# rasoolims/ImageTranslate

Measured on AMD Instinct MI355X. Metric: train tokens/sec (whole node), 6L enc-dec d=512 seq128 b64, 1/2/4/8 GPU, higher is better.
Workload: dtype bf16; 1 GPU; 6L/6L enc-dec d=512 h=8 ff=2048 V=30000, src[64,128] tgt[64,128], synthetic random-token MT; global_batch=64, seq_len=128, parallelism=dp1, distinct_batches=8, directions=2

## Files before the change

imagetranslate_amd/_lib.py:

```python
import ctypes
import os
from ctypes import POINTER, Structure, c_char_p, c_float, c_int, c_int32, c_int64, c_uint64, c_void_p

_HERE = os.path.dirname(os.path.abspath(__file__))
LIB_PATH = os.environ.get("IMT_LIB") or os.path.join(_HERE, "libimt_hip.so")

IMT_F32, IMT_BF16 = 0, 1
IMT_NT, IMT_NN, IMT_TN = 0, 1, 2
IMT_AUX_NONE, IMT_AUX_GELU_FWD, IMT_AUX_DGELU, IMT_AUX_SPLITK_WS = 0, 1, 2, 3


class GemmArgs(Structure):
    _fields_ = [
        ("dtype", c_int32), ("layout", c_int32),
        ("M", c_int32), ("N", c_int32), ("K", c_int32),
        ("A", c_void_p), ("lda", c_int64),
        ("B", c_void_p), ("ldb", c_int64),
        ("C", c_void_p), ("ldc", c_int64),
        ("c_dtype", c_int32), ("accumulate", c_int32),
        ("bias", c_void_p),
        ("resid", c_void_p), ("ldr", c_int64),
        ("aux", c_void_p), ("ldaux", c_int64),
        ("aux_mode", c_int32), ("split_k", c_int32),
        ("alpha", c_float), ("dropout_p", c_float),
        ("dropout_seed", c_uint64),
        ("alpha_dev", c_void_p),
        ("a_colsum", c_void_p),
        ("force_general", c_int32),
        ("ln_gamma", c_void_p), ("ln_beta", c_void_p),
        ("ln_out", c_void_p), ("ld_ln", c_int64),
        ("ln_mean", c_void_p), ("ln_rstd", c_void_p),
        ("ln_eps", c_float),
        ("splitk_ws", c_void_p), ("splitk_ws_bytes", c_int64),
    ]


class AttnArgs(Structure):
    _fields_ = [
        ("dtype", c_int32),
        ("B", c_int32), ("H", c_int32), ("Tq", c_int32), ("Tk", c_int32), ("head_dim", c_int32),
        ("Q", c_void_p), ("ldq", c_int64),
        ("K", c_void_p), ("ldk", c_int64),
        ("V", c_void_p), ("ldv", c_int64),
        ("O", c_void_p), ("ldo", c_int64),
        ("lse", c_void_p),
        ("key_mask", c_void_p), ("query_mask", c_void_p), ("mask3d", c_void_p),
        ("causal", c_int32), ("scale", c_float), ("dropout_p", c_float),
        ("dropout_seed", c_uint64),
        ("dO", c_void_p), ("lddo", c_int64),
        ("dQ", c_void_p), ("lddq", c_int64),
        ("dK", c_void_p), ("lddk", c_int64),
        ("dV", c_void_p), ("lddv", c_int64),
        ("delta", c_void_p),
    ]


class ProfRow(Structure):
    _fields_ = [("kind", ctypes.c_char * 48), ("launches", c_int64), ("total_ms", ctypes.c_double),
                ("flops", ctypes.c_double), ("bytes", ctypes.c_double)]


class AttnBlock(Structure):
    _fields_ = [("qkv_w", c_int64), ("qkv_b", c_int64), ("o_w", c_int64), ("o_b", c_int64), ("ln_g", c_int64),
                ("ln_b", c_int64)]


class LayerDesc(Structure):
    _fields_ = [("self_attn", AttnBlock), ("cross_attn", AttnBlock),
                ("ff1_w", c_int64), ("ff1_b", c_int64), ("ff2_w", c_int64), ("ff2_b", c_int64),
                ("ln2_g", c_int64), ("ln2_b", c_int64), ("cross_kv_w", c_int64), ("cross_kv_b", c_int64)]


class StackDesc(Structure):
    _fields_ = [
        ("dtype", c_int32),
        ("d", c_int32), ("heads", c_int32), ("ff", c_int32), ("vocab", c_int32), ("max_pos", c_int32),
        ("n_types", c_int32), ("n_layers", c_int32),
        ("is_decoder", c_int32), ("reserved", c_int32),
        ("pad_id", c_int64),
        ("ln_eps", c_float), ("hidden_dropout", c_float), ("attn_dropout", c_float), ("reserved_f", c_float),
        ("emb_word", c_int64), ("emb_pos", c_int64), ("emb_type", c_int64), ("emb_ln_g", c_int64), ("emb_ln_b", c_int64),
        ("layers", POINTER(LayerDesc)),
        ("params", c_void_p),
        ("grads", c_void_p),
    ]


class StackIO(Structure):
    _fields_ = [
        ("B", c_int32), ("T", c_int32), ("Tk", c_int32), ("training", c_int32),
        ("ids", c_void_p), ("type_ids", c_void_p), ("pos_ids", c_void_p),
        ("key_mask", c_void_p), ("query_mask", c_void_p), ("mask3d", c_void_p),
        ("causal", c_int32), ("reserved", c_int32),
        ("enc_states", c_void_p), ("enc_mask", c_void_p),
        ("out", c_void_p),
        ("dropout_seed", c_uint64),
        ("d_out", c_void_p), ("d_enc_states", c_void_p),
        ("wait_events", POINTER(c_void_p)), ("n_wait_events", c_int32), ("reserved2", c_int32),
    ]


class AttnDecodeArgs(Structure):
    _fields_ = [
        ("dtype", c_int32),
        ("R", c_int32), ("H", c_int32), ("head_dim", c_int32), ("n_keys", c_int32), ("rep", c_int32),
        ("Q", c_void_p), ("ldq", c_int64),
        ("K", c_void_p), ("V", c_void_p), ("ld_row", c_int64), ("ld_pos", c_int64),
        ("slots", c_void_p), ("ld_slots", c_int64),
        ("key_mask", c_void_p), ("ld_mask", c_int64),
        ("O", c_void_p), ("ldo", c_int64),
        ("scale", c_float), ("reserved", c_int32),
    ]


class DecodeIO(Structure):
    _fields_ = [
        ("R", c_int32), ("rep", c_int32), ("pos", c_int32), ("Tk", c_int32), ("t_max", c_int32), ("r_max", c_int32),
        ("ids", c_void_p), ("type_ids", c_void_p), ("pos_ids", c_void_p), ("slots", c_void_p), ("enc_mask", c_void_p),
        ("self_cache", c_void_p), ("cross_kv", c_void_p), ("out", c_void_p),
    ]


class BeamArgs(Structure):
    _fields_ = [
        ("B", c_int32), ("beam", c_int32), ("rep", c_int32), ("V", c_int32), ("step", c_int32), ("t_max", c_int32),
        ("logits", c_void_p), ("ld", c_int64),
        ("scores_in", c_void_p), ("sizes_in", c_void_p), ("eos_in", c_void_p), ("max_lens", c_void_p),
        ("hist_in", c_void_p), ("slots_in", c_void_p),
        ("len_penalty_ratio", c_float), ("reserved", c_int32),
        ("pad_idx", c_int64), ("eos", c_int64),
        ("cand_scores", c_void_p), ("cand_idx", c_void_p),
        ("scores_out", c_void_p), ("sizes_out", c_void_p), ("eos_out", c_void_p),
        ("hist_out", c_void_p), ("slots_out", c_void_p), ("parent_out", c_void_p), ("tokens_out", c_void_p),
        ("eos_count", c_void_p),
    ]


class SampleArgs(Structure):
    _fields_ = [
        ("B", c_int32), ("n", c_int32), ("rep", c_int32), ("V", c_int32), ("step", c_int32), ("t_max", c_int32),
        ("logits", c_void_p), ("ld", c_int64),
        ("scores_in", c_void_p), ("eos_in", c_void_p), ("max_lens", c_void_p), ("hist_in", c_void_p), ("slots_in", c_void_p),
        ("temperature", c_float), ("topk", c_int32), ("seed", c_uint64),
        ("pad_idx", c_int64), ("eos", c_int64),
        ("scores_out", c_void_p), ("eos_out", c_void_p),
        ("hist_out", c_void_p), ("slots_out", c_void_p), ("parent_out", c_void_p), ("tokens_out", c_void_p),
        ("eos_count", c_void_p),
    ]


class MassArgs(Structure):
    _fields_ = [
        ("n_rows", c_int32), ("width", c_int32), ("recover_width", c_int32), ("n_special", c_int32), ("vocab", c_int32),
        ("mask_prob", c_float), ("seed", c_uint64), ("mask_id", c_int64), ("pad_id", c_int64),
        ("src_text", c_void_p), ("pad_indices", c_void_p), ("row_offsets", c_void_p), ("first", c_void_p),
        ("src_mask", c_void_p),
        ("to_recover", c_void_p), ("positions", c_void_p), ("targets", c_void_p),
    ]


class MlmArgs(Structure):
    _fields_ = [
        ("n_rows", c_int32), ("width", c_int32), ("n_special", c_int32), ("vocab", c_int32),
        ("mask_eos", c_int32), ("mask_prob", c_float), ("seed", c_uint64), ("mask_id", c_int64), ("eos_id", c_int64),
        ("texts", c_void_p), ("pads", c_void_p), ("ld_pads", c_int64),
        ("mask", c_void_p), ("idx", c_void_p), ("targets", c_void_p), ("count", c_void_p),
    ]


class ScoreArgs(Structure):
    _fields_ = [
        ("dtype", c_int32), ("N", c_int32), ("V", c_int32), ("K", c_int32),
        ("x", c_void_p), ("ldx", c_int64),
        ("w", c_void_p), ("ldw", c_int64),
        ("bias", c_void_p), ("target", c_void_p),
        ("logprob", c_void_p), ("lse", c_void_p),
        ("seg_offsets", c_void_p), ("n_seg", c_int32), ("normalize", c_int32),
        ("seg_score", c_void_p),
        ("ws", c_void_p), ("ws_bytes", c_int64),
    ]


class KnnArgs(Structure):
    _fields_ = [
        ("dtype", c_int32), ("N", c_int32), ("M", c_int32), ("K", c_int32), ("k", c_int32),
        ("x", c_void_p), ("ldx", c_int64),
        ("y", c_void_p), ("ldy", c_int64),
        ("index_base", c_int32), ("splits", c_int32),
        ("val", c_void_p), ("idx", c_void_p),
        ("ws", c_void_p), ("ws_bytes", c_int64),
    ]


class AlignArgs(Structure):
    _fields_ = [
        ("dtype", c_int32), ("B", c_int32), ("S", c_int32), ("T", c_int32), ("d", c_int32),
        ("x", c_void_p), ("ldx", c_int64), ("bsx", c_int64),
        ("y", c_void_p), ("ldy", c_int64), ("bsy", c_int64),
        ("xr", c_void_p), ("yr", c_void_p),
        ("min_sim", c_float), ("reserved", c_int32),
        ("link", c_void_p), ("fwd_idx", c_void_p), ("fwd_val", c_void_p), ("bwd_idx", c_void_p), ("bwd_val", c_void_p),
    ]


class ConvArgs(Structure):
    _fields_ = [
        ("dtype", c_int32),
        ("B", c_int32), ("H", c_int32), ("W", c_int32), ("Cin", c_int32), ("Cout", c_int32), ("KH", c_int32), ("KW", c_int32),
        ("stride", c_int32), ("pad_h", c_int32), ("pad_w", c_int32), ("relu", c_int32),
        ("x", c_void_p), ("w", c_void_p), ("y", c_void_p),
        ("scale", c_void_p), ("shift", c_void_p), ("residual", c_void_p),
    ]


_P = c_void_p
SIGNATURES = {
    "imt_version": (c_int, []),
    "imt_last_error": (c_char_p, []),
    "imt_gemm": (c_int, [POINTER(GemmArgs), _P]),
    "imt_gemm_grouped_tn": (c_int, [POINTER(GemmArgs), c_int, _P]),
    "imt_gemm_grouped_tile_order": (c_int, [POINTER(c_int), POINTER(c_int), c_int, c_int, POINTER(c_int), c_int]),
    "imt_gemm_splitk_ws_bytes": (c_int64, []),
    "imt_gemm_bias_residual_ln_supported": (c_int, [c_int, c_int, c_int]),
    "imt_gemm_bias_residual_ln": (c_int, [c_int, _P, c_int64, _P, c_int64, _P, _P, c_int64, _P, _P, _P, _P, c_int64, _P, _P, c_int, c_int,
                                          c_int, c_float, c_float, c_uint64, _P]),
    "imt_colsum": (c_int, [c_int, _P, c_int64, c_int, c_int, _P, _P, _P]),
    "imt_layernorm_fwd": (c_int, [c_int, _P, _P, _P, _P, _P, _P, c_int, c_int, c_float, c_float, c_uint64, _P]),
    "imt_add_layernorm_fwd": (c_int, [c_int, _P, _P, _P, _P, _P, _P, _P, _P, c_int, c_int, c_float, c_float, c_uint64, _P]),
    "imt_embed_ln_fwd": (c_int, [c_int, _P, _P, _P, _P, _P, _P, _P, _P, _P, _P, _P, _P, c_int, c_int, c_int, c_int, c_int, c_int, c_float,
                                 c_float, c_uint64, _P]),
    "imt_layernorm_bwd": (c_int, [c_int, _P, _P, _P, _P, _P, _P, _P, _P, c_int, c_int, c_float, c_uint64, _P, c_float,
                                  c_uint64, _P, _P]),
    "imt_embed_fwd": (c_int, [c_int, _P, _P, _P, _P, _P, _P, _P, c_int, c_int, c_int, c_int, c_int, c_int, _P]),
    "imt_embed_bwd": (c_int, [c_int, _P, _P, _P, _P, _P, _P, _P, c_int, c_int, c_int, c_int64, _P]),
    "imt_attention_fwd": (c_int, [POINTER(AttnArgs), _P]),
    "imt_attention_bwd": (c_int, [POINTER(AttnArgs), _P]),
    "imt_attention_bwd_proj_supported": (c_int, [c_int, c_int, c_int, c_int, c_int, c_int, c_int]),
    "imt_attention_bwd_proj": (c_int, [POINTER(AttnArgs), _P, c_int64, _P, c_int64, c_int, _P]),
    "imt_gather_rows": (c_int, [c_int, _P, c_int64, _P, _P, c_int64, c_int, c_int, _P]),
    "imt_scatter_rows": (c_int, [c_int, _P, c_int64, _P, _P, c_int64, c_int, c_int, _P]),
    "imt_log_softmax_fwd": (c_int, [c_int, _P, c_int64, _P, c_int64, _P, c_int, c_int, _P]),
    "imt_log_softmax_bwd": (c_int, [_P, c_int64, _P, c_int64, c_int, _P, c_int64, c_int, c_int, _P]),
    "imt_smoothed_nll_fwd": (c_int, [_P, c_int64, _P, _P, c_int, c_int, c_float, c_int64, _P]),
    "imt_smoothed_nll_bwd": (c_int, [_P, _P, _P, c_int64, c_int, c_int, c_float, c_int64, _P]),
    "imt_xent_fused_fwd_bwd": (c_int, [c_int, _P, c_int64, _P, _P, c_int, c_int, c_float, c_int64, c_float, _P]),
    "imt_score_ws_bytes": (c_int64, [c_int, c_int]),
    "imt_score_supported": (c_int, [c_int, c_int, c_int]),
    "imt_score_rows": (c_int, [POINTER(ScoreArgs), _P]),
    "imt_knn_ws_bytes": (c_int64, [c_int, c_int, c_int, c_int]),
    "imt_knn_supported": (c_int, [c_int, c_int]),
    "imt_knn_rows": (c_int, [POINTER(KnnArgs), _P]),
    "imt_align_supported": (c_int, [c_int, c_int]),
    "imt_align_pairs": (c_int, [POINTER(AlignArgs), _P]),
    "imt_scaled_sum": (c_int, [_P, c_int, c_float, _P, _P]),
    "imt_conv2d_supported": (c_int, [c_int, c_int, c_int, c_int, c_int]),
    "imt_conv2d": (c_int, [POINTER(ConvArgs), _P]),
    "imt_maxpool2d_3x3s2": (c_int, [c_int, _P, _P, c_int, c_int, c_int, c_int, _P]),
    "imt_image_nhwc": (c_int, [c_int, _P, _P, c_int, c_int, c_int, POINTER(c_float), POINTER(c_float), _P]),
    "imt_sumsq": (c_int, [_P, c_int64, _P, _P, _P]),
    "imt_ln_partial_reduce": (c_int, [_P, c_int, c_int, _P, _P, _P, _P]),
    "imt_clip_adam": (c_int, [_P, _P, _P, _P, _P, c_int64, _P, c_float, c_float, c_float, c_float, c_float, c_float,
                              c_int64, c_int, _P]),
    "imt_clip_scale": (c_int, [_P, c_int64, _P, c_float, c_float, _P]),
    "imt_cast_f32_to_bf16": (c_int, [_P, _P, c_int64, _P]),
    "imt_gated_mix": (c_int, [c_int, _P, _P, _P, _P, c_int64, c_int, _P]),
    "imt_add_rows_dropout": (c_int, [c_int, _P, c_int, _P, _P, c_int64, c_int, c_int, c_float, c_uint64, _P]),
    "imt_obj_rows": (c_int, [c_int, c_int, _P, _P, _P, _P, _P, _P, _P, c_int64, c_int, c_int, _P, _P]),
    "imt_relu_dropout": (c_int, [c_int, _P, c_int64, c_int, c_float, c_uint64, _P]),
    "imt_relu_dropout_bwd": (c_int, [c_int, _P, _P, _P, c_int64, c_int, c_float, c_uint64, _P]),
    "imt_obj_fold_w": (c_int, [_P, _P, c_int, c_int, _P]),
    "imt_obj_embed_grad": (c_int, [c_int, _P, _P, c_int64, _P, c_int64, c_int, _P]),
    "imt_gated_mix_bwd": (c_int, [c_int, _P, _P, _P, _P, _P, _P, _P, _P, c_int64, c_int, _P]),
    "imt_attn_pool_plan": (c_int, [c_int, c_int, c_int]),
    "imt_attn_pool_fwd": (c_int, [c_int, _P, _P, _P, _P, _P, _P, _P, c_int64, c_int, c_int, _P]),
    "imt_attn_pool_bwd": (c_int, [c_int, _P, _P, _P, _P, _P, _P, _P, _P, _P, _P, _P, _P, c_int64, c_int, c_int, _P]),
    "imt_contrastive": (c_int, [_P, _P, _P, _P, _P, _P, c_int, c_int, c_int, _P]),
    "imt_sent_pool_fwd": (c_int, [c_int, _P, _P, _P, _P, _P, _P, c_int64, c_int, c_int, c_float, c_uint64, _P]),
    "imt_sent_pool_bwd": (c_int, [c_int, _P, _P, _P, _P, _P, _P, _P, _P, _P, c_int64, c_int, c_int, c_float, c_uint64, _P]),
    "imt_l2_dist": (c_int, [c_int, _P, _P, _P, _P, _P, c_int, c_int64, _P]),
    "imt_sensim_loss": (c_int, [_P, _P, _P, _P, _P, _P, c_int, c_int, c_int, c_int, _P]),
    "imt_pair_dot": (c_int, [_P, _P, _P, c_int64, c_int, _P]),
    "imt_pair_dot_bwd": (c_int, [_P, _P, _P, _P, _P, c_int64, c_int, _P]),
    "imt_proposal_attn_ws_bytes": (c_int64, [c_int64, c_int, c_int, c_int]),
    "imt_proposal_attn_fwd": (c_int, [c_int, _P, _P, _P, _P, _P, _P, _P, _P, _P, c_int64, c_int, c_int, c_int, c_int64, c_int64, c_float, _P]),
    "imt_proposal_attn_bwd": (c_int, [c_int, _P, _P, _P, _P, _P, _P, _P, _P, _P, _P, _P, _P, _P, _P, c_int64, c_int64, c_int, c_int, c_int,
                                      c_int64, c_int64, _P]),
    "imt_comm_unique_id_bytes": (c_int, []),
    "imt_comm_get_unique_id": (c_int, [_P]),
    "imt_comm_init": (c_int, [_P, c_int, c_int, POINTER(c_void_p)]),
    "imt_comm_allreduce": (c_int, [_P, _P, c_int64, c_int, _P]),
    "imt_comm_broadcast": (c_int, [_P, _P, c_int64, c_int, c_int, _P]),
    "imt_comm_destroy": (c_int, [_P]),
    "imt_set_gemm_share_cus": (c_int, [c_int]),
    "imt_set_gemm_grouped_tall_min_tiles": (c_int, [c_int]),
    "imt_debug_spin": (c_int, [c_int, c_int, c_int, c_int64, _P]),
    "imt_abi_sizeof": (c_int, [ctypes.c_char_p]),
    "imt_prof_enable": (c_int, [c_int]),
    "imt_prof_report": (c_int, [POINTER(ProfRow), c_int]),
    "imt_stack_workspace_bytes": (c_int64, [POINTER(StackDesc), c_int, c_int, c_int]),
    "imt_stack_forward": (c_int, [POINTER(StackDesc), POINTER(StackIO), _P, c_int64, _P]),
    "imt_stack_backward": (c_int, [POINTER(StackDesc), POINTER(StackIO), _P, c_int64, c_int, c_int, _P]),
    "imt_attention_decode": (c_int, [POINTER(AttnDecodeArgs), _P]),
    "imt_decode_workspace_bytes": (c_int64, [POINTER(StackDesc), c_int]),
    "imt_decode_self_cache_bytes": (c_int64, [POINTER(StackDesc), c_int, c_int]),
    "imt_decode_cross_bytes": (c_int64, [POINTER(StackDesc), c_int, c_int]),
    "imt_decode_begin": (c_int, [POINTER(StackDesc), _P, c_int, c_int, _P, _P]),
    "imt_decode_step": (c_int, [POINTER(StackDesc), POINTER(DecodeIO), _P, c_int64, _P]),
    "imt_decode_check": (c_int, [POINTER(StackDesc), c_int, _P, _P]),
    "imt_beam_step": (c_int, [POINTER(BeamArgs), _P]),
    "imt_sample_step": (c_int, [POINTER(SampleArgs), _P]),
    "imt_select_plan": (c_int, [_P, c_int64, _P, c_int64, c_int, c_int, c_int, _P, _P, _P, _P]),
    "imt_mass_mask": (c_int, [POINTER(MassArgs), _P]),
    "imt_mass_unmask": (c_int, [_P, _P, _P, _P, c_int, c_int, _P]),
    "imt_mlm_mask": (c_int, [POINTER(MlmArgs), _P]),
}

_lib = None


class ImtError(RuntimeError):
    pass


ABI_STRUCTS = {"imt_gemm_args": GemmArgs, "imt_attn_args": AttnArgs, "imt_prof_row": ProfRow, "imt_attn_block": AttnBlock,
               "imt_layer_desc": LayerDesc, "imt_stack_desc": StackDesc, "imt_stack_io": StackIO,
               "imt_attn_decode_args": AttnDecodeArgs, "imt_decode_io": DecodeIO, "imt_beam_args": BeamArgs,
               "imt_mass_args": MassArgs, "imt_score_args": ScoreArgs, "imt_sample_args": SampleArgs,
               "imt_knn_args": KnnArgs, "imt_mlm_args": MlmArgs, "imt_align_args": AlignArgs,
               "imt_conv_args": ConvArgs}


def load():
    global _lib
    if _lib is not None:
        return _lib
    if not os.path.exists(LIB_PATH):
        raise ImtError(
            "imagetranslate_amd: HIP extension %s is missing -- build it with "
            "`python -c 'import __graft_entry__ as g; g.build()'` (there is no CPU fallback)" % LIB_PATH)
    lib = ctypes.CDLL(LIB_PATH)
    for name, (res, args) in SIGNATURES.items():
        fn = getattr(lib, name)
        fn.restype = res
        fn.argtypes = args
    for cname, cls in ABI_STRUCTS.items():
        want = lib.imt_abi_sizeof(cname.encode())
        if want != ctypes.sizeof(cls):
            raise ImtError("imagetranslate_amd: %s is %d bytes in %s but %d in this binding -- rebuild the library "
                           "(python -c 'import __graft_entry__ as g; g.build()')" % (cname, want, LIB_PATH, ctypes.sizeof(cls)))
    _lib = lib
    return lib


def check(rc: int, what: str):
    if rc != 0:
        msg = load().imt_last_error()
        raise ImtError("%s failed (rc=%d): %s" % (what, rc, msg.decode() if msg else ""))
```

imagetranslate_amd/csrc/common.hpp:

```cpp
#pragma once
#include <hip/hip_runtime.h>
#include <stdint.h>
#include <stdio.h>
#include <string.h>
#include "../../include/imt_hip.h"

typedef __bf16 bf16_t;
typedef __attribute__((ext_vector_type(4))) float f32x4;
typedef __attribute__((ext_vector_type(2))) float f32x2;
typedef __attribute__((ext_vector_type(8))) __bf16 bf16x8;
typedef __attribute__((ext_vector_type(4))) __bf16 bf16x4;
typedef __attribute__((ext_vector_type(2))) __bf16 bf16x2;
typedef __attribute__((ext_vector_type(4))) short s16x4;
typedef __attribute__((ext_vector_type(4))) unsigned int u32x4;
typedef __attribute__((ext_vector_type(2))) unsigned int u32x2;

#define IMT_WAVE 64
#define IMT_DEVICE __device__ __forceinline__

void imt_set_error(const char* fmt, ...);

#define IMT_CHECK_ARG(cond, ...)                       \
  do {                                                  \
    if (!(cond)) {                                      \
      imt_set_error(__VA_ARGS__);                       \
      return IMT_ERR_BAD_ARG;                           \
    }                                                   \
  } while (0)

#define IMT_CHECK_LAUNCH()                                                   \
  do {                                                                       \
    hipError_t e__ = hipGetLastError();                                      \
    if (e__ != hipSuccess) {                                                 \
      imt_set_error("%s:%d launch failed: %s", __FILE__, __LINE__,           \
                    hipGetErrorString(e__));                                 \
      return IMT_ERR_LAUNCH;                                                 \
    }                                                                        \
  } while (0)

static inline int imt_cdiv(long a, long b) { return (int)((a + b - 1) / b); }
static inline bool imt_ok_dtype(int t) { return t == IMT_F32 || t == IMT_BF16; }
static inline int imt_dtype_bytes(int t) { return t == IMT_BF16 ? 2 : 4; }
static inline int64_t imt_align256(int64_t bytes) { return (bytes + 255) / 256 * 256; }
template <typename T> struct ImtType { typedef T type; };
template <typename F> static inline int imt_by_dtype(int dtype, F&& f) {
  return dtype == IMT_F32 ? f(ImtType<float>()) : f(ImtType<bf16_t>());
}

bool imt_gemm_grouped_tall(const imt_gemm_args* list, int count);

bool imt_prof_enabled();
const char* imt_prof_intern(const char* kind, int M, int N, int K);
void* imt_prof_begin_launch(const char* kind, double flops, double bytes, hipStream_t st);
void imt_prof_end_launch(void* tok, hipStream_t st);
#include <stdlib.h>
struct ImtTrace {
  static constexpr int MAXB = 4096;
  static constexpr int RING = 64;
  unsigned long long* dev = nullptr;
  const char* kind; int blocks; hipStream_t st;
  struct Slot { const char* kind; int blocks; };
  static Slot* slots() { static Slot s[RING]; return s; }
  static int& count() { static int c = 0; return c; }
  static bool ring() { static const bool r = getenv("IMT_TRACE_RING") != nullptr; return r; }
  ImtTrace(const char* kind_, int blocks_, hipStream_t st_) : kind(kind_), blocks(blocks_), st(st_) {
    static const char* want = getenv("IMT_TRACE");
    if (!want || (strcmp(want, kind_) != 0 && strcmp(want, "all") != 0) || blocks_ > MAXB || blocks_ <= 0) return;
    static unsigned long long* buf = nullptr;
    const size_t slice = (size_t)MAXB * 8;
    if (!buf && hipMalloc(&buf, (ring() ? RING : 1) * slice * sizeof(unsigned long long)) != hipSuccess) return;
    const int slot = ring() ? count() % RING : 0;
    if (ring()) slots()[slot] = Slot{kind_, blocks_};
    dev = buf + slot * slice;
    if (!ring()) (void)hipMemsetAsync(dev, 0, sizeof(unsigned long long) * 8 * blocks_, st);
    else if (slot == 0) (void)hipMemsetAsync(buf, 0, RING * slice * sizeof(unsigned long long), st);
  }
  ~ImtTrace() {
    if (!dev) return;
    static unsigned long long h[MAXB * 8];
    if (ring()) {
      if (++count() % RING != 0) return;
      (void)hipStreamSynchronize(st);
      unsigned long long* base = dev - (size_t)((count() - 1) % RING) * MAXB * 8;
      unsigned long long origin = 0, prev_end = 0;
      for (int s = 0; s < RING; ++s) {
        const Slot& sl = slots()[s];
        (void)hipMemcpy(h, base + (size_t)s * MAXB * 8, sizeof(unsigned long long) * 8 * sl.blocks, hipMemcpyDeviceToHost);
        unsigned long long t0 = ~0ull, t1 = 0, s1 = 0;
        for (int i = 0; i < 8 * sl.blocks; ++i) {
          if (!h[i]) continue;
          if (h[i] < t0) t0 = h[i];
          if (h[i] > t1) t1 = h[i];
          if ((i & 7) == 0 && h[i] > s1) s1 = h[i];
        }
        if (!origin) origin = t0;
        fprintf(stderr, "[ring %2d] %-10s %5d wgs  start %9.2f  last-start +%6.2f  end +%6.2f  dark-before %6.2f us\n", s, sl.kind, sl.blocks,
                (t0 - origin) * 0.01, (s1 - t0) * 0.01, (t1 - t0) * 0.01, prev_end ? ((double)t0 - (double)prev_end) * 0.01 : 0.0);
        prev_end = t1;
      }
      return;
    }
    (void)hipStreamSynchronize(st);
    (void)hipMemcpy(h, dev, sizeof(unsigned long long) * 8 * blocks, hipMemcpyDeviceToHost);
    unsigned long long t0 = ~0ull, t1 = 0;
    double ph[8] = {0, 0, 0, 0, 0, 0, 0, 0};
    int last = 0;
    for (int b = 0; b < blocks; ++b)
      for (int k = 0; k < 8; ++k) {
        const unsigned long long v = h[8 * b + k];
        if (!v) continue;
        if (v < t0) t0 = v;
        if (v > t1) t1 = v;
        if (k > last) last = k;
      }
    for (int b = 0; b < blocks; ++b) {
      unsigned long long prev = h[8 * b];
      for (int k = 1; k <= last; ++k) { const unsigned long long v = h[8 * b + k]; if (v && prev) { ph[k] += (v - prev) * 0.01; prev = v; } }
    }
    fprintf(stderr, "[trace %s] %d workgroups, span %.2f us; mean phases (us):", kind, blocks, (t1 - t0) * 0.01);
    for (int k = 1; k <= last; ++k) fprintf(stderr, " %.2f", ph[k] / blocks);
    fprintf(stderr, "\n");
  }
};
#define IMT_STAMP(trace, k) do { if ((trace) && threadIdx.x == 0) (trace)[8 * blockIdx.x + (k)] = wall_clock64(); } while (0)

struct ImtProfScope {
  void* tok; hipStream_t st;
  ImtProfScope(const char* kind, double flops, double bytes, hipStream_t s)
      : tok(imt_prof_enabled() ? imt_prof_begin_launch(kind, flops, bytes, s) : nullptr), st(s) {}
  ~ImtProfScope() { if (tok) imt_prof_end_launch(tok, st); }
};

IMT_DEVICE int imt_xcd_block(int bid, int nwg) {
  const int q = nwg >> 3, r = nwg & 7, xcd = bid & 7, idx = bid >> 3;
  return (xcd < r ? xcd * (q + 1) : r * (q + 1) + (xcd - r) * q) + idx;
}

template <typename T> IMT_DEVICE float to_f32(T v);
template <> IMT_DEVICE float to_f32<float>(float v) { return v; }
template <> IMT_DEVICE float to_f32<bf16_t>(bf16_t v) { return (float)v; }
template <typename T> IMT_DEVICE T from_f32(float v);
template <> IMT_DEVICE float from_f32<float>(float v) { return v; }
template <> IMT_DEVICE bf16_t from_f32<bf16_t>(float v) { return (bf16_t)v; }

template <typename T> struct Vec4;
template <> struct Vec4<float> {
  typedef f32x4 type;
  static IMT_DEVICE f32x4 load(const float* p) { return *reinterpret_cast<const f32x4*>(p); }
  static IMT_DEVICE void store(float* p, f32x4 v) { *reinterpret_cast<f32x4*>(p) = v; }
  static IMT_DEVICE void store_wt(float* p, f32x4 v) {
    typedef float f32x2_t __attribute__((ext_vector_type(2)));
    const f32x2_t lo = {v[0], v[1]}, hi = {v[2], v[3]};
    __hip_atomic_store(reinterpret_cast<unsigned long long*>(p), __builtin_bit_cast(unsigned long long, lo), __ATOMIC_RELAXED, __HIP_MEMORY_SCOPE_AGENT);
    __hip_atomic_store(reinterpret_cast<unsigned long long*>(p) + 1, __builtin_bit_cast(unsigned long long, hi), __ATOMIC_RELAXED, __HIP_MEMORY_SCOPE_AGENT);
  }
  static IMT_DEVICE type load_raw(const float* p) { return *reinterpret_cast<const f32x4*>(p); }
  static IMT_DEVICE f32x4 cvt(type v) { return v; }
};
template <> struct Vec4<bf16_t> {
  typedef bf16x4 type;
  static IMT_DEVICE f32x4 load(const bf16_t* p) {
    bf16x4 v = *reinterpret_cast<const bf16x4*>(p);
    f32x4 r = {(float)v[0], (float)v[1], (float)v[2], (float)v[3]};
    return r;
  }
  static IMT_DEVICE void store(bf16_t* p, f32x4 v) {
    bf16x4 r = {(bf16_t)v[0], (bf16_t)v[1], (bf16_t)v[2], (bf16_t)v[3]};
    *reinterpret_cast<bf16x4*>(p) = r;
  }
  static IMT_DEVICE void store_wt(bf16_t* p, f32x4 v) {
    bf16x4 r = {(bf16_t)v[0], (bf16_t)v[1], (bf16_t)v[2], (bf16_t)v[3]};
    __hip_atomic_store(reinterpret_cast<unsigned long long*>(p), __builtin_bit_cast(unsigned long long, r), __ATOMIC_RELAXED,
                       __HIP_MEMORY_SCOPE_AGENT);
  }
  static IMT_DEVICE type load_raw(const bf16_t* p) { return *reinterpret_cast<const bf16x4*>(p); }
  static IMT_DEVICE f32x4 cvt(type v) {
    f32x4 r = {(float)v[0], (float)v[1], (float)v[2], (float)v[3]};
    return r;
  }
};

IMT_DEVICE float wave_sum(float v) {
#pragma unroll
  for (int o = 32; o > 0; o >>= 1) v += __shfl_xor(v, o, 64);
  return v;
}
IMT_DEVICE float wave_max(float v) {
#pragma unroll
  for (int o = 32; o > 0; o >>= 1) v = fmaxf(v, __shfl_xor(v, o, 64));
  return v;
}
IMT_DEVICE bool better(float sa, int ia, float sb, int ib) { return sa > sb || (sa == sb && ia < ib); }
IMT_DEVICE void wave_best(float& s, int& i) {
#pragma unroll
  for (int o = 32; o > 0; o >>= 1) {
    const float so = __shfl_xor(s, o, 64);
    const int io = __shfl_xor(i, o, 64);
    if (better(so, io, s, i)) { s = so; i = io; }
  }
}

IMT_DEVICE void erf_and_gauss(float z, float& erf_v, float& gauss) {
  const float x = fabsf(z) * 0.70710678118654752440f;
  const float e = __expf(-x * x);
  const float t = __builtin_amdgcn_rcpf(fmaf(0.3275911f, x, 1.0f));
  float p = fmaf(1.061405429f, t, -1.453152027f);
  p = fmaf(p, t, 1.421413741f);
  p = fmaf(p, t, -0.284496736f);
  p = fmaf(p, t, 0.254829592f);
  const float y = 1.0f - p * t * e;
  erf_v = copysignf(y, z);
  gauss = e;
}
typedef float f32x2 __attribute__((ext_vector_type(2)));
IMT_DEVICE f32x2 pk_fma(f32x2 a, f32x2 b, f32x2 c) { return __builtin_elementwise_fma(a, b, c); }
IMT_DEVICE void erf_and_gauss2(f32x2 z, f32x2& erf_v, f32x2& gauss) {
  const f32x2 x = __builtin_elementwise_abs(z) * 0.70710678118654752440f;
  const f32x2 a = x * x * -1.4426950408889634f;
  f32x2 e, t;
  e.x = __builtin_amdgcn_exp2f(a.x); e.y = __builtin_amdgcn_exp2f(a.y);
  const f32x2 d = pk_fma(x, f32x2{0.3275911f, 0.3275911f}, f32x2{1.f, 1.f});
  t.x = __builtin_amdgcn_rcpf(d.x); t.y = __builtin_amdgcn_rcpf(d.y);
  f32x2 p = pk_fma(t, f32x2{-1.061405429f, -1.061405429f}, f32x2{1.453152027f, 1.453152027f});
  p = pk_fma(p, t, f32x2{-1.421413741f, -1.421413741f});
  p = pk_fma(p, t, f32x2{0.284496736f, 0.284496736f});
  p = pk_fma(p, t, f32x2{-0.254829592f, -0.254829592f});
  const f32x2 y = pk_fma(p * t, e, f32x2{1.f, 1.f});
  erf_v.x = copysignf(y.x, z.x); erf_v.y = copysignf(y.y, z.y);
  gauss = e;
}
IMT_DEVICE f32x4 gelu_erf4(f32x4 v) {
  f32x2 lo = {v[0], v[1]}, hi = {v[2], v[3]}, e0, g0, e1, g1;
  erf_and_gauss2(lo, e0, g0);
  erf_and_gauss2(hi, e1, g1);
  lo = lo * 0.5f * (e0 + 1.0f);
  hi = hi * 0.5f * (e1 + 1.0f);
  return f32x4{lo.x, lo.y, hi.x, hi.y};
}
IMT_DEVICE f32x4 gelu_erf_grad4(f32x4 z) {
  f32x2 lo = {z[0], z[1]}, hi = {z[2], z[3]}, e0, g0, e1, g1;
  erf_and_gauss2(lo, e0, g0);
  erf_and_gauss2(hi, e1, g1);
  lo = pk_fma(lo * 0.39894228040143267794f, g0, (e0 + 1.0f) * 0.5f);
  hi = pk_fma(hi * 0.39894228040143267794f, g1, (e1 + 1.0f) * 0.5f);
  return f32x4{lo.x, lo.y, hi.x, hi.y};
}
IMT_DEVICE float gelu_erf(float z) {
  float er, ga;
  erf_and_gauss(z, er, ga);
  return 0.5f * z * (1.0f + er);
}
IMT_DEVICE float gelu_erf_grad(float z) {
  float er, ga;
  erf_and_gauss(z, er, ga);
  return 0.5f * (1.0f + er) + z * 0.39894228040143267794f * ga;
}

IMT_DEVICE uint32_t mix32(uint32_t x) {
  x ^= x >> 16; x *= 0x7feb352dU; x ^= x >> 15; x *= 0x846ca68bU; x ^= x >> 16;
  return x;
}
IMT_DEVICE float counter_uniform(uint64_t seed, uint32_t stream, uint32_t index) {
  uint32_t h = mix32(index ^ (uint32_t)seed);
  h = mix32(h + stream * 0x9e3779b9U + (uint32_t)(seed >> 32));
  return (float)(h >> 8) * (1.0f / 16777216.0f);
}
IMT_DEVICE uint32_t dropout_key(uint64_t seed) { return (uint32_t)seed ^ ((uint32_t)(seed >> 32) * 0x9e3779b9U); }
IMT_DEVICE void dropout_block(uint32_t key, uint64_t idx4, uint32_t& h_lo, uint32_t& h_hi) {
  h_lo = mix32(((uint32_t)idx4 ^ key) + (uint32_t)(idx4 >> 32) * 0x85ebca6bU);
  h_hi = mix32(h_lo + 0x9e3779b9U);
}
IMT_DEVICE bool dropout_draw(uint32_t h_lo, uint32_t h_hi, int e , uint32_t thresh16) {
  const uint32_t w = (e & 2) ? h_hi : h_lo;
  return ((e & 1) ? (w >> 16) : (w & 0xffffu)) >= thresh16;
}
IMT_DEVICE bool dropout_keep(uint64_t seed, uint64_t idx, uint32_t thresh16) {
  uint32_t lo, hi;
  dropout_block(dropout_key(seed), idx >> 2, lo, hi);
  return dropout_draw(lo, hi, (int)(idx & 3), thresh16);
}
IMT_DEVICE void dropout_apply4(f32x4& v, uint64_t seed, uint64_t idx0, uint32_t thresh16, float inv_keep) {
  uint32_t lo, hi;
  dropout_block(dropout_key(seed), idx0 >> 2, lo, hi);
  v[0] = (lo & 0xffffu) >= thresh16 ? v[0] * inv_keep : 0.f;
  v[1] = (lo >> 16) >= thresh16 ? v[1] * inv_keep : 0.f;
  v[2] = (hi & 0xffffu) >= thresh16 ? v[2] * inv_keep : 0.f;
  v[3] = (hi >> 16) >= thresh16 ? v[3] * inv_keep : 0.f;
}
IMT_DEVICE uint32_t attn_drop_word(uint32_t key, uint64_t pair_idx) {
  return mix32(((uint32_t)pair_idx ^ key) + (uint32_t)(pair_idx >> 32) * 0x85ebca6bU);
}
IMT_DEVICE uint32_t attn_drop_word(uint32_t key, uint32_t pair_idx) { return mix32(pair_idx ^ key); }
IMT_DEVICE bool attn_drop_keep(uint32_t word, int j, uint32_t thresh16) {
  return ((j & 1) ? (word >> 16) : (word & 0xffffu)) >= thresh16;
}
static inline uint32_t dropout_thresh(float p) {
  if (p <= 0.f) return 0u;
  double t = (double)p * 65536.0 + 0.5;
  if (t > 65535.0) t = 65535.0;
  if (t < 1.0) t = 1.0;
  return (uint32_t)t;
}
```

imagetranslate_amd/csrc/model.hip:

```cpp
#include "common.hpp"
#include "decode_fused.hpp"

namespace {

struct Carver {
  char* base; int64_t off;
  explicit Carver(void* b) : base(reinterpret_cast<char*>(b)), off(0) {}
  void* take(int64_t bytes) {
    void* p = base ? base + off : nullptr;
    off += (bytes + 255) & ~(int64_t)255;
    return p;
  }
};

struct AttnWs {
  void* qkv;
  void* kv;
  int64_t kv_ld;
  void* ctx;
  float* lse;
  void* pre_ln;
  float* mean; float* rstd;
  void* out;
};
struct LayerWs {
  AttnWs self_attn, cross;
  void* z; void* h;
  void* pre_ln2; float* mean2; float* rstd2;
  void* out;
};
struct StackWs {
  void* emb_sum; float* emb_mean; float* emb_rstd; void* x0;
  LayerWs* layers;
  void* d_run;
  void* dpre[3]; void* ddrop[3];
  void* d_ctx;
  void* d_ff;
  void* d_qkv;
  void* d_q;
  void* d_kv;
  void* d_emb;
  static constexpr int N_SCRATCH = 4;
  struct Scratch { void* dpre[3]; void* ddrop[3]; void* d_ctx; void* d_ff; void* d_qkv; void* d_q; void* d_kv; } scr[N_SCRATCH];
  void use_scratch(int l) {
    const Scratch& z = scr[l % N_SCRATCH];
    for (int i = 0; i < 3; ++i) { dpre[i] = z.dpre[i]; ddrop[i] = z.ddrop[i]; }
    d_ctx = z.d_ctx; d_ff = z.d_ff; d_qkv = z.d_qkv; d_q = z.d_q; d_kv = z.d_kv;
  }
  void* kv_all; void* d_kv_all;
  float* delta;
  float* ln_partial;
  float* ln_site(int site, int d) const { return ln_partial + (int64_t)site * IMT_LN_BWD_WS_FLOATS(d); }
  void* splitk; int64_t splitk_bytes;
  int64_t bytes;
};

constexpr int MAX_LAYERS = 64;

int64_t kv_w_off(const imt_stack_desc* m, const imt_layer_desc& p) { return p.cross_kv_w >= 0 ? p.cross_kv_w : p.cross_attn.qkv_w + (int64_t)m->d * m->d; }
int64_t kv_b_off(const imt_stack_desc* m, const imt_layer_desc& p) { return p.cross_kv_b >= 0 ? p.cross_kv_b : p.cross_attn.qkv_b + m->d; }
bool cross_kv_batched(const imt_stack_desc* m) {
  if (!m->is_decoder || m->n_layers < 2) return false;
  const int64_t d = m->d;
  for (int l = 0; l < m->n_layers; ++l) {
    const imt_layer_desc& p = m->layers[l];
    if (p.cross_attn.qkv_w < 0 || p.cross_kv_w < 0 || p.cross_kv_b < 0) return false;
    if (p.cross_kv_w != m->layers[0].cross_kv_w + (int64_t)l * 2 * d * d) return false;
    if (p.cross_kv_b != m->layers[0].cross_kv_b + (int64_t)l * 2 * d) return false;
  }
  return true;
}

void carve(const imt_stack_desc* m, int B, int T, int Tk, void* ws, StackWs& w, LayerWs* layers) {
  Carver c(ws);
  const int64_t N = (int64_t)B * T, Nk = (int64_t)B * Tk, d = m->d, ff = m->ff, es = imt_dtype_bytes(m->dtype);
  w.emb_sum = c.take(N * d * es); w.emb_mean = (float*)c.take(N * 4); w.emb_rstd = (float*)c.take(N * 4);
  w.x0 = c.take(N * d * es);
  w.layers = layers;
  const bool batched = cross_kv_batched(m);
  const int64_t L2d = (int64_t)m->n_layers * 2 * d;
  w.kv_all = w.d_kv_all = nullptr;
  if (batched) { w.kv_all = c.take(Nk * L2d * es); w.d_kv_all = c.take(Nk * L2d * es); }
  for (int l = 0; l < m->n_layers; ++l) {
    LayerWs& L = layers[l];
    AttnWs& s = L.self_attn;
    s.qkv = c.take(N * 3 * d * es); s.kv = nullptr; s.ctx = c.take(N * d * es);
    s.lse = (float*)c.take((int64_t)B * m->heads * T * 4);
    s.pre_ln = c.take(N * d * es); s.mean = (float*)c.take(N * 4); s.rstd = (float*)c.take(N * 4);
    s.out = c.take(N * d * es);
    AttnWs& x = L.cross;
    memset(&x, 0, sizeof(x));
    if (m->is_decoder && m->layers[l].cross_attn.qkv_w >= 0) {
      x.qkv = c.take(N * d * es); x.ctx = c.take(N * d * es);
      if (batched) { x.kv = w.kv_all ? (void*)((char*)w.kv_all + (int64_t)l * 2 * d * es) : nullptr; x.kv_ld = L2d; }
      else { x.kv = c.take(Nk * 2 * d * es); x.kv_ld = 2 * d; }
      x.lse = (float*)c.take((int64_t)B * m->heads * T * 4);
      x.pre_ln = c.take(N * d * es); x.mean = (float*)c.take(N * 4); x.rstd = (float*)c.take(N * 4);
      x.out = c.take(N * d * es);
    }
    L.z = c.take(N * ff * es); L.h = c.take(N * ff * es);
    L.pre_ln2 = c.take(N * d * es); L.mean2 = (float*)c.take(N * 4); L.rstd2 = (float*)c.take(N * 4);
    L.out = c.take(N * d * es);
  }
  w.d_run = c.take(N * d * es);
  for (int k = 0; k < StackWs::N_SCRATCH; ++k) {
    StackWs::Scratch& z = w.scr[k];
    for (int i = 0; i < 3; ++i) { z.dpre[i] = c.take(N * d * es); z.ddrop[i] = c.take(N * d * es); }
    z.d_ctx = c.take(N * d * es);
    z.d_ff = c.take(N * ff * es);
    z.d_qkv = c.take(N * 3 * d * es);
    z.d_q = c.take(N * d * es);
    z.d_kv = c.take((Nk > 0 ? Nk : 1) * 2 * d * es);
  }
  w.use_scratch(0);
  w.d_emb = c.take(N * d * es);
  w.delta = (float*)c.take((int64_t)B * m->heads * T * 4);
  w.ln_partial = (float*)c.take((int64_t)(3 * m->n_layers + 1) * IMT_LN_BWD_WS_FLOATS(d) * 4);
  w.splitk_bytes = ((N + 127) / 128) * ((d + 127) / 128) <= 128 ? imt_gemm_splitk_ws_bytes() : 0;
  w.splitk = w.splitk_bytes ? c.take(w.splitk_bytes) : nullptr;
  w.bytes = c.off;
}

struct Ctx {
  const imt_stack_desc* m; hipStream_t st; int dtype; int64_t es;
  void* splitk = nullptr; int64_t splitk_bytes = 0;
  const char* P(int64_t off) const { return reinterpret_cast<const char*>(m->params) + off * es; }
  float* G(int64_t off) const { return m->grads + off; }
};

#define RC(x) do { int rc__ = (x); if (rc__ != IMT_OK) return rc__; } while (0)

int linear_fwd(const Ctx& c, const void* x, int64_t ldx, int M, int K, int64_t w_off, int64_t b_off, int N, void* y, int64_t ldy,
               const void* resid, int64_t ldr, void* aux, int aux_mode, float drop_p, uint64_t seed) {
  imt_gemm_args a;
  memset(&a, 0, sizeof(a));
  a.dtype = c.dtype; a.layout = IMT_NT; a.M = M; a.N = N; a.K = K;
  a.A = x; a.lda = ldx; a.B = c.P(w_off); a.ldb = K; a.C = y; a.ldc = ldy; a.c_dtype = c.dtype;
  a.bias = b_off >= 0 ? c.P(b_off) : nullptr;
  a.resid = resid; a.ldr = ldr; a.aux = aux; a.ldaux = N; a.aux_mode = aux_mode; a.split_k = 1; a.alpha = 1.f;
  a.dropout_p = drop_p; a.dropout_seed = seed;
  a.splitk_ws = c.splitk; a.splitk_ws_bytes = c.splitk_bytes;
  return imt_gemm(&a, c.st);
}

int linear_bwd_input(const Ctx& c, const void* dy, int64_t lddy, int M, int N, int64_t w_off, int K, void* dx, int64_t lddx,
                     const void* resid, int64_t ldr, void* aux, int aux_mode, int accumulate) {
  imt_gemm_args a;
  memset(&a, 0, sizeof(a));
  a.dtype = c.dtype; a.layout = IMT_NN; a.M = M; a.N = K; a.K = N;
  a.A = dy; a.lda = lddy; a.B = c.P(w_off); a.ldb = K; a.C = dx; a.ldc = lddx; a.c_dtype = c.dtype;
  a.resid = resid; a.ldr = ldr; a.aux = aux; a.ldaux = K; a.aux_mode = aux_mode; a.split_k = 1; a.alpha = 1.f;
  a.accumulate = accumulate;
  a.splitk_ws = c.splitk; a.splitk_ws_bytes = c.splitk_bytes;
  return imt_gemm(&a, c.st);
}

bool fuse_dense_ln(const Ctx& c, int M, int N, int K) {
  static const int mode = getenv("IMT_GEMM_LN") ? atoi(getenv("IMT_GEMM_LN")) : -1;
  if (mode == 0 || !imt_gemm_bias_residual_ln_supported(c.dtype, N, K)) return false;
  if (mode == 1) return true;
  return N <= 256 && K <= 1024;
}
int dense_resid_ln(const Ctx& c, const void* x, int64_t ldx, int M, int K, int64_t w_off, int64_t b_off, int N, const void* resid,
                   int64_t g_off, int64_t beta_off, void* pre_ln, void* out, float* mean, float* rstd, float drop_p, uint64_t seed) {
  if (fuse_dense_ln(c, M, N, K))
    return imt_gemm_bias_residual_ln(c.dtype, x, ldx, c.P(w_off), K, b_off >= 0 ? c.P(b_off) : nullptr, resid, N, c.P(g_off), c.P(beta_off),
                                     pre_ln, out, N, mean, rstd, M, N, K, c.m->ln_eps, drop_p, seed, c.st);
  imt_gemm_args a;
  memset(&a, 0, sizeof(a));
  a.dtype = c.dtype; a.layout = IMT_NT; a.M = M; a.N = N; a.K = K;
  a.A = x; a.lda = ldx; a.B = c.P(w_off); a.ldb = K; a.C = pre_ln; a.ldc = N; a.c_dtype = c.dtype;
  a.bias = b_off >= 0 ? c.P(b_off) : nullptr;
  a.resid = resid; a.ldr = N; a.aux_mode = IMT_AUX_NONE; a.split_k = 1; a.alpha = 1.f;
  a.dropout_p = drop_p; a.dropout_seed = seed;
  a.ln_gamma = c.P(g_off); a.ln_beta = c.P(beta_off); a.ln_out = out; a.ld_ln = N; a.ln_mean = mean; a.ln_rstd = rstd;
  a.ln_eps = c.m->ln_eps;
  a.splitk_ws = c.splitk; a.splitk_ws_bytes = c.splitk_bytes;
  return imt_gemm(&a, c.st);
}

struct DeferredDW {
  imt_gemm_args list[16];
  int n = 0;
  bool hold_for_pair() const {
    if (n == 0 || 2 * n > 16) return false;
    imt_gemm_args two[16];
    for (int i = 0; i < n; ++i) two[i] = two[n + i] = list[i];
    return imt_gemm_grouped_tall(two, 2 * n);
  }
  void add(const Ctx& c, const void* dy, int64_t lddy, const void* x, int64_t ldx, int M, int N, int K, int64_t w_off, int64_t b_off) {
    imt_gemm_args& a = list[n++];
    memset(&a, 0, sizeof(a));
    a.dtype = c.dtype; a.layout = IMT_TN; a.M = N; a.N = K; a.K = M;
    a.A = dy; a.lda = lddy; a.B = x; a.ldb = ldx; a.C = c.G(w_off); a.ldc = K; a.c_dtype = IMT_F32; a.alpha = 1.f;
    a.split_k = 1; a.accumulate = 1;
    a.a_colsum = b_off >= 0 ? c.G(b_off) : nullptr;
    const int tiles = imt_cdiv(N, 128) * imt_cdiv(K, 128);
    int sk = 1;
    while (sk < 8 && tiles * sk * 2 <= 256 && M / (sk * 2) >= 512) sk *= 2;
    if (M % (c.dtype == IMT_BF16 ? 64 : 32) != 0) { a.split_k = sk; a.accumulate = (sk == 1); }
  }
  int flush(hipStream_t st) {
    const int rc = n ? imt_gemm_grouped_tn(list, n, st) : IMT_OK;
    n = 0;
    return rc;
  }
};

struct SideQueue {
  hipStream_t st = nullptr;
  hipEvent_t ready[MAX_LAYERS], done[MAX_LAYERS];
  bool ok = false;
  bool init() {
    if (st) return ok;
    if (hipStreamCreateWithFlags(&st, hipStreamNonBlocking) != hipSuccess) { st = (hipStream_t)1; return ok = false; }
    for (int i = 0; i < MAX_LAYERS; ++i)
      if (hipEventCreateWithFlags(&ready[i], hipEventDisableTiming) != hipSuccess ||
          hipEventCreateWithFlags(&done[i], hipEventDisableTiming) != hipSuccess) return ok = false;
    return ok = true;
  }
};
SideQueue g_side;

uint64_t site_seed(uint64_t base, int layer, int site) { return base + 0x9E3779B97F4A7C15ull * (uint64_t)(layer * 16 + site + 1); }

struct MaskSet { const uint8_t* key; const uint8_t* query; const uint8_t* m3d; int causal; };

inline const char* offp(const void* p, int64_t elems, int64_t es) { return reinterpret_cast<const char*>(p) + elems * es; }
inline char* offp(void* p, int64_t elems, int64_t es) { return reinterpret_cast<char*>(p) + elems * es; }

imt_attn_args attn_block_args(const Ctx& c, const AttnWs& w, bool cross, int B, int T, int Tk, const MaskSet& ms, float drop_p,
                              uint64_t seed) {
  const int d = c.m->d;
  imt_attn_args a;
  memset(&a, 0, sizeof(a));
  a.dtype = c.dtype; a.B = B; a.H = c.m->heads; a.Tq = T; a.Tk = cross ? Tk : T; a.head_dim = d / c.m->heads;
  a.Q = w.qkv; a.ldq = cross ? d : 3 * d;
  if (cross) { a.K = w.kv; a.ldk = w.kv_ld; a.V = offp(w.kv, d, c.es); a.ldv = w.kv_ld; }
  else       { a.K = offp(w.qkv, d, c.es); a.ldk = 3 * d; a.V = offp(w.qkv, 2 * d, c.es); a.ldv = 3 * d; }
  a.O = w.ctx; a.ldo = d; a.lse = w.lse;
  a.key_mask = ms.key; a.query_mask = ms.query; a.mask3d = ms.m3d; a.causal = ms.causal;
  a.scale = 1.0f / sqrtf((float)a.head_dim);
  a.dropout_p = drop_p; a.dropout_seed = seed;
  return a;
}

int attn_block_fwd(const Ctx& c, const imt_attn_block& p, AttnWs& w, const void* x, int B, int T, const void* kv_src, int Tk,
                   const MaskSet& ms, bool training, uint64_t seed, int layer, int site0, int64_t kv_w = -1, int64_t kv_b = -1,
                   bool kv_ready = false) {
  const int d = c.m->d;
  const int N = B * T;
  const float hp = training ? c.m->hidden_dropout : 0.f, ap = training ? c.m->attn_dropout : 0.f;
  if (!kv_src) {
    RC(linear_fwd(c, x, d, N, d, p.qkv_w, p.qkv_b, 3 * d, w.qkv, 3 * d, nullptr, 0, nullptr, IMT_AUX_NONE, 0.f, 0));
  } else {
    const int Nk = B * Tk;
    RC(linear_fwd(c, x, d, N, d, p.qkv_w, p.qkv_b, d, w.qkv, d, nullptr, 0, nullptr, IMT_AUX_NONE, 0.f, 0));
    if (!kv_ready)
      RC(linear_fwd(c, kv_src, d, Nk, d, kv_w, kv_b, 2 * d, w.kv, w.kv_ld, nullptr, 0, nullptr, IMT_AUX_NONE, 0.f, 0));
  }
  const imt_attn_args a = attn_block_args(c, w, kv_src != nullptr, B, T, Tk, ms, ap, site_seed(seed, layer, site0));
  RC(imt_attention_fwd(&a, c.st));
  RC(dense_resid_ln(c, w.ctx, d, N, d, p.o_w, p.o_b, d, x, p.ln_g, p.ln_b, w.pre_ln, w.out, w.mean, w.rstd, hp, site_seed(seed, layer, site0 + 1)));
  return IMT_OK;
}

int attn_block_bwd(const Ctx& c, const imt_attn_block& p, AttnWs& w, StackWs& sw, DeferredDW& dw, int slot, const void* x, int B, int T,
                   const void* kv_src, int Tk, const MaskSet& ms, bool training, uint64_t seed, int layer, int site0, const void* dy,
                   void* d_kv_src, int accumulate_kv, int64_t kv_w = -1, int64_t kv_b = -1, void* d_kv_batched = nullptr) {
  const int d = c.m->d;
  const int N = B * T;
  const float hp = training ? c.m->hidden_dropout : 0.f, ap = training ? c.m->attn_dropout : 0.f;
  void* d_pre = sw.dpre[slot];
  void* d_dense = (hp > 0.f) ? sw.ddrop[slot] : d_pre;
  RC(imt_layernorm_bwd(c.dtype, dy, w.pre_ln, c.P(p.ln_g), w.mean, w.rstd, d_pre, c.G(p.ln_g), c.G(p.ln_b), N, d, 0.f, 0,
                       (hp > 0.f) ? d_dense : nullptr, hp, site_seed(seed, layer, site0 + 1), sw.ln_site(3 * layer + slot, d), c.st));
  dw.add(c, d_dense, d, w.ctx, d, N, d, d, p.o_w, p.o_b);
  imt_attn_args a = attn_block_args(c, w, kv_src != nullptr, B, T, Tk, ms, ap, site_seed(seed, layer, site0));
  const bool proj = imt_attention_bwd_proj_supported(a.dtype, a.head_dim, a.H, a.Tq, a.Tk, d, ms.m3d != nullptr);
  if (!proj) RC(linear_bwd_input(c, d_dense, d, N, d, p.o_w, d, sw.d_ctx, d, nullptr, 0, nullptr, IMT_AUX_NONE, 0));
  a.dO = proj ? nullptr : sw.d_ctx; a.lddo = d;
  a.delta = sw.delta;
  auto attn_bwd = [&]() { return proj ? imt_attention_bwd_proj(&a, d_dense, d, c.P(p.o_w), d, d, c.st) : imt_attention_bwd(&a, c.st); };
  if (!kv_src) {
    a.dQ = sw.d_qkv; a.lddq = 3 * d; a.dK = offp(sw.d_qkv, d, c.es); a.lddk = 3 * d; a.dV = offp(sw.d_qkv, 2 * d, c.es); a.lddv = 3 * d;
    RC(attn_bwd());
    dw.add(c, sw.d_qkv, 3 * d, x, d, N, 3 * d, d, p.qkv_w, p.qkv_b);
    RC(linear_bwd_input(c, sw.d_qkv, 3 * d, N, 3 * d, p.qkv_w, d, sw.d_run, d, d_pre, d, nullptr, IMT_AUX_NONE, 0));
  } else {
    const int Nk = B * Tk;
    void* dkv = d_kv_batched ? d_kv_batched : sw.d_kv;
    const int64_t lddkv = d_kv_batched ? w.kv_ld : 2 * d;
    a.dQ = sw.d_q; a.lddq = d; a.dK = dkv; a.lddk = lddkv; a.dV = offp(dkv, d, c.es); a.lddv = lddkv;
    RC(attn_bwd());
    dw.add(c, sw.d_q, d, x, d, N, d, d, p.qkv_w, p.qkv_b);
    RC(linear_bwd_input(c, sw.d_q, d, N, d, p.qkv_w, d, sw.d_run, d, d_pre, d, nullptr, IMT_AUX_NONE, 0));
    dw.add(c, dkv, lddkv, kv_src, d, Nk, 2 * d, d, kv_w, kv_b);
    if (!d_kv_batched) {
      if (d_kv_src)
        RC(linear_bwd_input(c, sw.d_kv, 2 * d, Nk, 2 * d, kv_w, d, d_kv_src, d, nullptr, 0, nullptr, IMT_AUX_NONE, accumulate_kv));
    }
  }
  return IMT_OK;
}

int ffn_fwd(const Ctx& c, const imt_layer_desc& p, LayerWs& w, const void* x, int N, bool training, uint64_t seed, int layer) {
  const int d = c.m->d, ff = c.m->ff;
  const float hp = training ? c.m->hidden_dropout : 0.f;
  RC(linear_fwd(c, x, d, N, d, p.ff1_w, p.ff1_b, ff, w.h, ff, nullptr, 0, w.z, IMT_AUX_GELU_FWD, 0.f, 0));
  RC(dense_resid_ln(c, w.h, ff, N, ff, p.ff2_w, p.ff2_b, d, x, p.ln2_g, p.ln2_b, w.pre_ln2, w.out, w.mean2, w.rstd2, hp, site_seed(seed, layer, 8)));
  return IMT_OK;
}

int ffn_bwd(const Ctx& c, const imt_layer_desc& p, LayerWs& w, StackWs& sw, DeferredDW& dw, const void* x, int N, bool training,
            uint64_t seed, int layer, const void* dy) {
  const int d = c.m->d, ff = c.m->ff;
  const float hp = training ? c.m->hidden_dropout : 0.f;
  void* d_pre = sw.dpre[0];
  void* d_dense = (hp > 0.f) ? sw.ddrop[0] : d_pre;
  RC(imt_layernorm_bwd(c.dtype, dy, w.pre_ln2, c.P(p.ln2_g), w.mean2, w.rstd2, d_pre, c.G(p.ln2_g), c.G(p.ln2_b), N, d, 0.f, 0,
                       (hp > 0.f) ? d_dense : nullptr, hp, site_seed(seed, layer, 8), sw.ln_site(3 * layer, d), c.st));
  dw.add(c, d_dense, d, w.h, ff, N, d, ff, p.ff2_w, p.ff2_b);
  RC(linear_bwd_input(c, d_dense, d, N, d, p.ff2_w, ff, sw.d_ff, ff, nullptr, 0, w.z, IMT_AUX_DGELU, 0));
  dw.add(c, sw.d_ff, ff, x, d, N, ff, d, p.ff1_w, p.ff1_b);
  RC(linear_bwd_input(c, sw.d_ff, ff, N, ff, p.ff1_w, d, sw.d_run, d, d_pre, d, nullptr, IMT_AUX_NONE, 0));
  return IMT_OK;
}

int validate(const imt_stack_desc* m, const imt_stack_io* io, const void* ws, int64_t ws_bytes, StackWs& w, LayerWs* layers) {
  IMT_CHECK_ARG(m && io, "stack: null descriptor");
  IMT_CHECK_ARG(imt_ok_dtype(m->dtype), "stack: bad dtype");
  IMT_CHECK_ARG(m->n_layers >= 0 && m->n_layers <= MAX_LAYERS && (m->n_layers == 0 || m->layers), "stack: bad layer table");
  IMT_CHECK_ARG(m->d > 0 && m->heads > 0 && m->d % m->heads == 0, "stack: hidden size %d not a multiple of heads %d", m->d, m->heads);
  const int dh = m->d / m->heads;
  IMT_CHECK_ARG(dh == 32 || dh == 64, "stack: head_dim %d unsupported (32 or 64)", dh);
  IMT_CHECK_ARG(m->d % 8 == 0 && m->ff % 8 == 0, "stack: d and ff must be multiples of 8");
  IMT_CHECK_ARG(io->B > 0 && io->T > 0, "stack: empty batch");
  IMT_CHECK_ARG(io->T <= m->max_pos || io->pos_ids, "stack: sequence longer than max_position_embeddings");
  IMT_CHECK_ARG(m->params && io->ids && io->out, "stack: null tensor");
  if (m->is_decoder) IMT_CHECK_ARG(io->enc_states && io->Tk > 0, "stack: decoder needs encoder states");
  carve(m, io->B, io->T, m->is_decoder ? io->Tk : 0, const_cast<void*>(ws), w, layers);
  IMT_CHECK_ARG(ws && ws_bytes >= w.bytes, "stack: workspace too small (%lld < %lld)", (long long)ws_bytes, (long long)w.bytes);
  IMT_CHECK_ARG(((uintptr_t)ws & 255) == 0, "stack: workspace must be 256-B aligned");
  return IMT_OK;
}

}

extern "C" int64_t imt_stack_workspace_bytes(const imt_stack_desc* m, int B, int T, int Tk) {
  if (!m || m->n_layers > MAX_LAYERS || (m->n_layers > 0 && !m->layers)) return -1;
  StackWs w; LayerWs layers[MAX_LAYERS];
  carve(m, B, T, m->is_decoder ? Tk : 0, nullptr, w, layers);
  return w.bytes;
}

extern "C" int imt_stack_forward(const imt_stack_desc* m, const imt_stack_io* io, void* ws, int64_t ws_bytes, void* stream) {
  StackWs w; LayerWs layers[MAX_LAYERS];
  RC(validate(m, io, ws, ws_bytes, w, layers));
  Ctx c{m, (hipStream_t)stream, m->dtype, imt_dtype_bytes(m->dtype)};
  c.splitk = w.splitk; c.splitk_bytes = w.splitk_bytes;
  const int B = io->B, T = io->T, N = B * T, d = m->d;
  const bool training = io->training != 0;
  const uint64_t seed = io->dropout_seed;
  void* x0 = (m->n_layers == 0) ? io->out : w.x0;
  auto wait_site = [&](int k) {
    if (io->wait_events && k < io->n_wait_events && io->wait_events[k])
      (void)hipStreamWaitEvent(c.st, (hipEvent_t)const_cast<void*>(io->wait_events[k]), 0);
  };
  wait_site(0);
  RC(imt_embed_ln_fwd(c.dtype, io->ids, io->pos_ids, io->type_ids, c.P(m->emb_word), c.P(m->emb_pos), c.P(m->emb_type), c.P(m->emb_ln_g),
                      c.P(m->emb_ln_b), w.emb_sum, x0, w.emb_mean, w.emb_rstd, N, T, d, m->vocab, m->max_pos, m->n_types, m->ln_eps,
                      training ? m->hidden_dropout : 0.f, site_seed(seed, 1000, 0), c.st));
  const void* x = x0;
  const MaskSet self_ms{io->key_mask, io->query_mask, io->mask3d, io->causal};
  const MaskSet cross_ms{io->enc_mask, nullptr, nullptr, 0};
  const bool batched = cross_kv_batched(m);
  if (batched)
    RC(linear_fwd(c, io->enc_states, d, B * io->Tk, d, m->layers[0].cross_kv_w, m->layers[0].cross_kv_b, m->n_layers * 2 * d, w.kv_all,
                  (int64_t)m->n_layers * 2 * d, nullptr, 0, nullptr, IMT_AUX_NONE, 0.f, 0));
  for (int l = 0; l < m->n_layers; ++l) {
    const imt_layer_desc& p = m->layers[l];
    LayerWs& L = layers[l];
    wait_site(1 + l);
    RC(attn_block_fwd(c, p.self_attn, L.self_attn, x, B, T, nullptr, 0, self_ms, training, seed, l, 0));
    const void* a = L.self_attn.out;
    if (m->is_decoder && p.cross_attn.qkv_w >= 0) {
      RC(attn_block_fwd(c, p.cross_attn, L.cross, a, B, T, io->enc_states, io->Tk, cross_ms, training, seed, l, 4, kv_w_off(m, p),
                        kv_b_off(m, p), batched));
      a = L.cross.out;
    }
    if (l == m->n_layers - 1) L.out = io->out;
    RC(ffn_fwd(c, p, L, a, N, training, seed, l));
    x = L.out;
  }
  return IMT_OK;
}

extern "C" int imt_stack_backward(const imt_stack_desc* m, const imt_stack_io* io, void* ws, int64_t ws_bytes, int layer_lo,
                                  int layer_hi, void* stream) {
  StackWs w; LayerWs layers[MAX_LAYERS];
  RC(validate(m, io, ws, ws_bytes, w, layers));
  IMT_CHECK_ARG(m->grads && io->d_out, "stack_backward: grads / d_out missing");
  IMT_CHECK_ARG(0 <= layer_lo && layer_lo <= layer_hi && layer_hi <= m->n_layers, "stack_backward: bad layer range");
  Ctx c{m, (hipStream_t)stream, m->dtype, imt_dtype_bytes(m->dtype)};
  c.splitk = w.splitk; c.splitk_bytes = w.splitk_bytes;
  const int B = io->B, T = io->T, N = B * T, d = m->d;
  const bool training = io->training != 0;
  const uint64_t seed = io->dropout_seed;
  const MaskSet self_ms{io->key_mask, io->query_mask, io->mask3d, io->causal};
  const MaskSet cross_ms{io->enc_mask, nullptr, nullptr, 0};
  const void* dy = (layer_hi == m->n_layers) ? io->d_out : w.d_run;
  const bool batched = cross_kv_batched(m);
  DeferredDW dw;
  const int64_t lnf = IMT_LN_BWD_WS_FLOATS(d);
  if (layer_hi > layer_lo) (void)hipMemsetAsync(w.ln_site(3 * layer_lo, d), 0, (size_t)(3 * (layer_hi - layer_lo)) * lnf * 4, c.st);
  if (layer_lo == 0) (void)hipMemsetAsync(w.ln_site(3 * m->n_layers, d), 0, (size_t)lnf * 4, c.st);
  static const bool side_env = !(getenv("IMT_DW_SIDE_STREAM") && atoi(getenv("IMT_DW_SIDE_STREAM")) == 0);
  const bool whole = layer_lo == 0 && layer_hi == m->n_layers && m->n_layers >= 2;
  const bool side = side_env && !imt_prof_enabled() && whole && g_side.init();
  const bool pairs = whole && !imt_prof_enabled();
  int last_side = -1;
  int held = -1;
  for (int l = layer_hi - 1; l >= layer_lo; --l) {
    const imt_layer_desc& p = m->layers[l];
    LayerWs& L = layers[l];
    w.use_scratch(l);
    if (side && l + StackWs::N_SCRATCH < layer_hi) (void)hipStreamWaitEvent(c.st, g_side.done[l + StackWs::N_SCRATCH], 0);
    if (l == m->n_layers - 1) L.out = io->out;
    const bool has_cross = m->is_decoder && p.cross_attn.qkv_w >= 0;
    const void* x_in = (l == 0) ? w.x0 : (const void*)layers[l - 1].out;
    const void* a_self = L.self_attn.out;
    const void* a_ffn_in = has_cross ? L.cross.out : a_self;
    RC(ffn_bwd(c, p, L, w, dw, a_ffn_in, N, training, seed, l, dy));
    if (has_cross) {
      const bool first_cross = (l == m->n_layers - 1);
      void* dkv_l = batched ? offp(w.d_kv_all, (int64_t)l * 2 * d, c.es) : nullptr;
      RC(attn_block_bwd(c, p.cross_attn, L.cross, w, dw, 1, a_self, B, T, io->enc_states, io->Tk, cross_ms, training, seed, l, 4, w.d_run,
                        io->d_enc_states, first_cross ? 0 : 1, kv_w_off(m, p), kv_b_off(m, p), dkv_l));
    }
    RC(attn_block_bwd(c, p.self_attn, L.self_attn, w, dw, 2, x_in, B, T, nullptr, 0, self_ms, training, seed, l, 0, w.d_run, nullptr, 0));
    const bool first_of_pair = pairs && held < 0 && l > layer_lo && dw.hold_for_pair();
    if (first_of_pair) {
      held = l;
    } else if (side) {
      (void)hipEventRecord(g_side.ready[l], c.st);
      (void)hipStreamWaitEvent(g_side.st, g_side.ready[l], 0);
      RC(dw.flush(g_side.st));
      (void)hipEventRecord(g_side.done[l], g_side.st);
      if (held >= 0) (void)hipEventRecord(g_side.done[held], g_side.st);
      held = -1;
      last_side = l;
    } else {
      RC(dw.flush(c.st));
      held = -1;
    }
    dy = w.d_run;
  }
  if (layer_lo == 0 && batched) {
    const int Nk = B * io->Tk;
    const int L2d = m->n_layers * 2 * d;
    if (io->d_enc_states)
      RC(linear_bwd_input(c, w.d_kv_all, L2d, Nk, L2d, m->layers[0].cross_kv_w, d, io->d_enc_states, d, nullptr, 0, nullptr, IMT_AUX_NONE, 0));
  }
  if (layer_lo == 0) {
    const void* dy0 = (m->n_layers == 0) ? io->d_out : dy;
    RC(imt_layernorm_bwd(c.dtype, dy0, w.emb_sum, c.P(m->emb_ln_g), w.emb_mean, w.emb_rstd, w.d_emb, c.G(m->emb_ln_g), c.G(m->emb_ln_b), N, d,
                         training ? m->hidden_dropout : 0.f, site_seed(seed, 1000, 0), nullptr, 0.f, 0, w.ln_site(3 * m->n_layers, d), c.st));
    RC(imt_embed_bwd(c.dtype, io->ids, io->pos_ids, io->type_ids, w.d_emb, c.G(m->emb_word), c.G(m->emb_pos), c.G(m->emb_type), N, T, d,
                     m->pad_id, c.st));
  }
  {
    static int64_t g_off[3 * MAX_LAYERS + 1], b_off[3 * MAX_LAYERS + 1];
    const int first = 3 * layer_lo, emb = 3 * m->n_layers;
    const int last = (layer_lo == 0) ? emb + 1 : 3 * layer_hi;
    for (int sidx = first; sidx < last; ++sidx) {
      g_off[sidx - first] = -1; b_off[sidx - first] = -1;
      if (sidx == emb) { g_off[sidx - first] = m->emb_ln_g; b_off[sidx - first] = m->emb_ln_b; continue; }
      const int l = sidx / 3, slot = sidx % 3;
      if (l >= layer_hi) continue;
      const imt_layer_desc& p = m->layers[l];
      if (slot == 0) { g_off[sidx - first] = p.ln2_g; b_off[sidx - first] = p.ln2_b; }
      else if (slot == 2) { g_off[sidx - first] = p.self_attn.ln_g; b_off[sidx - first] = p.self_attn.ln_b; }
      else if (m->is_decoder && p.cross_attn.qkv_w >= 0) { g_off[sidx - first] = p.cross_attn.ln_g; b_off[sidx - first] = p.cross_attn.ln_b; }
    }
    if (last > first) RC(imt_ln_partial_reduce(w.ln_site(first, d), last - first, d, g_off, b_off, m->grads, c.st));
  }
  if (last_side >= 0) (void)hipStreamWaitEvent(c.st, g_side.done[last_side], 0);
  return IMT_OK;
}

namespace {

struct DecodeWs {
  void* emb_sum; void* x; void* ctx; void* pre_ln; void* a; void* q; void* b; void* h; void* z; float* mean; float* rstd;
  void* splitk; int64_t splitk_bytes;
  char* fused; int64_t fused_layer_bytes; unsigned* fused_bar;
  int64_t bytes;
};

bool fused_decode_shape(const imt_stack_desc* m) {
  return m->dtype == IMT_BF16 && imt_decode_fused_shape(m->d, m->heads, m->ff, m->n_layers);
}

void carve_decode(const imt_stack_desc* m, int r_max, void* ws, DecodeWs& w) {
  Carver c(ws);
  const int64_t R = r_max, d = m->d, ff = m->ff, es = imt_dtype_bytes(m->dtype);
  w.emb_sum = c.take(R * d * es); w.x = c.take(R * d * es); w.ctx = c.take(R * d * es); w.pre_ln = c.take(R * d * es);
  w.a = c.take(R * d * es); w.q = c.take(R * d * es); w.b = c.take(R * d * es);
  w.h = c.take(R * ff * es); w.z = c.take(R * ff * es);
  w.mean = (float*)c.take(R * 4); w.rstd = (float*)c.take(R * 4);
  w.splitk_bytes = imt_gemm_splitk_ws_bytes();
  w.splitk = c.take(w.splitk_bytes);
  w.fused = nullptr; w.fused_layer_bytes = 0; w.fused_bar = nullptr;
  if (fused_decode_shape(m)) {
    w.fused_layer_bytes = (imt_decode_fused_layer_bytes(r_max, m->d, m->ff) + 255) & ~(int64_t)255;
    w.fused = (char*)c.take(w.fused_layer_bytes * m->n_layers);
    w.fused_bar = (unsigned*)c.take(IMT_FUSED_BAR_WORDS * sizeof(unsigned));
  }
  w.bytes = c.off;
}

int validate_decoder(const imt_stack_desc* m) {
  IMT_CHECK_ARG(m, "decode: null descriptor");
  IMT_CHECK_ARG(imt_ok_dtype(m->dtype), "decode: bad dtype");
  IMT_CHECK_ARG(m->is_decoder, "decode: stack is not a decoder");
  IMT_CHECK_ARG(m->n_layers > 0 && m->n_layers <= MAX_LAYERS && m->layers, "decode: bad layer table");
  IMT_CHECK_ARG(m->d > 0 && m->heads > 0 && m->d % m->heads == 0, "decode: hidden size %d not a multiple of heads %d", m->d, m->heads);
  const int dh = m->d / m->heads;
  IMT_CHECK_ARG(dh == 32 || dh == 64, "decode: head_dim %d unsupported (32 or 64)", dh);
  IMT_CHECK_ARG(m->d % 8 == 0 && m->ff % 8 == 0, "decode: d and ff must be multiples of 8");
  IMT_CHECK_ARG(m->params, "decode: null parameter buffer");
  for (int l = 0; l < m->n_layers; ++l)
    IMT_CHECK_ARG(m->layers[l].cross_attn.qkv_w >= 0, "decode: layer %d has no crossattention block", l);
  return IMT_OK;
}

}

extern "C" int64_t imt_decode_workspace_bytes(const imt_stack_desc* m, int r_max) {
  if (!m || r_max <= 0) return -1;
  DecodeWs w;
  carve_decode(m, r_max, nullptr, w);
  return w.bytes;
}
extern "C" int64_t imt_decode_self_cache_bytes(const imt_stack_desc* m, int r_max, int t_max) {
  if (!m || r_max <= 0 || t_max <= 0) return -1;
  return (int64_t)m->n_layers * r_max * t_max * 3 * m->d * imt_dtype_bytes(m->dtype);
}
extern "C" int64_t imt_decode_cross_bytes(const imt_stack_desc* m, int B, int Tk) {
  if (!m || B <= 0 || Tk <= 0) return -1;
  return (int64_t)m->n_layers * B * Tk * 2 * m->d * imt_dtype_bytes(m->dtype);
}

extern "C" int imt_decode_begin(const imt_stack_desc* m, const void* enc_states, int B, int Tk, void* cross_kv, void* stream) {
  RC(validate_decoder(m));
  IMT_CHECK_ARG(enc_states && cross_kv && B > 0 && Tk > 0, "decode_begin: bad arguments");
  Ctx c{m, (hipStream_t)stream, m->dtype, imt_dtype_bytes(m->dtype)};
  const int d = m->d;
  const int64_t per_layer = (int64_t)B * Tk * 2 * d;
  for (int l = 0; l < m->n_layers; ++l) {
    const imt_attn_block& p = m->layers[l].cross_attn;
    RC(linear_fwd(c, enc_states, d, B * Tk, d, kv_w_off(m, m->layers[l]), kv_b_off(m, m->layers[l]), 2 * d,
                  offp(cross_kv, l * per_layer, c.es), 2 * d, nullptr, 0, nullptr, IMT_AUX_NONE, 0.f, 0));
  }
  return IMT_OK;
}

extern "C" int imt_decode_check(const imt_stack_desc* m, int r_max, const void* ws, void* stream) {
  RC(validate_decoder(m));
  IMT_CHECK_ARG(ws && r_max > 0, "decode_check: bad arguments");
  DecodeWs w;
  carve_decode(m, r_max, const_cast<void*>(ws), w);
  if (!w.fused || !imt_decode_fused_enabled()) return IMT_OK;
  unsigned status = 0;
  if (hipMemcpyAsync(&status, w.fused_bar + IMT_FUSED_BAR_WORDS - 1, sizeof(unsigned), hipMemcpyDeviceToHost, (hipStream_t)stream) != hipSuccess ||
      hipStreamSynchronize((hipStream_t)stream) != hipSuccess) {
    imt_set_error("decode_check: cannot read the status word");
    return IMT_ERR_LAUNCH;
  }
  if (status != 0) {
    imt_set_error("decode: a one-launch decoder step was abandoned (grid barrier %u timed out); its tokens are not valid", status & 0xfffu);
    return IMT_ERR_LAUNCH;
  }
  return IMT_OK;
}

extern "C" int imt_decode_step(const imt_stack_desc* m, const imt_decode_io* io, void* ws, int64_t ws_bytes, void* stream) {
  RC(validate_decoder(m));
  IMT_CHECK_ARG(io, "decode_step: null io");
  IMT_CHECK_ARG(io->R > 0 && io->rep > 0 && io->R % io->rep == 0 && io->R <= io->r_max, "decode_step: bad row counts (R=%d rep=%d r_max=%d)", io->R, io->rep, io->r_max);
  IMT_CHECK_ARG(io->pos >= 0 && io->pos < io->t_max && io->Tk > 0, "decode_step: position %d outside the cache (t_max=%d)", io->pos, io->t_max);
  IMT_CHECK_ARG(io->ids && io->pos_ids && io->self_cache && io->cross_kv && io->out, "decode_step: null tensor");
  DecodeWs w;
  carve_decode(m, io->r_max, ws, w);
  IMT_CHECK_ARG(ws && ws_bytes >= w.bytes, "decode_step: workspace too small (%lld < %lld)", (long long)ws_bytes, (long long)w.bytes);
  IMT_CHECK_ARG(((uintptr_t)ws & 255) == 0, "decode_step: workspace must be 256-B aligned");
  Ctx c{m, (hipStream_t)stream, m->dtype, imt_dtype_bytes(m->dtype)};
  c.splitk = w.splitk; c.splitk_bytes = w.splitk_bytes;
  const int R = io->R, d = m->d, ff = m->ff, H = m->heads, dh = d / H;
  const int64_t row3 = (int64_t)io->t_max * 3 * d;
  const int64_t self_layer = (int64_t)io->r_max * row3;
  const int B = R / io->rep;
  const int64_t cross_layer = (int64_t)B * io->Tk * 2 * d;
  if (w.fused && imt_decode_fused_enabled()) {
    ImtFusedArgs f;
    memset(&f, 0, sizeof(f));
    const bf16_t* P = reinterpret_cast<const bf16_t*>(m->params);
    for (int l = 0; l < m->n_layers; ++l) {
      const imt_layer_desc& p = m->layers[l];
      ImtFusedLayer& L = f.L[l];
      L.wqkv = P + p.self_attn.qkv_w; L.bqkv = P + p.self_attn.qkv_b; L.wo = P + p.self_attn.o_w; L.bo = P + p.self_attn.o_b;
      L.g1 = P + p.self_attn.ln_g; L.b1 = P + p.self_attn.ln_b;
      L.wq = P + p.cross_attn.qkv_w; L.bq = P + p.cross_attn.qkv_b; L.wo2 = P + p.cross_attn.o_w; L.bo2 = P + p.cross_attn.o_b;
      L.g2 = P + p.cross_attn.ln_g; L.b2 = P + p.cross_attn.ln_b;
      L.w1 = P + p.ff1_w; L.bf1 = P + p.ff1_b; L.w2 = P + p.ff2_w; L.bf2 = P + p.ff2_b; L.g3 = P + p.ln2_g; L.b3 = P + p.ln2_b;
      L.cache = reinterpret_cast<bf16_t*>(offp(io->self_cache, l * self_layer, c.es));
      L.cross_kv = reinterpret_cast<const bf16_t*>(offp(io->cross_kv, l * cross_layer, c.es));
      Carver fc(w.fused + l * w.fused_layer_bytes);
      const int64_t rm = io->r_max;
      L.xin = (bf16_t*)fc.take(rm * d * 2); L.ctx1 = (bf16_t*)fc.take(rm * d * 2); L.a = (bf16_t*)fc.take(rm * d * 2);
      L.q = (bf16_t*)fc.take(rm * d * 2); L.ctx2 = (bf16_t*)fc.take(rm * d * 2); L.b = (bf16_t*)fc.take(rm * d * 2);
      L.h = (bf16_t*)fc.take(rm * ff * 2);
      L.pre1 = (float*)fc.take(rm * d * 4); L.pre2 = (float*)fc.take(rm * d * 4); L.pre3 = (float*)fc.take(rm * d * 4);
    }
    f.n_layers = m->n_layers; f.d = d; f.R = R; f.rep = io->rep; f.pos = io->pos; f.Tk = io->Tk; f.t_max = io->t_max; f.r_max = io->r_max;
    f.H = H; f.dh = dh; f.ff = ff;
    f.ids = io->ids; f.pos_ids = io->pos_ids; f.type_ids = io->type_ids;
    f.emb_word = P + m->emb_word; f.emb_pos = P + m->emb_pos; f.emb_type = P + m->emb_type; f.emb_g = P + m->emb_ln_g; f.emb_b = P + m->emb_ln_b;
    f.vocab = m->vocab; f.max_pos = m->max_pos; f.n_types = m->n_types;
    f.out = reinterpret_cast<bf16_t*>(io->out);
    f.slots = io->slots; f.enc_mask = io->enc_mask; f.eps = m->ln_eps; f.bar = w.fused_bar;
    if (io->pos == 0 && hipMemsetAsync(w.fused_bar + IMT_FUSED_BAR_WORDS - 1, 0, sizeof(unsigned), c.st) != hipSuccess) {
      imt_set_error("decode_step: memset failed");
      return IMT_ERR_LAUNCH;
    }
    return imt_decode_fused_launch(f, c.st);
  }
  RC(imt_embed_ln_fwd(c.dtype, io->ids, io->pos_ids, io->type_ids, c.P(m->emb_word), c.P(m->emb_pos), c.P(m->emb_type), c.P(m->emb_ln_g),
                      c.P(m->emb_ln_b), w.emb_sum, w.x, w.mean, w.rstd, R, 1, d, m->vocab, m->max_pos, m->n_types, m->ln_eps, 0.f, 0, c.st));
  const void* x = w.x;
  for (int l = 0; l < m->n_layers; ++l) {
    const imt_layer_desc& p = m->layers[l];
    void* cache_l = offp(io->self_cache, l * self_layer, c.es);
    void* qkv_new = offp(cache_l, (int64_t)io->pos * 3 * d, c.es);
    RC(linear_fwd(c, x, d, R, d, p.self_attn.qkv_w, p.self_attn.qkv_b, 3 * d, qkv_new, row3, nullptr, 0, nullptr, IMT_AUX_NONE, 0.f, 0));
    imt_attn_decode_args a;
    memset(&a, 0, sizeof(a));
    a.dtype = c.dtype; a.R = R; a.H = H; a.head_dim = dh; a.n_keys = io->pos + 1; a.rep = 1;
    a.Q = qkv_new; a.ldq = row3;
    a.K = offp(cache_l, d, c.es); a.V = offp(cache_l, 2 * d, c.es); a.ld_row = row3; a.ld_pos = 3 * d;
    a.slots = io->slots; a.ld_slots = io->t_max;
    a.O = w.ctx; a.ldo = d; a.scale = 1.0f / sqrtf((float)dh);
    RC(imt_attention_decode(&a, c.st));
    RC(dense_resid_ln(c, w.ctx, d, R, d, p.self_attn.o_w, p.self_attn.o_b, d, x, p.self_attn.ln_g, p.self_attn.ln_b, w.pre_ln, w.a, w.mean, w.rstd, 0.f, 0));
    RC(linear_fwd(c, w.a, d, R, d, p.cross_attn.qkv_w, p.cross_attn.qkv_b, d, w.q, d, nullptr, 0, nullptr, IMT_AUX_NONE, 0.f, 0));
    const void* kv_l = offp(io->cross_kv, l * cross_layer, c.es);
    memset(&a, 0, sizeof(a));
    a.dtype = c.dtype; a.R = R; a.H = H; a.head_dim = dh; a.n_keys = io->Tk; a.rep = io->rep;
    a.Q = w.q; a.ldq = d;
    a.K = kv_l; a.V = offp(kv_l, d, c.es); a.ld_row = (int64_t)io->Tk * 2 * d; a.ld_pos = 2 * d;
    a.key_mask = io->enc_mask; a.ld_mask = io->Tk;
    a.O = w.ctx; a.ldo = d; a.scale = 1.0f / sqrtf((float)dh);
    RC(imt_attention_decode(&a, c.st));
    RC(dense_resid_ln(c, w.ctx, d, R, d, p.cross_attn.o_w, p.cross_attn.o_b, d, w.a, p.cross_attn.ln_g, p.cross_attn.ln_b, w.pre_ln, w.b, w.mean, w.rstd, 0.f, 0));
    RC(linear_fwd(c, w.b, d, R, d, p.ff1_w, p.ff1_b, ff, w.h, ff, nullptr, 0, w.z, IMT_AUX_GELU_FWD, 0.f, 0));
    void* y = (l == m->n_layers - 1) ? io->out : w.x;
    RC(dense_resid_ln(c, w.h, ff, R, ff, p.ff2_w, p.ff2_b, d, w.b, p.ln2_g, p.ln2_b, w.pre_ln, y, w.mean, w.rstd, 0.f, 0));
    x = y;
  }
  return IMT_OK;
}
```

imagetranslate_amd/csrc/rowops.hip:

```cpp
#include <stdlib.h>
#include "common.hpp"

namespace {

constexpr int ROWS_PER_BLOCK = 4;

template <typename T> struct LnSrc {
  const T* x; const T* resid; T* sum_out;
  const int64_t* ids; const int64_t* pos_ids; const int64_t* type_ids;
  const T* word; const T* pos; const T* type;
  int seq_len, vocab, max_pos, n_types;
};

template <typename T, int NCH, int SRC>
__global__ __launch_bounds__(256) void ln_fwd_kernel(LnSrc<T> src, const T* __restrict__ gamma,
                                                     const T* __restrict__ beta, T* __restrict__ y,
                                                     float* __restrict__ mean_out, float* __restrict__ rstd_out,
                                                     int rows, int d, float eps, uint32_t thresh, float inv_keep,
                                                     uint64_t seed) {
  const int lane = threadIdx.x & 63;
  const int row = imt_xcd_block(blockIdx.x, gridDim.x) * ROWS_PER_BLOCK + (threadIdx.x >> 6);
  if (row >= rows) return;
  f32x4 v[NCH], gv[NCH], bv[NCH];
  float s = 0.f;
  if (SRC == 2) {
    int64_t wi = src.ids[row];
    int64_t pi = src.pos_ids ? src.pos_ids[row] : (int64_t)(row % src.seq_len);
    int64_t ti = src.type_ids ? src.type_ids[row] : 0;
    if (wi < 0 || wi >= src.vocab) wi = 0;
    if (pi < 0 || pi >= src.max_pos) pi = 0;
    if (ti < 0 || ti >= src.n_types) ti = 0;
    const T* wr = src.word + wi * d;
    const T* pr = src.pos + pi * d;
    const T* tr = src.type + ti * d;
#pragma unroll
    for (int i = 0; i < NCH; ++i) {
      const int c = min(lane * 4 + i * 256, d - 4);
      const f32x4 a = Vec4<T>::load(wr + c), b = Vec4<T>::load(pr + c), t = Vec4<T>::load(tr + c);
      gv[i] = Vec4<T>::load(gamma + c);
      bv[i] = Vec4<T>::load(beta + c);
      v[i] = a + b;
      v[i] += t;
    }
  } else {
    const T* xr = src.x + (int64_t)row * d;
    const T* rr = (SRC == 1) ? src.resid + (int64_t)row * d : xr;
#pragma unroll
    for (int i = 0; i < NCH; ++i) {
      const int c = min(lane * 4 + i * 256, d - 4);
      v[i] = Vec4<T>::load(xr + c);
      if (SRC == 1) v[i] += Vec4<T>::load(rr + c);
      gv[i] = Vec4<T>::load(gamma + c);
      bv[i] = Vec4<T>::load(beta + c);
    }
  }
  if (SRC != 0) {
    T* so = src.sum_out + (int64_t)row * d;
#pragma unroll
    for (int i = 0; i < NCH; ++i) {
      const int c = lane * 4 + i * 256;
#pragma unroll
      for (int e = 0; e < 4; ++e) v[i][e] = to_f32<T>(from_f32<T>(v[i][e]));
      if (c < d) Vec4<T>::store(so + c, v[i]);
    }
  }
#pragma unroll
  for (int i = 0; i < NCH; ++i)
    if (lane * 4 + i * 256 < d) s += v[i][0] + v[i][1] + v[i][2] + v[i][3];
  const float mean = wave_sum(s) / (float)d;
  float q = 0.f;
#pragma unroll
  for (int i = 0; i < NCH; ++i) {
    const int c = lane * 4 + i * 256;
    if (c < d) {
#pragma unroll
      for (int e = 0; e < 4; ++e) { const float t = v[i][e] - mean; q += t * t; }
    }
  }
  const float var = wave_sum(q) / (float)d;
  const float rstd = 1.0f / sqrtf(var + eps);
  if (lane == 0) { mean_out[row] = mean; rstd_out[row] = rstd; }
  T* yr = y + (int64_t)row * d;
#pragma unroll
  for (int i = 0; i < NCH; ++i) {
    const int c = lane * 4 + i * 256;
    if (c < d) {
      const f32x4 g = gv[i], b = bv[i];
      f32x4 o;
#pragma unroll
      for (int e = 0; e < 4; ++e) o[e] = (v[i][e] - mean) * rstd * g[e] + b[e];
      if (thresh) dropout_apply4(o, seed, (uint64_t)row * d + c, thresh, inv_keep);
      Vec4<T>::store(yr + c, o);
    }
  }
}

template <typename T, int NCH, int WPB>
__global__ __launch_bounds__(WPB * 64, ((WPB == 8 && NCH <= 2 && sizeof(T) == 2) ? 4 : 1)) void ln_bwd_kernel(const T* __restrict__ dy, const T* __restrict__ x,
                                                     const T* __restrict__ gamma, const float* __restrict__ mean,
                                                     const float* __restrict__ rstd, T* __restrict__ dx,
                                                     float* __restrict__ dgamma, float* __restrict__ dbeta, int rows,
                                                     int d, int rows_per_wave, uint32_t y_thresh, float y_inv_keep,
                                                     uint64_t y_seed, T* __restrict__ dx_drop, uint32_t dx_thresh,
                                                     float dx_inv_keep, uint64_t dx_seed, float* __restrict__ partial,
                                                     unsigned long long* trace) {
  __shared__ float red[2][WPB][NCH * 256];
  IMT_STAMP(trace, 0);
  const int lane = threadIdx.x & 63, w = threadIdx.x >> 6;
  f32x4 g[NCH], ag[NCH], ab[NCH];
#pragma unroll
  for (int i = 0; i < NCH; ++i) {
    const int c = lane * 4 + i * 256;
    g[i] = Vec4<T>::load(gamma + min(c, d - 4));
    ag[i] = f32x4{0.f, 0.f, 0.f, 0.f};
    ab[i] = f32x4{0.f, 0.f, 0.f, 0.f};
  }
  const int row_begin = (imt_xcd_block(blockIdx.x, gridDim.x) * WPB + w) * rows_per_wave;
  constexpr int RB = 4;
  for (int r0 = 0; r0 < rows_per_wave; r0 += RB) {
    f32x4 xb[RB][NCH], db[RB][NCH];
    float mub[RB], rsb[RB];
#pragma unroll
    for (int k = 0; k < RB; ++k) {
      const int row = min(row_begin + r0 + k, rows - 1);
      mub[k] = mean[row];
      rsb[k] = rstd[row];
#pragma unroll
      for (int i = 0; i < NCH; ++i) {
        const int c = min(lane * 4 + i * 256, d - 4);
        xb[k][i] = Vec4<T>::load(x + (int64_t)row * d + c);
        db[k][i] = Vec4<T>::load(dy + (int64_t)row * d + c);
      }
    }
    if (r0 == 0) IMT_STAMP(trace, 1);
#pragma unroll
    for (int k = 0; k < RB; ++k) {
      const int row = row_begin + r0 + k;
      if (r0 == 0 && k == 1) IMT_STAMP(trace, 3);
      if (!((r0 + k < rows_per_wave) && (row < rows))) continue;
      const float mu = mub[k], rs = rsb[k];
      float s1 = 0.f, s2 = 0.f;
#pragma unroll
      for (int i = 0; i < NCH; ++i) {
        const int c = lane * 4 + i * 256;
        if (c < d) {
          if (y_thresh) dropout_apply4(db[k][i], y_seed, (uint64_t)row * d + c, y_thresh, y_inv_keep);
#pragma unroll
          for (int e = 0; e < 4; ++e) {
            xb[k][i][e] = (xb[k][i][e] - mu) * rs;
            const float dg = db[k][i][e] * g[i][e];
            s1 += dg;
            s2 += dg * xb[k][i][e];
            ag[i][e] += db[k][i][e] * xb[k][i][e];
            ab[i][e] += db[k][i][e];
          }
        }
      }
      const float c1 = wave_sum(s1) / (float)d, c2 = wave_sum(s2) / (float)d;
      if (r0 == 0 && k == 0) IMT_STAMP(trace, 2);
#pragma unroll
      for (int i = 0; i < NCH; ++i) {
        const int c = lane * 4 + i * 256;
        if (c < d) {
          f32x4 o;
#pragma unroll
          for (int e = 0; e < 4; ++e) o[e] = rs * (db[k][i][e] * g[i][e] - c1 - xb[k][i][e] * c2);
          Vec4<T>::store(dx + (int64_t)row * d + c, o);
          if (dx_drop) {
            f32x4 o2 = o;
            if (dx_thresh) dropout_apply4(o2, dx_seed, (uint64_t)row * d + c, dx_thresh, dx_inv_keep);
            Vec4<T>::store(dx_drop + (int64_t)row * d + c, o2);
          }
        }
      }
    }
  }
  IMT_STAMP(trace, 5);
#pragma unroll
  for (int i = 0; i < NCH; ++i)
#pragma unroll
    for (int e = 0; e < 4; ++e) {
      red[0][w][i * 256 + lane * 4 + e] = ag[i][e];
      red[1][w][i * 256 + lane * 4 + e] = ab[i][e];
    }
  __syncthreads();
  for (int c = threadIdx.x; c < d; c += WPB * 64) {
    float sg = 0.f, sb = 0.f;
#pragma unroll
    for (int k = 0; k < WPB; ++k) { sg += red[0][k][c]; sb += red[1][k][c]; }
    if (partial) {
      float* pc = partial + (size_t)(blockIdx.x & (IMT_LN_PARTIAL_COPIES - 1)) * 2 * d;
      atomicAdd(pc + c, sg);
      atomicAdd(pc + d + c, sb);
    } else if (dgamma) {
      atomicAdd(dgamma + c, sg);
      atomicAdd(dbeta + c, sb);
    }
  }
  IMT_STAMP(trace, 6);
}

template <typename T>
__global__ __launch_bounds__(256) void embed_fwd_kernel(const int64_t* __restrict__ ids, const int64_t* __restrict__ pos_ids,
                                                        const int64_t* __restrict__ type_ids, const T* __restrict__ word,
                                                        const T* __restrict__ pos, const T* __restrict__ type,
                                                        T* __restrict__ out, int n_tokens, int seq_len, int d, int vocab,
                                                        int max_pos, int n_types) {
  const int lane = threadIdx.x & 63;
  const int n = imt_xcd_block(blockIdx.x, gridDim.x) * ROWS_PER_BLOCK + (threadIdx.x >> 6);
  if (n >= n_tokens) return;
  int64_t wi = ids[n];
  int64_t pi = pos_ids ? pos_ids[n] : (int64_t)(n % seq_len);
  int64_t ti = type_ids ? type_ids[n] : 0;
  if (wi < 0 || wi >= vocab) wi = 0;
  if (pi < 0 || pi >= max_pos) pi = 0;
  if (ti < 0 || ti >= n_types) ti = 0;
  const T* wr = word + wi * d;
  const T* pr = pos + pi * d;
  const T* tr = type + ti * d;
  for (int c = lane * 4; c < d; c += 256) {
    f32x4 v = Vec4<T>::load(wr + c) + Vec4<T>::load(pr + c);
    v += Vec4<T>::load(tr + c);
    Vec4<T>::store(out + (int64_t)n * d + c, v);
  }
}

template <typename T, int NT_REG>
__global__ __launch_bounds__(256) void embed_bwd_kernel(const int64_t* __restrict__ ids, const int64_t* __restrict__ pos_ids,
                                                        const int64_t* __restrict__ type_ids, const T* __restrict__ dsum,
                                                        float* __restrict__ dword, float* __restrict__ dpos,
                                                        float* __restrict__ dtype_tab, int n_tokens, int seq_len, int d,
                                                        int64_t pad_id, int tokb) {
  const bool posmajor = (pos_ids == nullptr) && (n_tokens % seq_len == 0);
  const int nsent = n_tokens / seq_len;
  int first, stride, count, p_own = 0;
  if (posmajor) {
    p_own = blockIdx.x % seq_len;
    const int s0 = (blockIdx.x / seq_len) * tokb;
    first = s0 * seq_len + p_own; stride = seq_len; count = min(tokb, nsent - s0);
  } else {
    first = imt_xcd_block(blockIdx.x, gridDim.x) * tokb; stride = 1; count = min(tokb, n_tokens - first);
  }
  if (count <= 0) return;
  for (int c = threadIdx.x; c < d; c += 256) {
    float tacc[NT_REG], pacc = 0.f;
#pragma unroll
    for (int k = 0; k < NT_REG; ++k) tacc[k] = 0.f;
    for (int kb = 0; kb < count; kb += 4) {
      float vb[4];
      int64_t wb[4], pb[4], tb[4];
      const int64_t* pp = pos_ids ? pos_ids : ids;
      const int64_t* tp = type_ids ? type_ids : ids;
#pragma unroll
      for (int k = 0; k < 4; ++k) {
        const int n = first + min(kb + k, count - 1) * stride;
        vb[k] = to_f32<T>(dsum[(int64_t)n * d + c]);
        wb[k] = ids[n];
        pb[k] = pp[n];
        tb[k] = tp[n];
      }
#pragma unroll
      for (int k = 0; k < 4; ++k) {
        if (kb + k >= count) break;
        const int n = first + (kb + k) * stride;
        const float v = vb[k];
        const int64_t wi = wb[k];
        const int64_t ti = type_ids ? tb[k] : 0;
        if (wi != pad_id) atomicAdd(dword + wi * d + c, v);
        if (posmajor) pacc += v;
        else atomicAdd(dpos + (pos_ids ? pb[k] : (int64_t)(n % seq_len)) * d + c, v);
        bool hit = false;
#pragma unroll
        for (int q = 0; q < NT_REG; ++q)
          if (ti == q) { tacc[q] += v; hit = true; }
        if (!hit) atomicAdd(dtype_tab + ti * d + c, v);
      }
    }
    if (posmajor) atomicAdd(dpos + (int64_t)p_own * d + c, pacc);
#pragma unroll
    for (int k = 0; k < NT_REG; ++k)
      if (tacc[k] != 0.f) atomicAdd(dtype_tab + (int64_t)k * d + c, tacc[k]);
  }
}

template <typename T>
__global__ __launch_bounds__(256) void colsum_kernel(const T* __restrict__ X, int64_t ldx, int M, int N,
                                                     float* __restrict__ out, int rows_per_block,
                                                     const float* __restrict__ scale_dev) {
  __shared__ f32x4 red[4][64];
  const int lane = threadIdx.x & 63, w = threadIdx.x >> 6;
  const int c = blockIdx.x * 256 + lane * 4;
  const int r0 = blockIdx.y * rows_per_block;
  const int r1 = min(M, r0 + rows_per_block);
  f32x4 acc = {0.f, 0.f, 0.f, 0.f};
  if (c < N) {
    const bool full = (c + 3 < N);
    for (int r = r0 + w; r < r1; r += 4) {
      if (full) acc += Vec4<T>::load(X + (int64_t)r * ldx + c);
      else
        for (int e = 0; e < 4 && c + e < N; ++e) acc[e] += to_f32<T>(X[(int64_t)r * ldx + c + e]);
    }
  }
  red[w][lane] = acc;
  __syncthreads();
  if (w == 0 && c < N) {
    f32x4 s = red[0][lane] + red[1][lane] + red[2][lane] + red[3][lane];
    if (scale_dev) s *= scale_dev[0];
    for (int e = 0; e < 4 && c + e < N; ++e) atomicAdd(out + c + e, s[e]);
  }
}

template <typename T>
__global__ __launch_bounds__(256) void gather_rows_kernel(const T* __restrict__ x, int64_t ldx, const int32_t* __restrict__ idx,
                                                          T* __restrict__ out, int64_t ldo, int n_sel, int d, int scatter) {
  const int lane = threadIdx.x & 63;
  const int r = imt_xcd_block(blockIdx.x, gridDim.x) * ROWS_PER_BLOCK + (threadIdx.x >> 6);
  if (r >= n_sel) return;
  const int64_t src = scatter ? (int64_t)r : (int64_t)idx[r];
  const int64_t dst = scatter ? (int64_t)idx[r] : (int64_t)r;
  for (int c = lane * 4; c < d; c += 256) {
    typedef typename Vec4<T>::type raw_t;
    *reinterpret_cast<raw_t*>(out + dst * ldo + c) = *reinterpret_cast<const raw_t*>(x + src * ldx + c);
  }
}

__global__ __launch_bounds__(256) void cast_bf16_kernel(const float* __restrict__ src, bf16_t* __restrict__ dst, int64_t n) {
  const int64_t stride = (int64_t)gridDim.x * 256 * 4;
  for (int64_t i = ((int64_t)blockIdx.x * 256 + threadIdx.x) * 4; i < n; i += stride) {
    if (i + 3 < n) Vec4<bf16_t>::store(dst + i, Vec4<float>::load(src + i));
    else
      for (int64_t e = i; e < n; ++e) dst[e] = (bf16_t)src[e];
  }
}

template <typename T>
__global__ __launch_bounds__(256) void gated_mix_kernel(const T* __restrict__ a, const T* __restrict__ b,
                                                        const T* __restrict__ gate, T* __restrict__ out, int64_t rows, int d) {
  const int lane = threadIdx.x & 63;
  const int64_t r = (int64_t)blockIdx.x * ROWS_PER_BLOCK + (threadIdx.x >> 6);
  if (r >= rows) return;
  for (int c = lane * 4; c < d; c += 256) {
    const f32x4 av = Vec4<T>::load(a + r * d + c), bv = Vec4<T>::load(b + r * d + c), gv = Vec4<T>::load(gate + c);
    f32x4 o;
#pragma unroll
    for (int e = 0; e < 4; ++e) {
      const float s = 1.0f / (1.0f + __expf(-(gv[e] + 1e-7f)));
      o[e] = s * av[e] + (1.0f - s) * bv[e];
    }
    Vec4<T>::store(out + r * d + c, o);
  }
}

template <typename TI, typename TO>
__global__ __launch_bounds__(256) void add_rows_dropout_kernel(const TI* __restrict__ x, TO* __restrict__ out,
                                                               const TO* __restrict__ add, int64_t rows, int d, int period,
                                                               uint32_t thresh, float inv_keep, uint64_t seed) {
  const int lane = threadIdx.x & 63;
  const int64_t r = (int64_t)blockIdx.x * ROWS_PER_BLOCK + (threadIdx.x >> 6);
  if (r >= rows) return;
  const TO* ar = add ? add + (int64_t)(r % period) * d : nullptr;
  for (int c = lane * 4; c < d; c += 256) {
    f32x4 v = Vec4<TI>::load(x + r * d + c);
    if (ar) v += Vec4<TO>::load(ar + c);
    if (thresh) dropout_apply4(v, seed, (uint64_t)r * d + c, thresh, inv_keep);
    Vec4<TO>::store(out + r * d + c, v);
  }
}

template <typename T, int NCH>
int ln_fwd_launch(int mode, const LnSrc<T>& src, const void* gamma, const void* beta, void* y, float* mean, float* rstd, int rows,
                  int d, float eps, float p, uint64_t seed, hipStream_t st) {
  static const char* const kinds[3] = {"layernorm_fwd", "add_layernorm_fwd", "embed_ln_fwd"};
  ImtProfScope prof(kinds[mode], 0.0, (mode == 0 ? 2.0 : mode == 1 ? 4.0 : 5.0) * rows * d * sizeof(T), st);
  const dim3 grid(imt_cdiv(rows, ROWS_PER_BLOCK));
  const uint32_t th = dropout_thresh(p);
  const float ik = p > 0.f ? 1.f / (1.f - p) : 1.f;
  if (mode == 0)
    hipLaunchKernelGGL((ln_fwd_kernel<T, NCH, 0>), grid, dim3(256), 0, st, src, (const T*)gamma, (const T*)beta, (T*)y, mean, rstd, rows, d, eps, th, ik, seed);
  else if (mode == 1)
    hipLaunchKernelGGL((ln_fwd_kernel<T, NCH, 1>), grid, dim3(256), 0, st, src, (const T*)gamma, (const T*)beta, (T*)y, mean, rstd, rows, d, eps, th, ik, seed);
  else
    hipLaunchKernelGGL((ln_fwd_kernel<T, NCH, 2>), grid, dim3(256), 0, st, src, (const T*)gamma, (const T*)beta, (T*)y, mean, rstd, rows, d, eps, th, ik, seed);
  IMT_CHECK_LAUNCH();
  return IMT_OK;
}

template <typename T, int NCH>
int ln_bwd_launch(const void* dy, const void* x, const void* gamma, const float* mean, const float* rstd, void* dx,
                  float* dgamma, float* dbeta, int rows, int d, float yp, uint64_t yseed, void* dx_drop, float dxp,
                  uint64_t dxseed, float* partial, hipStream_t st) {
  int wpb = 8;
  if (const char* e = getenv("IMT_LN_WPB")) wpb = atoi(e);
  int nblk = partial ? 512 : 256;
  if (const char* e = getenv("IMT_LN_BLOCKS")) nblk = atoi(e) > 0 ? atoi(e) : nblk;
  int rpw = imt_cdiv(rows, nblk * wpb);
  if (rpw < 1) rpw = 1;
  const int blocks = imt_cdiv(rows, rpw * wpb);
  ImtProfScope prof("layernorm_bwd", 0.0, (dx_drop ? 4.0 : 3.0) * rows * d * sizeof(T), st);
#define IMT_LN_BWD_LAUNCH(W)                                                                                          \
  hipLaunchKernelGGL((ln_bwd_kernel<T, NCH, W>), dim3(blocks), dim3(W * 64), 0, st, (const T*)dy, (const T*)x,        \
                     (const T*)gamma, mean, rstd, (T*)dx, dgamma, dbeta, rows, d, rpw, dropout_thresh(yp),            \
                     yp > 0.f ? 1.f / (1.f - yp) : 1.f, yseed, (T*)dx_drop, dropout_thresh(dxp),                      \
                     dxp > 0.f ? 1.f / (1.f - dxp) : 1.f, dxseed, partial, trace)
  ImtTrace tr("ln_bwd", blocks, st);
  unsigned long long* trace = tr.dev;
  if (wpb == 4) IMT_LN_BWD_LAUNCH(4);
  else if (wpb == 8) IMT_LN_BWD_LAUNCH(8);
  else IMT_LN_BWD_LAUNCH(16);
#undef IMT_LN_BWD_LAUNCH
  IMT_CHECK_LAUNCH();
  return IMT_OK;
}

#define IMT_DISPATCH_NCH(FN, T, d, ...)                                          \
  do {                                                                           \
    const int nch__ = imt_cdiv(d, 256);                                          \
    if (nch__ <= 1) return FN<T, 1>(__VA_ARGS__);                                \
    if (nch__ <= 2) return FN<T, 2>(__VA_ARGS__);                                \
    if (nch__ <= 3) return FN<T, 3>(__VA_ARGS__);                                \
    if (nch__ <= 4) return FN<T, 4>(__VA_ARGS__);                                \
    imt_set_error("layernorm: d=%d > 1024 unsupported", d);                      \
    return IMT_ERR_UNSUPPORTED;                                                  \
  } while (0)

}

template <typename T>
int ln_fwd_dispatch(int mode, const LnSrc<T>& src, const void* gamma, const void* beta, void* y, float* mean, float* rstd, int rows,
                    int d, float eps, float p, uint64_t seed, hipStream_t st) {
  IMT_DISPATCH_NCH(ln_fwd_launch, T, d, mode, src, gamma, beta, y, mean, rstd, rows, d, eps, p, seed, st);
}

extern "C" int imt_layernorm_fwd(int dtype, const void* x, const void* gamma, const void* beta, void* y, float* mean,
                                 float* rstd, int rows, int d, float eps, float dropout_p, uint64_t dropout_seed,
                                 void* stream) {
  IMT_CHECK_ARG(imt_ok_dtype(dtype), "layernorm_fwd: bad dtype");
  IMT_CHECK_ARG(d > 0 && d % 4 == 0, "layernorm_fwd: d must be a positive multiple of 4");
  if (rows <= 0) return IMT_OK;
  IMT_CHECK_ARG(x && gamma && beta && y && mean && rstd, "layernorm_fwd: null pointer");
  hipStream_t st = (hipStream_t)stream;
  return imt_by_dtype(dtype, [&](auto tag) {
    using T = typename decltype(tag)::type;
    LnSrc<T> s{}; s.x = (const T*)x;
    return ln_fwd_dispatch<T>(0, s, gamma, beta, y, mean, rstd, rows, d, eps, dropout_p, dropout_seed, st);
  });
}

extern "C" int imt_add_layernorm_fwd(int dtype, const void* x, const void* resid, const void* gamma, const void* beta, void* sum_out,
                                     void* y, float* mean, float* rstd, int rows, int d, float eps, float dropout_p,
                                     uint64_t dropout_seed, void* stream) {
  IMT_CHECK_ARG(imt_ok_dtype(dtype), "add_layernorm_fwd: bad dtype");
  IMT_CHECK_ARG(d > 0 && d % 4 == 0, "add_layernorm_fwd: d must be a positive multiple of 4");
  if (rows <= 0) return IMT_OK;
  IMT_CHECK_ARG(x && resid && gamma && beta && sum_out && y && mean && rstd, "add_layernorm_fwd: null pointer");
  hipStream_t st = (hipStream_t)stream;
  return imt_by_dtype(dtype, [&](auto tag) {
    using T = typename decltype(tag)::type;
    LnSrc<T> s{}; s.x = (const T*)x; s.resid = (const T*)resid; s.sum_out = (T*)sum_out;
    return ln_fwd_dispatch<T>(1, s, gamma, beta, y, mean, rstd, rows, d, eps, dropout_p, dropout_seed, st);
  });
}

extern "C" int imt_embed_ln_fwd(int dtype, const int64_t* ids, const int64_t* pos_ids, const int64_t* type_ids, const void* word,
                                const void* pos, const void* type, const void* gamma, const void* beta, void* sum_out, void* y,
                                float* mean, float* rstd, int n_tokens, int seq_len, int d, int vocab, int max_pos, int n_types,
                                float eps, float dropout_p, uint64_t dropout_seed, void* stream) {
  IMT_CHECK_ARG(imt_ok_dtype(dtype), "embed_ln_fwd: bad dtype");
  IMT_CHECK_ARG(d > 0 && d % 4 == 0 && seq_len > 0, "embed_ln_fwd: bad dims");
  if (n_tokens <= 0) return IMT_OK;
  IMT_CHECK_ARG(ids && word && pos && type && gamma && beta && sum_out && y && mean && rstd, "embed_ln_fwd: null pointer");
  hipStream_t st = (hipStream_t)stream;
  return imt_by_dtype(dtype, [&](auto tag) {
    using T = typename decltype(tag)::type;
    LnSrc<T> s{}; s.ids = ids; s.pos_ids = pos_ids; s.type_ids = type_ids; s.word = (const T*)word; s.pos = (const T*)pos;
    s.type = (const T*)type; s.sum_out = (T*)sum_out; s.seq_len = seq_len; s.vocab = vocab; s.max_pos = max_pos; s.n_types = n_types;
    return ln_fwd_dispatch<T>(2, s, gamma, beta, y, mean, rstd, n_tokens, d, eps, dropout_p, dropout_seed, st);
  });
}

constexpr int LN_MAX_SITES = 224;
struct LnReduceArgs { int n, d; int64_t g_off[LN_MAX_SITES], b_off[LN_MAX_SITES]; };
__global__ __launch_bounds__(256) void ln_partial_reduce_kernel(const float* __restrict__ partials, float* __restrict__ grads,
                                                                LnReduceArgs a) {
  const int site = blockIdx.y;
  const int c = blockIdx.x * 256 + threadIdx.x;
  if (c >= 2 * a.d || a.g_off[site] < 0) return;
  const float* p = partials + (size_t)site * IMT_LN_PARTIAL_COPIES * 2 * a.d + c;
  float sum = 0.f;
#pragma unroll
  for (int k = 0; k < IMT_LN_PARTIAL_COPIES; ++k) sum += p[(size_t)k * 2 * a.d];
  float* g = grads + (c < a.d ? a.g_off[site] + c : a.b_off[site] + (c - a.d));
  *g += sum;
}

extern "C" int imt_ln_partial_reduce(const float* partials, int n_sites, int d, const int64_t* host_dgamma_off,
                                     const int64_t* host_dbeta_off, float* grads, void* stream) {
  if (n_sites <= 0) return IMT_OK;
  IMT_CHECK_ARG(partials && grads && host_dgamma_off && host_dbeta_off && d > 0, "ln_partial_reduce: bad args");
  IMT_CHECK_ARG(n_sites <= LN_MAX_SITES, "ln_partial_reduce: at most %d sites per call", LN_MAX_SITES);
  LnReduceArgs a;
  a.n = n_sites; a.d = d;
  for (int i = 0; i < n_sites; ++i) { a.g_off[i] = host_dgamma_off[i]; a.b_off[i] = host_dbeta_off[i]; }
  hipStream_t st = (hipStream_t)stream;
  ImtProfScope prof("ln_partial_reduce", 0.0, (double)n_sites * (2.0 * IMT_LN_PARTIAL_COPIES + 2.0) * d * 4.0, st);
  hipLaunchKernelGGL(ln_partial_reduce_kernel, dim3(imt_cdiv(2 * d, 256), n_sites), dim3(256), 0, st, partials, grads, a);
  IMT_CHECK_LAUNCH();
  return IMT_OK;
}

extern "C" int imt_layernorm_bwd(int dtype, const void* dy, const void* x, const void* gamma, const float* mean,
                                 const float* rstd, void* dx, float* dgamma, float* dbeta, int rows, int d,
                                 float y_dropout_p, uint64_t y_dropout_seed, void* dx_drop, float dx_dropout_p,
                                 uint64_t dx_dropout_seed, float* partial_ws, void* stream) {
  IMT_CHECK_ARG(imt_ok_dtype(dtype), "layernorm_bwd: bad dtype");
  IMT_CHECK_ARG(d > 0 && d % 4 == 0, "layernorm_bwd: d must be a positive multiple of 4");
  if (rows <= 0) return IMT_OK;
  IMT_CHECK_ARG(dy && x && gamma && mean && rstd && dx && dgamma && dbeta, "layernorm_bwd: null pointer");
  hipStream_t st = (hipStream_t)stream;
  return imt_by_dtype(dtype, [&](auto tag) -> int {
    using T = typename decltype(tag)::type;
    IMT_DISPATCH_NCH(ln_bwd_launch, T, d, dy, x, gamma, mean, rstd, dx, dgamma, dbeta, rows, d, y_dropout_p,
                     y_dropout_seed, dx_drop, dx_dropout_p, dx_dropout_seed, partial_ws, st);
  });
}

extern "C" int imt_embed_fwd(int dtype, const int64_t* ids, const int64_t* pos_ids, const int64_t* type_ids,
                             const void* word, const void* pos, const void* type, void* out, int n_tokens, int seq_len,
                             int d, int vocab, int max_pos, int n_types, void* stream) {
  IMT_CHECK_ARG(imt_ok_dtype(dtype), "embed_fwd: bad dtype");
  IMT_CHECK_ARG(d > 0 && d % 4 == 0 && seq_len > 0, "embed_fwd: bad dims");
  if (n_tokens <= 0) return IMT_OK;
  IMT_CHECK_ARG(ids && word && pos && type && out, "embed_fwd: null pointer");
  hipStream_t st = (hipStream_t)stream;
  dim3 grid(imt_cdiv(n_tokens, ROWS_PER_BLOCK));
  ImtProfScope prof("embed_fwd", 0.0, 4.0 * n_tokens * d * imt_dtype_bytes(dtype), st);
  return imt_by_dtype(dtype, [&](auto tag) {
    using T = typename decltype(tag)::type;
    hipLaunchKernelGGL(embed_fwd_kernel<T>, grid, dim3(256), 0, st, ids, pos_ids, type_ids, (const T*)word, (const T*)pos,
                       (const T*)type, (T*)out, n_tokens, seq_len, d, vocab, max_pos, n_types);
    IMT_CHECK_LAUNCH();
    return IMT_OK;
  });
}

extern "C" int imt_embed_bwd(int dtype, const int64_t* ids, const int64_t* pos_ids, const int64_t* type_ids,
                             const void* dsum, float* dword, float* dpos, float* dtype_tab, int n_tokens, int seq_len,
                             int d, int64_t pad_id, void* stream) {
  IMT_CHECK_ARG(imt_ok_dtype(dtype), "embed_bwd: bad dtype");
  IMT_CHECK_ARG(d > 0 && seq_len > 0, "embed_bwd: bad dims");
  if (n_tokens <= 0) return IMT_OK;
  IMT_CHECK_ARG(ids && dsum && dword && dpos && dtype_tab, "embed_bwd: null pointer");
  hipStream_t st = (hipStream_t)stream;
  static const int tokb_env = getenv("IMT_EMBED_TOKB") ? atoi(getenv("IMT_EMBED_TOKB")) : 0;
  const int tokb = tokb_env > 0 ? tokb_env : 16;
  const bool posmajor = (pos_ids == nullptr) && (n_tokens % seq_len == 0);
  dim3 grid(posmajor ? seq_len * imt_cdiv(n_tokens / seq_len, tokb) : imt_cdiv(n_tokens, tokb));
  ImtProfScope prof("embed_bwd", 0.0, (double)n_tokens * d * (imt_dtype_bytes(dtype) + 16.0), st);
  return imt_by_dtype(dtype, [&](auto tag) {
    using T = typename decltype(tag)::type;
    hipLaunchKernelGGL((embed_bwd_kernel<T, 4>), grid, dim3(256), 0, st, ids, pos_ids, type_ids, (const T*)dsum, dword, dpos,
                       dtype_tab, n_tokens, seq_len, d, pad_id, tokb);
    IMT_CHECK_LAUNCH();
    return IMT_OK;
  });
}

extern "C" int imt_colsum(int dtype, const void* X, int64_t ldx, int M, int N, float* out, const float* scale_dev,
                          void* stream) {
  IMT_CHECK_ARG(imt_ok_dtype(dtype), "colsum: bad dtype");
  if (M <= 0 || N <= 0) return IMT_OK;
  IMT_CHECK_ARG(X && out && ldx % 4 == 0, "colsum: bad args");
  hipStream_t st = (hipStream_t)stream;
  const int rpb = 64;
  dim3 grid(imt_cdiv(N, 256), imt_cdiv(M, rpb));
  ImtProfScope prof("colsum", 0.0, (double)M * N * imt_dtype_bytes(dtype), st);
  return imt_by_dtype(dtype, [&](auto tag) {
    using T = typename decltype(tag)::type;
    hipLaunchKernelGGL(colsum_kernel<T>, grid, dim3(256), 0, st, (const T*)X, ldx, M, N, out, rpb, scale_dev);
    IMT_CHECK_LAUNCH();
    return IMT_OK;
  });
}

static int gather_scatter(int dtype, const void* x, int64_t ldx, const int32_t* idx, void* out, int64_t ldo, int n_sel,
                          int d, int scatter, void* stream) {
  IMT_CHECK_ARG(imt_ok_dtype(dtype), "gather_rows: bad dtype");
  IMT_CHECK_ARG(d > 0 && d % 4 == 0 && ldx % 4 == 0 && ldo % 4 == 0, "gather_rows: d/ld must be multiples of 4");
  if (n_sel <= 0) return IMT_OK;
  IMT_CHECK_ARG(x && idx && out, "gather_rows: null pointer");
  hipStream_t st = (hipStream_t)stream;
  dim3 grid(imt_cdiv(n_sel, ROWS_PER_BLOCK));
  ImtProfScope prof(scatter ? "scatter_rows" : "gather_rows", 0.0, 2.0 * n_sel * d * imt_dtype_bytes(dtype), st);
  return imt_by_dtype(dtype, [&](auto tag) {
    using T = typename decltype(tag)::type;
    hipLaunchKernelGGL(gather_rows_kernel<T>, grid, dim3(256), 0, st, (const T*)x, ldx, idx, (T*)out, ldo, n_sel, d, scatter);
    IMT_CHECK_LAUNCH();
    return IMT_OK;
  });
}

extern "C" int imt_gather_rows(int dtype, const void* x, int64_t ldx, const int32_t* idx, void* out, int64_t ldo,
                               int n_sel, int d, void* stream) {
  return gather_scatter(dtype, x, ldx, idx, out, ldo, n_sel, d, 0, stream);
}
extern "C" int imt_scatter_rows(int dtype, const void* dout, int64_t ldo, const int32_t* idx, void* dx, int64_t ldx,
                                int n_sel, int d, void* stream) {
  return gather_scatter(dtype, dout, ldo, idx, dx, ldx, n_sel, d, 1, stream);
}

extern "C" int imt_cast_f32_to_bf16(const float* src, void* dst, int64_t n, void* stream) {
  if (n <= 0) return IMT_OK;
  IMT_CHECK_ARG(src && dst, "cast: null pointer");
  int blocks = imt_cdiv(n, 1024);
  if (blocks > 2048) blocks = 2048;
  ImtProfScope prof("cast_f32_to_bf16", 0.0, 6.0 * n, (hipStream_t)stream);
  hipLaunchKernelGGL(cast_bf16_kernel, dim3(blocks), dim3(256), 0, (hipStream_t)stream, src, (bf16_t*)dst, n);
  IMT_CHECK_LAUNCH();
  return IMT_OK;
}

extern "C" int imt_add_rows_dropout(int in_dtype, const void* x, int out_dtype, void* out, const void* add, int64_t rows,
                                    int d, int period, float dropout_p, uint64_t dropout_seed, void* stream) {
  IMT_CHECK_ARG(imt_ok_dtype(in_dtype) && imt_ok_dtype(out_dtype), "add_rows_dropout: bad dtype");
  IMT_CHECK_ARG(d > 0 && d % 4 == 0, "add_rows_dropout: d must be a multiple of 4");
  IMT_CHECK_ARG(!add || period > 0, "add_rows_dropout: period must be positive");
  IMT_CHECK_ARG(dropout_p >= 0.f && dropout_p < 1.f, "add_rows_dropout: dropout_p outside [0, 1)");
  if (rows <= 0) return IMT_OK;
  IMT_CHECK_ARG(x && out, "add_rows_dropout: null pointer");
  hipStream_t st = (hipStream_t)stream;
  dim3 grid(imt_cdiv(rows, ROWS_PER_BLOCK));
  const uint32_t th = dropout_thresh(dropout_p);
  const float ik = dropout_p > 0.f ? 1.f / (1.f - dropout_p) : 1.f;
  ImtProfScope prof("add_rows_dropout", 0.0, (double)rows * d * (imt_dtype_bytes(in_dtype) + imt_dtype_bytes(out_dtype)), st);
  return imt_by_dtype(in_dtype, [&](auto in_tag) {
    return imt_by_dtype(out_dtype, [&](auto out_tag) {
      using TI = typename decltype(in_tag)::type;
      using TO = typename decltype(out_tag)::type;
      hipLaunchKernelGGL((add_rows_dropout_kernel<TI, TO>), grid, dim3(256), 0, st, (const TI*)x, (TO*)out, (const TO*)add, rows, d,
                         period, th, ik, dropout_seed);
      IMT_CHECK_LAUNCH();
      return IMT_OK;
    });
  });
}

extern "C" int imt_gated_mix(int dtype, const void* a, const void* b, const void* gate, void* out, int64_t rows, int d,
                             void* stream) {
  IMT_CHECK_ARG(imt_ok_dtype(dtype), "gated_mix: bad dtype");
  IMT_CHECK_ARG(d > 0 && d % 4 == 0, "gated_mix: d must be a multiple of 4");
  if (rows <= 0) return IMT_OK;
  hipStream_t st = (hipStream_t)stream;
  dim3 grid(imt_cdiv(rows, ROWS_PER_BLOCK));
  return imt_by_dtype(dtype, [&](auto tag) {
    using T = typename decltype(tag)::type;
    hipLaunchKernelGGL(gated_mix_kernel<T>, grid, dim3(256), 0, st, (const T*)a, (const T*)b, (const T*)gate, (T*)out, rows, d);
    IMT_CHECK_LAUNCH();
    return IMT_OK;
  });
}
```

imagetranslate_amd/hip_ops.py:

```python
import contextlib
import ctypes
import os
import math

import torch

from . import _lib as L
from ._lib import IMT_AUX_DGELU, IMT_AUX_GELU_FWD, IMT_AUX_NONE, IMT_AUX_SPLITK_WS, IMT_BF16, IMT_F32, IMT_NN, IMT_NT, IMT_TN


def dt(t: torch.Tensor) -> int:
    if t.dtype == torch.float32:
        return IMT_F32
    if t.dtype == torch.bfloat16:
        return IMT_BF16
    raise TypeError("imagetranslate_amd supports float32 and bfloat16 tensors, got %s" % t.dtype)


def _stream():
    return ctypes.c_void_p(torch.cuda.current_stream().cuda_stream)


def _p(t):
    return None if t is None else ctypes.c_void_p(t.data_ptr())


def _req_cuda(*ts):
    for t in ts:
        if t is not None and not t.is_cuda:
            raise L.ImtError("imagetranslate_amd HIP ops need tensors on the GPU (no CPU fallback)")


def alloc_rows(n_rows, width, dtype, device):
    padded = (width + 7) // 8 * 8
    if padded == width:
        return torch.empty((n_rows, width), device=device, dtype=dtype)
    return torch.zeros((n_rows, padded), device=device, dtype=dtype)[:, :width]


def rows16(t):
    if t.dim() == 2 and t.stride(1) == 1 and (t.stride(0) % 8 == 0 or t.shape[0] <= 1) and t.data_ptr() % 16 == 0:
        return t
    out = alloc_rows(t.shape[0], t.shape[1], t.dtype, t.device)
    out.copy_(t)
    return out


def _rowmajor(t):
    assert t.dim() == 2 and t.stride(1) == 1, "row-major 2-D view expected"
    return t.stride(0)


def gemm(A, B, layout, *, out=None, out_dtype=None, bias=None, resid=None, aux=None, aux_mode=IMT_AUX_NONE,
         accumulate=False, split_k=1, alpha=1.0, dropout_p=0.0, dropout_seed=0, alpha_dev=None, a_colsum=None,
         force_general=False, ln=None, splitk_ws=None, _launch=True):
    _req_cuda(A, B, out, bias, resid, aux)
    if layout == IMT_NT:
        M, K = A.shape; N = B.shape[0]; assert B.shape[1] == K
    elif layout == IMT_NN:
        M, K = A.shape; N = B.shape[1]; assert B.shape[0] == K
    else:
        K, M = A.shape; N = B.shape[1]; assert B.shape[0] == K
    if out is None:
        out = alloc_rows(M, N, out_dtype or A.dtype, A.device)
        assert not accumulate and split_k == 1
    a = L.GemmArgs()
    a.dtype, a.layout = dt(A), layout
    a.M, a.N, a.K = M, N, K
    a.A, a.lda = A.data_ptr(), _rowmajor(A)
    a.B, a.ldb = B.data_ptr(), _rowmajor(B)
    a.C, a.ldc = out.data_ptr(), _rowmajor(out)
    a.c_dtype = dt(out)
    a.accumulate = int(accumulate)
    a.bias = bias.data_ptr() if bias is not None else None
    a.resid, a.ldr = (resid.data_ptr(), _rowmajor(resid)) if resid is not None else (None, 0)
    a.aux, a.ldaux = (aux.data_ptr(), _rowmajor(aux)) if aux is not None else (None, 0)
    a.aux_mode, a.split_k = aux_mode, split_k
    a.alpha, a.dropout_p, a.dropout_seed = alpha, dropout_p, dropout_seed
    a.alpha_dev = alpha_dev.data_ptr() if alpha_dev is not None else None
    a.a_colsum = a_colsum.data_ptr() if a_colsum is not None else None
    a.force_general = int(force_general)
    if splitk_ws is not None:
        _req_cuda(splitk_ws)
        a.splitk_ws, a.splitk_ws_bytes = splitk_ws.data_ptr(), splitk_ws.numel() * splitk_ws.element_size()
    if ln is not None:
        _req_cuda(ln["gamma"], ln["beta"], ln["out"], ln["mean"], ln["rstd"])
        a.ln_gamma, a.ln_beta = ln["gamma"].data_ptr(), ln["beta"].data_ptr()
        a.ln_out, a.ld_ln = ln["out"].data_ptr(), _rowmajor(ln["out"])
        a.ln_mean, a.ln_rstd = ln["mean"].data_ptr(), ln["rstd"].data_ptr()
        a.ln_eps = float(ln.get("eps", 1e-12))
    if not _launch:
        return a
    L.check(L.load().imt_gemm(ctypes.byref(a), _stream()), "imt_gemm")
    return out


_SPLITK_WS = {}


def splitk_workspace(device):
    key = (device.type, device.index)
    ws = _SPLITK_WS.get(key)
    if ws is None:
        ws = torch.empty(int(L.load().imt_gemm_splitk_ws_bytes()) // 4, device=device, dtype=torch.float32)
        _SPLITK_WS[key] = ws
    return ws


def dw_split_k(rows: int, N: int, K: int, rows_per_split: int) -> int:
    return max(1, min(rows // rows_per_split, 512 // max(1, ((N + 127) // 128) * ((K + 127) // 128))))


@contextlib.contextmanager
def grouped_tall_min_tiles(min_tiles):
    prev = L.load().imt_set_gemm_grouped_tall_min_tiles(int(min_tiles))
    try:
        yield
    finally:
        L.load().imt_set_gemm_grouped_tall_min_tiles(prev)


def gemm_grouped_tn(problems, tile_rows=0):
    arr = (L.GemmArgs * len(problems))()
    for i, pr in enumerate(problems):
        arr[i] = gemm(pr["A"], pr["B"], IMT_TN, out=pr["out"], accumulate=True, a_colsum=pr.get("a_colsum"), _launch=False)
    with grouped_tall_min_tiles({128: 1 << 30, 256: 1}[tile_rows]) if tile_rows else contextlib.nullcontext():
        L.check(L.load().imt_gemm_grouped_tn(arr, len(problems), _stream()), "imt_gemm_grouped_tn")


def grouped_tile_order(grids, plain=False):
    n = len(grids)
    total = sum(r * c for r, c in grids)
    rows, cols = (ctypes.c_int * n)(*[g[0] for g in grids]), (ctypes.c_int * n)(*[g[1] for g in grids])
    order = (ctypes.c_int * (3 * total))()
    L.check(L.load().imt_gemm_grouped_tile_order(rows, cols, n, int(plain), order, total), "imt_gemm_grouped_tile_order")
    return [(order[3 * w], order[3 * w + 1], order[3 * w + 2]) for w in range(total)]


def gemm_bias_residual_ln(x, w, bias, resid, gamma, beta, eps=1e-12, dropout_p=0.0, dropout_seed=0, want_pre_ln=True):
    _req_cuda(x, w, bias, resid, gamma, beta)
    M, K = x.shape
    N = w.shape[0]
    assert w.shape[1] == K
    out = torch.empty((M, N), device=x.device, dtype=x.dtype)
    pre = torch.empty((M, N), device=x.device, dtype=x.dtype) if want_pre_ln else None
    mean = torch.empty(M, device=x.device, dtype=torch.float32)
    rstd = torch.empty(M, device=x.device, dtype=torch.float32)
    L.check(L.load().imt_gemm_bias_residual_ln(dt(x), _p(x), _rowmajor(x), _p(w), _rowmajor(w), _p(bias), _p(resid),
                                               _rowmajor(resid) if resid is not None else 0, _p(gamma), _p(beta), _p(pre), _p(out), N,
                                               _p(mean), _p(rstd), M, N, K, eps, dropout_p, dropout_seed, _stream()),
            "imt_gemm_bias_residual_ln")
    return out, pre, mean, rstd


def colsum(X, out, scale_dev=None):
    _req_cuda(X, out)
    L.check(L.load().imt_colsum(dt(X), _p(X), _rowmajor(X), X.shape[0], X.shape[1], _p(out), _p(scale_dev), _stream()),
            "imt_colsum")
    return out


def layernorm_fwd(x, gamma, beta, eps=1e-12, dropout_p=0.0, dropout_seed=0):
    _req_cuda(x, gamma, beta)
    rows, d = x.shape
    y = torch.empty_like(x)
    mean = torch.empty(rows, device=x.device, dtype=torch.float32)
    rstd = torch.empty(rows, device=x.device, dtype=torch.float32)
    L.check(L.load().imt_layernorm_fwd(dt(x), _p(x), _p(gamma), _p(beta), _p(y), _p(mean), _p(rstd), rows, d, eps,
                                       dropout_p, dropout_seed, _stream()), "imt_layernorm_fwd")
    return y, mean, rstd


def add_layernorm_fwd(x, resid, gamma, beta, eps=1e-12, dropout_p=0.0, dropout_seed=0):
    _req_cuda(x, resid, gamma, beta)
    rows, d = x.shape
    y, ssum = torch.empty_like(x), torch.empty_like(x)
    mean = torch.empty(rows, device=x.device, dtype=torch.float32)
    rstd = torch.empty(rows, device=x.device, dtype=torch.float32)
    L.check(L.load().imt_add_layernorm_fwd(dt(x), _p(x), _p(resid), _p(gamma), _p(beta), _p(ssum), _p(y), _p(mean), _p(rstd), rows, d,
                                           eps, dropout_p, dropout_seed, _stream()), "imt_add_layernorm_fwd")
    return y, ssum, mean, rstd


def embed_ln_fwd(ids, pos_ids, type_ids, word, pos, typ, gamma, beta, seq_len, eps=1e-12, dropout_p=0.0, dropout_seed=0):
    _req_cuda(ids, word, gamma, beta)
    n, d = ids.numel(), word.shape[1]
    y = torch.empty((n, d), device=word.device, dtype=word.dtype)
    ssum = torch.empty_like(y)
    mean = torch.empty(n, device=word.device, dtype=torch.float32)
    rstd = torch.empty(n, device=word.device, dtype=torch.float32)
    L.check(L.load().imt_embed_ln_fwd(dt(word), _p(ids), _p(pos_ids), _p(type_ids), _p(word), _p(pos), _p(typ), _p(gamma), _p(beta),
                                      _p(ssum), _p(y), _p(mean), _p(rstd), n, seq_len, d, word.shape[0], pos.shape[0], typ.shape[0], eps,
                                      dropout_p, dropout_seed, _stream()), "imt_embed_ln_fwd")
    return y, ssum, mean, rstd


LN_PARTIAL_COPIES = 32


def layernorm_bwd(dy, x, gamma, mean, rstd, dgamma, dbeta, y_dropout_p=0.0, y_dropout_seed=0, want_dx_drop=False,
                  dx_dropout_p=0.0, dx_dropout_seed=0, partial_ws=None):
    _req_cuda(dy, x, gamma, dgamma, dbeta, partial_ws)
    rows, d = x.shape
    dx = torch.empty_like(x)
    dx_drop = torch.empty_like(x) if want_dx_drop else None
    ws = partial_ws
    if ws is not None:
        assert ws.dtype == torch.float32 and ws.is_contiguous() and ws.numel() == LN_PARTIAL_COPIES * 2 * d
    L.check(L.load().imt_layernorm_bwd(dt(x), _p(dy), _p(x), _p(gamma), _p(mean), _p(rstd), _p(dx), _p(dgamma),
                                       _p(dbeta), rows, d, y_dropout_p, y_dropout_seed, _p(dx_drop), dx_dropout_p,
                                       dx_dropout_seed, _p(ws), _stream()), "imt_layernorm_bwd")
    return (dx, dx_drop) if want_dx_drop else dx


def ln_partial_reduce(partials, grads, dgamma_offsets, dbeta_offsets):
    _req_cuda(partials, grads)
    n, copies, two, d = partials.shape
    assert copies == LN_PARTIAL_COPIES and two == 2 and partials.is_contiguous() and grads.dtype == torch.float32
    g = (ctypes.c_int64 * n)(*[int(v) for v in dgamma_offsets])
    b = (ctypes.c_int64 * n)(*[int(v) for v in dbeta_offsets])
    L.check(L.load().imt_ln_partial_reduce(_p(partials), n, d, g, b, _p(grads), _stream()), "imt_ln_partial_reduce")


def embed_fwd(ids, pos_ids, type_ids, word, pos, typ, seq_len):
    _req_cuda(ids, word)
    n = ids.numel()
    d = word.shape[1]
    out = torch.empty((n, d), device=word.device, dtype=word.dtype)
    L.check(L.load().imt_embed_fwd(dt(word), _p(ids), _p(pos_ids), _p(type_ids), _p(word), _p(pos), _p(typ), _p(out), n,
                                   seq_len, d, word.shape[0], pos.shape[0], typ.shape[0], _stream()), "imt_embed_fwd")
    return out


def embed_bwd(ids, pos_ids, type_ids, dsum, dword, dpos, dtype_tab, seq_len, pad_id):
    _req_cuda(ids, dsum, dword, dpos, dtype_tab)
    n, d = dsum.shape
    L.check(L.load().imt_embed_bwd(dt(dsum), _p(ids), _p(pos_ids), _p(type_ids), _p(dsum), _p(dword), _p(dpos),
                                   _p(dtype_tab), n, seq_len, d, pad_id, _stream()), "imt_embed_bwd")


def _attn_args(q, k, v, B, H, Tq, Tk, head_dim, key_mask, query_mask, mask3d, causal, scale, dropout_p, dropout_seed):
    a = L.AttnArgs()
    a.dtype = dt(q)
    a.B, a.H, a.Tq, a.Tk, a.head_dim = B, H, Tq, Tk, head_dim
    a.Q, a.ldq = q.data_ptr(), _rowmajor(q)
    a.K, a.ldk = k.data_ptr(), _rowmajor(k)
    a.V, a.ldv = v.data_ptr(), _rowmajor(v)
    a.key_mask = key_mask.data_ptr() if key_mask is not None else None
    a.query_mask = query_mask.data_ptr() if query_mask is not None else None
    a.mask3d = mask3d.data_ptr() if mask3d is not None else None
    a.causal = int(causal)
    a.scale = scale if scale is not None else 1.0 / math.sqrt(head_dim)
    a.dropout_p, a.dropout_seed = dropout_p, dropout_seed
    return a


def attention_fwd(q, k, v, B, H, Tq, Tk, head_dim, key_mask=None, query_mask=None, mask3d=None, causal=False,
                  scale=None, dropout_p=0.0, dropout_seed=0, o=None, lse=None):
    _req_cuda(q, k, v, key_mask, query_mask, mask3d, o, lse)
    a = _attn_args(q, k, v, B, H, Tq, Tk, head_dim, key_mask, query_mask, mask3d, causal, scale, dropout_p, dropout_seed)
    if o is None:
        o = torch.empty((B * Tq, H * head_dim), device=q.device, dtype=q.dtype)
    else:
        assert o.dtype == q.dtype and tuple(o.shape) == (B * Tq, H * head_dim), "attention_fwd: o must be [B*Tq, H*head_dim] of q's dtype"
    if lse is None:
        lse = torch.empty((B, H, Tq), device=q.device, dtype=torch.float32)
    else:
        assert lse.dtype == torch.float32 and tuple(lse.shape) == (B, H, Tq) and lse.is_contiguous(), "attention_fwd: lse must be contiguous fp32 [B, H, Tq]"
    a.O, a.ldo, a.lse = o.data_ptr(), _rowmajor(o), lse.data_ptr()
    L.check(L.load().imt_attention_fwd(ctypes.byref(a), _stream()), "imt_attention_fwd")
    return o, lse


def attention_bwd(do, q, k, v, o, lse, B, H, Tq, Tk, head_dim, key_mask=None, query_mask=None, mask3d=None,
                  causal=False, scale=None, dropout_p=0.0, dropout_seed=0, dq=None, dk=None, dv=None):
    _req_cuda(do, q, k, v, o, lse)
    a = _attn_args(q, k, v, B, H, Tq, Tk, head_dim, key_mask, query_mask, mask3d, causal, scale, dropout_p, dropout_seed)
    if dq is None:
        dq = torch.empty((B * Tq, H * head_dim), device=q.device, dtype=q.dtype)
    if dk is None:
        dk = torch.empty((B * Tk, H * head_dim), device=q.device, dtype=q.dtype)
    if dv is None:
        dv = torch.empty((B * Tk, H * head_dim), device=q.device, dtype=q.dtype)
    delta = torch.empty((B, H, Tq), device=q.device, dtype=torch.float32)
    a.O, a.ldo, a.lse = o.data_ptr(), _rowmajor(o), lse.data_ptr()
    a.dO, a.lddo = do.data_ptr(), _rowmajor(do)
    a.dQ, a.lddq = dq.data_ptr(), _rowmajor(dq)
    a.dK, a.lddk = dk.data_ptr(), _rowmajor(dk)
    a.dV, a.lddv = dv.data_ptr(), _rowmajor(dv)
    a.delta = delta.data_ptr()
    L.check(L.load().imt_attention_bwd(ctypes.byref(a), _stream()), "imt_attention_bwd")
    return dq, dk, dv


def attention_bwd_proj(dy, w_o, q, k, v, o, lse, B, H, Tq, Tk, head_dim, key_mask=None, query_mask=None, causal=False,
                       scale=None, dropout_p=0.0, dropout_seed=0, do_out=None):
    _req_cuda(dy, w_o, q, k, v, o, lse, do_out)
    d = H * head_dim
    a = _attn_args(q, k, v, B, H, Tq, Tk, head_dim, key_mask, query_mask, None, causal, scale, dropout_p, dropout_seed)
    dq = torch.empty((B * Tq, d), device=q.device, dtype=q.dtype)
    dk = torch.empty((B * Tk, d), device=q.device, dtype=q.dtype)
    dv = torch.empty((B * Tk, d), device=q.device, dtype=q.dtype)
    delta = torch.empty((B, H, Tq), device=q.device, dtype=torch.float32)
    a.O, a.ldo, a.lse = o.data_ptr(), _rowmajor(o), lse.data_ptr()
    if do_out is not None:
        a.dO, a.lddo = do_out.data_ptr(), _rowmajor(do_out)
    a.dQ, a.lddq = dq.data_ptr(), _rowmajor(dq)
    a.dK, a.lddk = dk.data_ptr(), _rowmajor(dk)
    a.dV, a.lddv = dv.data_ptr(), _rowmajor(dv)
    a.delta = delta.data_ptr()
    L.check(L.load().imt_attention_bwd_proj(ctypes.byref(a), _p(dy), _rowmajor(dy), _p(w_o), _rowmajor(w_o), d, _stream()),
            "imt_attention_bwd_proj")
    return dq, dk, dv


def gather_rows(x, idx):
    _req_cuda(x, idx)
    out = torch.empty((idx.numel(), x.shape[1]), device=x.device, dtype=x.dtype)
    L.check(L.load().imt_gather_rows(dt(x), _p(x), _rowmajor(x), _p(idx), _p(out), out.stride(0) if out.numel() else x.shape[1],
                                     idx.numel(), x.shape[1], _stream()), "imt_gather_rows")
    return out


def scatter_rows(dout, idx, dx):
    _req_cuda(dout, idx, dx)
    L.check(L.load().imt_scatter_rows(dt(dout), _p(dout), _rowmajor(dout) if dout.numel() else dx.shape[1], _p(idx), _p(dx),
                                      _rowmajor(dx), idx.numel(), dx.shape[1], _stream()), "imt_scatter_rows")
    return dx


def log_softmax_fwd(logits):
    _req_cuda(logits)
    N, V = logits.shape
    lp = alloc_rows(N, V, torch.float32, logits.device)
    lse = torch.empty(N, device=logits.device, dtype=torch.float32)
    L.check(L.load().imt_log_softmax_fwd(dt(logits), _p(logits), _rowmajor(logits) if N else V, _p(lp), lp.stride(0) if N else V, _p(lse), N, V,
                                         _stream()), "imt_log_softmax_fwd")
    return lp, lse


_SCORE_WS = {}
SCORE_CHUNK_ROWS = 2048


def score_workspace(device, nbytes):
    key = (device.type, device.index)
    ws = _SCORE_WS.get(key)
    if ws is None or ws.numel() < nbytes:
        ws = torch.empty(int(nbytes), device=device, dtype=torch.uint8)
        _SCORE_WS[key] = ws
    return ws


def score_rows(x, weight, bias, targets, seg_offsets=None, normalize=True):
    _req_cuda(x, weight, bias, targets, seg_offsets)
    N, K = x.shape
    V = weight.shape[0]
    assert weight.shape[1] == K and weight.dtype == x.dtype and (bias is None or bias.dtype == x.dtype)
    assert targets.dtype == torch.int64 and targets.numel() == N
    dev = x.device
    n_seg = 0 if seg_offsets is None else seg_offsets.numel() - 1
    logprob = torch.empty(N, device=dev, dtype=torch.float32)
    lse = torch.empty(N, device=dev, dtype=torch.float32)
    seg = torch.zeros(max(n_seg, 0), device=dev, dtype=torch.float32) if seg_offsets is not None else None
    if N == 0:
        return logprob, lse, seg
    x, weight, targets = rows16(x), rows16(weight), targets.contiguous()
    if bias is not None and (bias.data_ptr() % 16 or bias.stride(0) != 1):
        bias = bias.clone()
    lib = L.load()
    if lib.imt_score_supported(dt(x), V, K):
        if seg_offsets is not None:
            assert seg_offsets.dtype == torch.int64 and n_seg >= 1
            seg_offsets = seg_offsets.contiguous()
        nbytes = int(lib.imt_score_ws_bytes(N, V))
        ws = score_workspace(dev, nbytes)
        a = L.ScoreArgs()
        a.dtype, a.N, a.V, a.K = dt(x), N, V, K
        a.x, a.ldx = x.data_ptr(), _rowmajor(x) if N > 1 else max(K, x.stride(0))
        a.w, a.ldw = weight.data_ptr(), _rowmajor(weight) if V > 1 else max(K, weight.stride(0))
        a.bias = bias.data_ptr() if bias is not None else None
        a.target, a.logprob, a.lse = targets.data_ptr(), logprob.data_ptr(), lse.data_ptr()
        if seg_offsets is not None:
            a.seg_offsets, a.n_seg, a.seg_score = seg_offsets.data_ptr(), n_seg, seg.data_ptr()
        a.normalize = int(bool(normalize))
        a.ws, a.ws_bytes = ws.data_ptr(), nbytes
        L.check(lib.imt_score_rows(ctypes.byref(a), _stream()), "imt_score_rows")
        return logprob, lse, seg
    valid = (targets >= 0) & (targets < V)
    safe = torch.where(valid, targets, torch.zeros_like(targets))
    for r0 in range(0, N, SCORE_CHUNK_ROWS):
        r1 = min(N, r0 + SCORE_CHUNK_ROWS)
        logits = gemm(x[r0:r1], weight, IMT_NT, bias=bias, out_dtype=torch.float32)
        lp, l = log_softmax_fwd(logits)
        logprob[r0:r1] = lp.gather(1, safe[r0:r1].unsqueeze(1)).squeeze(1)
        lse[r0:r1] = l
    logprob.masked_fill_(~valid, 0.0)
    if seg_offsets is not None:
        off = seg_offsets.clamp(0, N)
        csum = torch.cat([logprob.new_zeros(1, dtype=torch.float64), logprob.double().cumsum(0)])
        ccnt = torch.cat([off.new_zeros(1), valid.long().cumsum(0)])
        tot = (csum[off[1:]] - csum[off[:-1]])
        cnt = (ccnt[off[1:]] - ccnt[off[:-1]])
        if normalize:
            tot = torch.where(cnt > 0, tot / cnt.clamp(min=1).double(), tot)
        seg = tot.float()
    return logprob, lse, seg


KNN_MAX_K = 8


def _knn_operand(t):
    tile = 128 // t.element_size()
    K = t.shape[1]
    if K % tile:
        out = torch.zeros((t.shape[0], (K + tile - 1) // tile * tile), device=t.device, dtype=t.dtype)
        out[:, :K] = t
        return out
    return rows16(t)


def _knn_max_rows(t):
    ld = max(t.shape[1], t.stride(0))
    return ((1 << 31) - 1) // (ld * t.element_size()) - 256


def knn_rows(x, y, k, *, splits=0, _key_chunk=None, _query_chunk=None):
    _req_cuda(x, y)
    N, K = x.shape
    M = y.shape[0]
    if y.shape[1] != K or y.dtype != x.dtype:
        raise ValueError("knn_rows: queries %s %s against keys %s %s" % (tuple(x.shape), x.dtype, tuple(y.shape), y.dtype))
    if not 1 <= k <= KNN_MAX_K:
        raise ValueError("knn_rows: k = %d outside 1..%d" % (k, KNN_MAX_K))
    dev = x.device
    if N == 0 or M == 0:
        return (torch.full((N, k), float("-inf"), device=dev, dtype=torch.float32),
                torch.full((N, k), -1, device=dev, dtype=torch.int64))
    x, y = _knn_operand(x), _knn_operand(y)
    Kp = x.shape[1]
    lib = L.load()
    if not lib.imt_knn_supported(dt(x), Kp):
        raise L.ImtError("knn_rows: (dtype %s, K %d) is not taken by imt_knn_rows" % (x.dtype, Kp))
    q_rows = max(1, min(_knn_max_rows(x), int(_query_chunk) if _query_chunk else N))
    k_rows = max(1, min(_knn_max_rows(y), int(_key_chunk) if _key_chunk else M))
    val = torch.empty((N, k), device=dev, dtype=torch.float32)
    idx = torch.empty((N, k), device=dev, dtype=torch.int64)
    n_chunks = (M + k_rows - 1) // k_rows
    for r0 in range(0, N, q_rows):
        r1 = min(N, r0 + q_rows)
        xs = x[r0:r1]
        cv = torch.empty((r1 - r0, n_chunks * k), device=dev, dtype=torch.float32)
        ci = torch.empty((r1 - r0, n_chunks * k), device=dev, dtype=torch.int32)
        for c, c0 in enumerate(range(0, M, k_rows)):
            ys = y[c0:min(M, c0 + k_rows)]
            v = torch.empty((r1 - r0, k), device=dev, dtype=torch.float32)
            i = torch.empty((r1 - r0, k), device=dev, dtype=torch.int32)
            nbytes = int(lib.imt_knn_ws_bytes(xs.shape[0], ys.shape[0], k, splits))
            ws = score_workspace(dev, nbytes)
            a = L.KnnArgs()
            a.dtype, a.N, a.M, a.K, a.k = dt(x), xs.shape[0], ys.shape[0], Kp, k
            a.x, a.ldx = xs.data_ptr(), max(Kp, xs.stride(0))
            a.y, a.ldy = ys.data_ptr(), max(Kp, ys.stride(0))
            a.index_base, a.splits = c0, int(splits)
            a.val, a.idx = v.data_ptr(), i.data_ptr()
            a.ws, a.ws_bytes = ws.data_ptr(), nbytes
            L.check(lib.imt_knn_rows(ctypes.byref(a), _stream()), "imt_knn_rows")
            cv[:, c * k:(c + 1) * k] = v
            ci[:, c * k:(c + 1) * k] = i
        if n_chunks == 1:
            val[r0:r1], idx[r0:r1] = cv, ci.long()
        else:
            sv, order = torch.sort(cv, dim=1, descending=True, stable=True)
            val[r0:r1] = sv[:, :k]
            idx[r0:r1] = ci.gather(1, order[:, :k]).long()
    return val, idx


ALIGN_MAX_LEN = 512


def _align_operand(t):
    step = 128 // t.element_size()
    epv = 16 // t.element_size()
    B, rows, d = t.shape
    if d % step:
        out = torch.zeros((B, rows, (d + step - 1) // step * step), device=t.device, dtype=t.dtype)
        out[:, :, :d] = t
        return out
    ok = t.stride(2) == 1 and t.data_ptr() % 16 == 0
    ok = ok and (rows == 1 or (t.stride(1) >= d and t.stride(1) % epv == 0))
    ok = ok and (B == 1 or (t.stride(0) % epv == 0 and t.stride(0) >= (rows - 1) * (t.stride(1) if rows > 1 else 0) + d))
    return t if ok else t.contiguous()


def align_pairs(x, y, x_range, y_range, min_sim=float("-inf")):
    if x.dim() != 3 or y.dim() != 3 or x.shape[0] != y.shape[0] or x.shape[2] != y.shape[2] or x.dtype != y.dtype:
        raise ValueError("align_pairs: x %s %s against y %s %s" % (tuple(x.shape), x.dtype, tuple(y.shape), y.dtype))
    B, S, d = x.shape
    T = y.shape[1]
    if x.dtype not in (torch.float32, torch.bfloat16):
        raise ValueError("align_pairs: float32 or bfloat16 states, got %s" % x.dtype)
    for name, rng in (("x_range", x_range), ("y_range", y_range)):
        if tuple(rng.shape) != (B, 2) or rng.dtype.is_floating_point or rng.dtype == torch.bool:
            raise ValueError("align_pairs: %s must be integer [%d, 2], got %s %s" % (name, B, tuple(rng.shape), rng.dtype))
    _req_cuda(x, y, x_range, y_range)
    dev = x.device
    link = torch.full((B, S), -1, device=dev, dtype=torch.int32)
    fwd_idx = torch.full((B, S), -1, device=dev, dtype=torch.int32)
    fwd_val = torch.full((B, S), float("-inf"), device=dev, dtype=torch.float32)
    bwd_idx = torch.full((B, T), -1, device=dev, dtype=torch.int32)
    bwd_val = torch.full((B, T), float("-inf"), device=dev, dtype=torch.float32)
    if B > 0:
        x, y = _align_operand(x), _align_operand(y)
        dp = x.shape[2]
        lib = L.load()
        if not lib.imt_align_supported(dt(x), dp):
            raise L.ImtError("align_pairs: (dtype %s, d %d) is not taken by imt_align_pairs" % (x.dtype, dp))
        lim = torch.iinfo(torch.int32)
        xr = x_range.clamp(lim.min, lim.max).to(torch.int32).contiguous()
        yr = y_range.clamp(lim.min, lim.max).to(torch.int32).contiguous()
        a = L.AlignArgs()
        a.dtype, a.B, a.S, a.T, a.d = dt(x), B, S, T, dp
        a.x, a.ldx = x.data_ptr(), x.stride(1) if S > 1 else dp
        a.bsx = x.stride(0) if B > 1 else (S - 1) * a.ldx + dp
        a.y, a.ldy = y.data_ptr(), y.stride(1) if T > 1 else dp
        a.bsy = y.stride(0) if B > 1 else (T - 1) * a.ldy + dp
        a.xr, a.yr = xr.data_ptr(), yr.data_ptr()
        a.min_sim = float(min_sim)
        a.link, a.fwd_idx, a.fwd_val = link.data_ptr(), fwd_idx.data_ptr(), fwd_val.data_ptr()
        a.bwd_idx, a.bwd_val = bwd_idx.data_ptr(), bwd_val.data_ptr()
        L.check(lib.imt_align_pairs(ctypes.byref(a), _stream()), "imt_align_pairs")
    return link.long(), fwd_idx.long(), fwd_val, bwd_idx.long(), bwd_val


def conv_out_size(size, kernel, stride, pad):
    return (size + 2 * pad - kernel) // stride + 1


def conv2d_nhwc(x, w, *, stride=1, pad=0, scale=None, shift=None, residual=None, relu=False, out=None):
# ... 443 lines not shown
```

include/imt_hip.h:

```cpp
#ifndef IMT_HIP_H
#define IMT_HIP_H
#include <stdint.h>
#ifdef __cplusplus
extern "C" {
#endif

#define IMT_OK 0
#define IMT_ERR_BAD_ARG (-1)
#define IMT_ERR_UNSUPPORTED (-2)
#define IMT_ERR_LAUNCH (-3)

#define IMT_F32 0
#define IMT_BF16 1

int imt_version(void);
const char* imt_last_error(void);

int imt_abi_sizeof(const char* struct_name);

typedef struct imt_prof_row {
  char kind[48];
  int64_t launches;
  double total_ms;
  double flops;
  double bytes;
} imt_prof_row;
int imt_debug_spin(int blocks, int threads, int lds_bytes, int64_t cycles, void* stream);
int imt_prof_enable(int on);
int imt_prof_report(imt_prof_row* rows, int max_kinds);

#define IMT_NT 0
#define IMT_NN 1
#define IMT_TN 2
#define IMT_AUX_NONE 0
#define IMT_AUX_GELU_FWD 1
#define IMT_AUX_DGELU 2
#define IMT_AUX_SPLITK_WS 3

typedef struct imt_gemm_args {
  int32_t dtype, layout;
  int32_t M, N, K;
  const void* A; int64_t lda;
  const void* B; int64_t ldb;
  void* C; int64_t ldc;
  int32_t c_dtype;
  int32_t accumulate;
  const void* bias;
  const void* resid; int64_t ldr;
  void* aux; int64_t ldaux;
  int32_t aux_mode;
  int32_t split_k;
  float alpha;
  float dropout_p;
  uint64_t dropout_seed;
  const float* alpha_dev;
  float* a_colsum;
  int32_t force_general;
  const void* ln_gamma; const void* ln_beta;
  void* ln_out; int64_t ld_ln;
  float* ln_mean; float* ln_rstd;
  float ln_eps;
  void* splitk_ws; int64_t splitk_ws_bytes;
} imt_gemm_args;
int64_t imt_gemm_splitk_ws_bytes(void);
int imt_gemm(const imt_gemm_args* a, void* stream);
int imt_gemm_grouped_tn(const imt_gemm_args* list, int count, void* stream);
int imt_gemm_grouped_tile_order(const int* tile_rows, const int* tile_cols, int count, int plain, int* order, int order_tiles);

int imt_gemm_bias_residual_ln_supported(int dtype, int N, int K);
int imt_gemm_bias_residual_ln(int dtype, const void* x, int64_t ldx, const void* w, int64_t ldw, const void* bias,
                              const void* resid, int64_t ldr, const void* gamma, const void* beta, void* pre_ln, void* out,
                              int64_t ldo, float* mean, float* rstd, int M, int N, int K, float eps, float dropout_p,
                              uint64_t dropout_seed, void* stream);

int imt_colsum(int dtype, const void* X, int64_t ldx, int M, int N, float* out, const float* scale_dev, void* stream);

int imt_layernorm_fwd(int dtype, const void* x, const void* gamma, const void* beta, void* y, float* mean,
                      float* rstd, int rows, int d, float eps, float dropout_p, uint64_t dropout_seed,
                      void* stream);
int imt_add_layernorm_fwd(int dtype, const void* x, const void* resid, const void* gamma, const void* beta, void* sum_out,
                          void* y, float* mean, float* rstd, int rows, int d, float eps, float dropout_p,
                          uint64_t dropout_seed, void* stream);
int imt_layernorm_bwd(int dtype, const void* dy, const void* x, const void* gamma, const float* mean,
                      const float* rstd, void* dx, float* dgamma, float* dbeta, int rows, int d,
                      float y_dropout_p, uint64_t y_dropout_seed, void* dx_drop, float dx_dropout_p,
                      uint64_t dx_dropout_seed, float* partial_ws, void* stream);
#define IMT_LN_PARTIAL_COPIES 32
#define IMT_LN_BWD_WS_FLOATS(d) (IMT_LN_PARTIAL_COPIES * 2 * (int64_t)(d))
int imt_ln_partial_reduce(const float* partials, int n_sites, int d, const int64_t* host_dgamma_off,
                          const int64_t* host_dbeta_off, float* grads, void* stream);

int imt_embed_fwd(int dtype, const int64_t* ids, const int64_t* pos_ids, const int64_t* type_ids,
                  const void* word, const void* pos, const void* type, void* out, int n_tokens, int seq_len,
                  int d, int vocab, int max_pos, int n_types, void* stream);
int imt_embed_bwd(int dtype, const int64_t* ids, const int64_t* pos_ids, const int64_t* type_ids,
                  const void* dsum, float* dword, float* dpos, float* dtype_tab, int n_tokens, int seq_len, int d,
                  int64_t pad_id, void* stream);
int imt_embed_ln_fwd(int dtype, const int64_t* ids, const int64_t* pos_ids, const int64_t* type_ids, const void* word,
                     const void* pos, const void* type, const void* gamma, const void* beta, void* sum_out, void* y,
                     float* mean, float* rstd, int n_tokens, int seq_len, int d, int vocab, int max_pos, int n_types, float eps,
                     float dropout_p, uint64_t dropout_seed, void* stream);

typedef struct imt_attn_args {
  int32_t dtype;
  int32_t B, H, Tq, Tk, head_dim;
  const void* Q; int64_t ldq;
  const void* K; int64_t ldk;
  const void* V; int64_t ldv;
  void* O; int64_t ldo;
  float* lse;
  const uint8_t* key_mask;
  const uint8_t* query_mask;
  const uint8_t* mask3d;
  int32_t causal;
  float scale;
  float dropout_p;
  uint64_t dropout_seed;
  const void* dO; int64_t lddo;
  void* dQ; int64_t lddq;
  void* dK; int64_t lddk;
  void* dV; int64_t lddv;
  float* delta;
} imt_attn_args;
int imt_attention_fwd(const imt_attn_args* a, void* stream);
int imt_attention_bwd(const imt_attn_args* a, void* stream);
int imt_attention_bwd_proj_supported(int dtype, int head_dim, int H, int Tq, int Tk, int d_model, int has_mask3d);
int imt_attention_bwd_proj(const imt_attn_args* a, const void* dy, int64_t lddy, const void* w_o, int64_t ldw, int d_model,
                           void* stream);

int imt_gather_rows(int dtype, const void* x, int64_t ldx, const int32_t* idx, void* out, int64_t ldo, int n_sel,
                    int d, void* stream);
int imt_scatter_rows(int dtype, const void* dout, int64_t ldo, const int32_t* idx, void* dx, int64_t ldx, int n_sel,
                     int d, void* stream);

int imt_log_softmax_fwd(int dtype, const void* logits, int64_t ld, float* lp, int64_t ldlp, float* lse, int N, int V,
                        void* stream);
int imt_log_softmax_bwd(const float* dlp, int64_t lddlp, const float* lp, int64_t ldlp, int out_dtype, void* dlogits,
                        int64_t ld, int N, int V, void* stream);
int imt_smoothed_nll_fwd(const float* lp, int64_t ldlp, const int64_t* target, float* loss, int N, int V,
                         float epsilon, int64_t ignore_index, void* stream);
int imt_smoothed_nll_bwd(const float* dloss, const int64_t* target, float* dlp, int64_t lddlp, int N, int V,
                         float epsilon, int64_t ignore_index, void* stream);
int imt_xent_fused_fwd_bwd(int dtype, void* logits, int64_t ld, const int64_t* target, float* loss_rows, int N,
                           int V, float epsilon, int64_t ignore_index, float grad_scale, void* stream);

typedef struct imt_score_args {
  int32_t dtype;
  int32_t N, V, K;
  const void* x; int64_t ldx;
  const void* w; int64_t ldw;
  const void* bias;
  const int64_t* target;
  float* logprob;
  float* lse;
  const int64_t* seg_offsets;
  int32_t n_seg, normalize;
  float* seg_score;
  void* ws; int64_t ws_bytes;
} imt_score_args;
int64_t imt_score_ws_bytes(int N, int V);
int imt_score_supported(int dtype, int V, int K);
int imt_score_rows(const imt_score_args* a, void* stream);
#define IMT_KNN_MAX_K 8
#define IMT_KNN_MAX_SPLITS 256
typedef struct imt_knn_args {
  int32_t dtype;
  int32_t N, M, K, k;
  const void* x; int64_t ldx;
  const void* y; int64_t ldy;
  int32_t index_base;
  int32_t splits;
  float* val;
  int32_t* idx;
  void* ws; int64_t ws_bytes;
} imt_knn_args;
int64_t imt_knn_ws_bytes(int N, int M, int k, int splits);
int imt_knn_supported(int dtype, int K);
int imt_knn_rows(const imt_knn_args* a, void* stream);
#define IMT_ALIGN_MAX_LEN 512
typedef struct imt_align_args {
  int32_t dtype;
  int32_t B, S, T, d;
  const void* x; int64_t ldx, bsx;
  const void* y; int64_t ldy, bsy;
  const int32_t* xr;
  const int32_t* yr;
  float min_sim; int32_t reserved;
  int32_t* link;
  int32_t* fwd_idx; float* fwd_val;
  int32_t* bwd_idx; float* bwd_val;
} imt_align_args;
int imt_align_supported(int dtype, int d);
int imt_align_pairs(const imt_align_args* a, void* stream);
int imt_scaled_sum(const float* x, int n, float scale, float* out, void* stream);

typedef struct imt_conv_args {
  int32_t dtype;
  int32_t B, H, W, Cin, Cout, KH, KW;
  int32_t stride, pad_h, pad_w;
  int32_t relu;
  const void* x; const void* w; void* y;
  const float* scale; const float* shift;
  const void* residual;
} imt_conv_args;
int imt_conv2d_supported(int dtype, int Cin, int KH, int KW, int stride);
int imt_conv2d(const imt_conv_args* a, void* stream);
int imt_maxpool2d_3x3s2(int dtype, const void* x, void* y, int B, int H, int W, int C, void* stream);
int imt_image_nhwc(int dtype, const uint8_t* img, void* out, int B, int H, int W, const float* host_mean, const float* host_std,
                   void* stream);

int imt_comm_unique_id_bytes(void);
int imt_comm_get_unique_id(void* host_id_out);
int imt_comm_init(const void* host_unique_id, int world_size, int rank, void** comm_out);
int imt_comm_allreduce(void* comm, void* buf, int64_t count, int dtype, void* stream);
int imt_comm_broadcast(void* comm, void* buf, int64_t count, int dtype, int root, void* stream);
int imt_comm_destroy(void* comm);

int imt_set_gemm_share_cus(int share_cus);
int imt_set_gemm_grouped_tall_min_tiles(int min_tiles);

#define IMT_SUMSQ_WS_FLOATS 1024
int imt_sumsq(const float* g, int64_t n, float* out, float* partial_ws, void* stream);
int imt_clip_adam(float* p, float* g, float* m, float* v, void* p_bf16, int64_t n, const float* sumsq,
                  float max_norm, float grad_scale, float lr, float beta1, float beta2, float eps, int64_t step,
                  int zero_grad, void* stream);
int imt_clip_scale(float* g, int64_t n, const float* sumsq, float max_norm, float grad_scale, void* stream);
int imt_cast_f32_to_bf16(const float* src, void* dst, int64_t n, void* stream);
int imt_gated_mix(int dtype, const void* a, const void* b, const void* gate, void* out, int64_t rows, int d,
                  void* stream);
int imt_add_rows_dropout(int in_dtype, const void* x, int out_dtype, void* out, const void* add, int64_t rows, int d,
                         int period, float dropout_p, uint64_t dropout_seed, void* stream);

#define IMT_OBJ_FEAT_DIM 1024
#define IMT_OBJ_LABELS 91
#define IMT_GATED_MIX_BWD_PARTS 64
int imt_obj_rows(int feat_dtype, int dtype, const int64_t* labels, const void* feats, const float* boxes, const void* emb,
                 const void* w, void* x_out, void* w_out, int64_t R, int d, int Kp, int* status, void* stream);
int imt_relu_dropout(int dtype, void* y, int64_t rows, int d, float dropout_p, uint64_t dropout_seed, void* stream);
int imt_relu_dropout_bwd(int dtype, const void* dy, const void* y, void* dz, int64_t rows, int d, float dropout_p,
                         uint64_t dropout_seed, void* stream);
int imt_obj_fold_w(const float* dw_pad, float* grad, int d, int Kp, void* stream);
int imt_obj_embed_grad(int dtype, const int64_t* labels, const void* dx, int64_t ldx, float* grad, int64_t R, int d,
                       void* stream);
int imt_gated_mix_bwd(int dtype, const void* dy, const void* a, const void* b, const void* gate, void* da, void* db,
                      float* dgate, float* partial_ws, int64_t rows, int d, void* stream);

#define IMT_POOL_MAX_S 4096
#define IMT_POOL_MAX_D 1024
#define IMT_POOL_LDS_BYTES 65536
#define IMT_CONTRASTIVE_MAX_N 4096
int imt_attn_pool_plan(int dtype, int S, int d);
int imt_attn_pool_fwd(int dtype, const void* x, const void* w, const void* b, const uint8_t* mask, float* u, float* probs,
                      float* norm, int64_t rows, int S, int d, void* stream);
int imt_attn_pool_bwd(int dtype, const void* x, const void* w, const uint8_t* mask, const float* u, const float* probs,
                      const float* norm, const float* du, const float* du_scale, void* dx, float* dw, float* db, float* ws,
                      int64_t rows, int S, int d, void* stream);
int imt_contrastive(const float* img, const float* txt, float* loss, float* d_img, float* d_txt, float* ws, int B, int N, int d,
                    void* stream);

#define IMT_L2_DIST_PARTS 256
int imt_sent_pool_fwd(int dtype, const void* x, const void* w, const void* b, const uint8_t* mask, void* v, float* probs,
                      int64_t rows, int S, int d, float dropout_p, uint64_t dropout_seed, void* stream);
int imt_sent_pool_bwd(int dtype, const void* x, const void* w, const uint8_t* mask, const float* probs, const void* dv, void* dx,
                      float* dw, float* db, float* ws, int64_t rows, int S, int d, float dropout_p, uint64_t dropout_seed,
                      void* stream);
int imt_l2_dist(int dtype, const void* pred, const void* target, float* loss, void* dpred, float* ws, int B, int64_t n,
                void* stream);

int imt_sensim_loss(const float* scat, const float* tcat, float* loss, float* d_scat, float* d_tcat, float* ws, int B, int Ns,
                    int Nt, int d, void* stream);
int imt_pair_dot(const float* a, const float* b, float* out, int64_t rows, int d, void* stream);
int imt_pair_dot_bwd(const float* a, const float* b, const float* g, float* da, float* db, int64_t rows, int d, void* stream);

#define IMT_PROPOSAL_MAX_D 1024
int64_t imt_proposal_attn_ws_bytes(int64_t rows, int rows_per_group, int P, int d);
int imt_proposal_attn_fwd(int dtype, const void* x, const void* table, const int64_t* prop, const float* gate, const float* gamma,
                          const float* beta, void* y, float* scores, float* stats, int64_t rows, int rows_per_group, int P, int d,
                          int64_t vocab, int64_t pad_idx, float eps, void* stream);
int imt_proposal_attn_bwd(int dtype, const void* dy, const void* x, const void* table, const int64_t* prop, const float* gate,
                          const float* gamma, const float* scores, const float* stats, void* dx, float* dtable, float* dgate,
                          float* dgamma, float* dbeta, void* ws, int64_t ws_bytes, int64_t rows, int rows_per_group, int P, int d,
                          int64_t vocab, int64_t pad_idx, void* stream);


typedef struct imt_attn_block {
  int64_t qkv_w, qkv_b;
  int64_t o_w, o_b;
  int64_t ln_g, ln_b;
} imt_attn_block;

typedef struct imt_layer_desc {
  imt_attn_block self_attn;
  imt_attn_block cross_attn;
  int64_t ff1_w, ff1_b;
  int64_t ff2_w, ff2_b;
  int64_t ln2_g, ln2_b;
  int64_t cross_kv_w, cross_kv_b;
} imt_layer_desc;

typedef struct imt_stack_desc {
  int32_t dtype;
  int32_t d, heads, ff, vocab, max_pos, n_types, n_layers;
  int32_t is_decoder;
  int32_t reserved;
  int64_t pad_id;
  float ln_eps, hidden_dropout, attn_dropout;
  float reserved_f;
  int64_t emb_word, emb_pos, emb_type, emb_ln_g, emb_ln_b;
  const imt_layer_desc* layers;
  const void* params;
  float* grads;
} imt_stack_desc;

typedef struct imt_stack_io {
  int32_t B, T;
  int32_t Tk;
  int32_t training;
  const int64_t* ids;
  const int64_t* type_ids;
  const int64_t* pos_ids;
  const uint8_t* key_mask;
  const uint8_t* query_mask;
  const uint8_t* mask3d;
  int32_t causal;
  int32_t reserved;
  const void* enc_states;
  const uint8_t* enc_mask;
  void* out;
  uint64_t dropout_seed;
  const void* d_out;
  void* d_enc_states;
  const void* const* wait_events;
  int32_t n_wait_events;
  int32_t reserved2;
} imt_stack_io;

int64_t imt_stack_workspace_bytes(const imt_stack_desc* m, int B, int T, int Tk);
int imt_stack_forward(const imt_stack_desc* m, const imt_stack_io* io, void* ws, int64_t ws_bytes, void* stream);
int imt_stack_backward(const imt_stack_desc* m, const imt_stack_io* io, void* ws, int64_t ws_bytes, int layer_lo,
                       int layer_hi, void* stream);

typedef struct imt_attn_decode_args {
  int32_t dtype;
  int32_t R, H, head_dim;
  int32_t n_keys;
  int32_t rep;
  const void* Q; int64_t ldq;
  const void* K; const void* V;
  int64_t ld_row, ld_pos;
  const int32_t* slots; int64_t ld_slots;
  const uint8_t* key_mask; int64_t ld_mask;
  void* O; int64_t ldo;
  float scale;
  int32_t reserved;
} imt_attn_decode_args;
int imt_attention_decode(const imt_attn_decode_args* a, void* stream);

typedef struct imt_decode_io {
  int32_t R;
  int32_t rep;
  int32_t pos;
  int32_t Tk;
  int32_t t_max, r_max;
  const int64_t* ids;
  const int64_t* type_ids;
  const int64_t* pos_ids;
  const int32_t* slots;
  const uint8_t* enc_mask;
  void* self_cache;
  const void* cross_kv;
  void* out;
} imt_decode_io;
int64_t imt_decode_workspace_bytes(const imt_stack_desc* m, int r_max);
int64_t imt_decode_self_cache_bytes(const imt_stack_desc* m, int r_max, int t_max);
int64_t imt_decode_cross_bytes(const imt_stack_desc* m, int B, int Tk);
int imt_decode_begin(const imt_stack_desc* m, const void* enc_states, int B, int Tk, void* cross_kv, void* stream);
int imt_decode_step(const imt_stack_desc* m, const imt_decode_io* io, void* ws, int64_t ws_bytes, void* stream);
int imt_decode_check(const imt_stack_desc* m, int r_max, const void* ws, void* stream);

typedef struct imt_beam_args {
  int32_t B, beam, rep, V;
  int32_t step, t_max;
  const float* logits; int64_t ld;
  const float* scores_in;
  const float* sizes_in;
  const uint8_t* eos_in;
  const int64_t* max_lens;
  const int64_t* hist_in;
  const int32_t* slots_in;
  float len_penalty_ratio;
  int32_t reserved;
  int64_t pad_idx, eos;
  float* cand_scores; int32_t* cand_idx;
  float* scores_out; float* sizes_out; uint8_t* eos_out;
  int64_t* hist_out;
  int32_t* slots_out;
  int32_t* parent_out;
  int64_t* tokens_out;
  int32_t* eos_count;
} imt_beam_args;
// ... 68 lines not shown
```

Measured before the change: 1.176 million tokens/s.

## Fuse embedding LayerNorm backward with embedding scatter and fold workspace zeroing into forward

Adds a fused embed_ln_bwd kernel that computes the embedding LayerNorm backward and directly scatters gradients into word, position and type tables. It keeps position and type sums in registers to cut atomics and skips writing and rereading the intermediate d_emb. The LN partial-workspace memsets are removed from backward and done by the spare threads of the embedding LN forward kernel. The workspace grows by two sites for type-table partials. This adds complexity and more atomics on the word table.

Result: no change. 1.186 million tokens/s, median of 6 (+0.8%).

```diff
diff --git a/imagetranslate_amd/_lib.py b/imagetranslate_amd/_lib.py
--- a/imagetranslate_amd/_lib.py
+++ b/imagetranslate_amd/_lib.py
@@ -233,6 +233,8 @@
                                   c_uint64, _P, _P]),
     "imt_embed_fwd": (c_int, [c_int, _P, _P, _P, _P, _P, _P, _P, c_int, c_int, c_int, c_int, c_int, c_int, _P]),
     "imt_embed_bwd": (c_int, [c_int, _P, _P, _P, _P, _P, _P, _P, c_int, c_int, c_int, c_int64, _P]),
+    "imt_embed_ln_bwd": (c_int, [c_int, _P, _P, _P, _P, _P, c_float, c_uint64, _P, _P, _P, c_int64, c_int, c_int, c_int, _P, _P, _P, _P, _P,
+                                 _P, _P, _P, _P]),
     "imt_attention_fwd": (c_int, [POINTER(AttnArgs), _P]),
     "imt_attention_bwd": (c_int, [POINTER(AttnArgs), _P]),
     "imt_attention_bwd_proj_supported": (c_int, [c_int, c_int, c_int, c_int, c_int, c_int, c_int]),
diff --git a/imagetranslate_amd/csrc/common.hpp b/imagetranslate_amd/csrc/common.hpp
--- a/imagetranslate_amd/csrc/common.hpp
+++ b/imagetranslate_amd/csrc/common.hpp
@@ -48,6 +48,11 @@
 }
 
 bool imt_gemm_grouped_tall(const imt_gemm_args* list, int count);
+
+int imt_embed_ln_fwd_zero(int dtype, const int64_t* ids, const int64_t* pos_ids, const int64_t* type_ids, const void* word,
+                          const void* pos, const void* type, const void* gamma, const void* beta, void* sum_out, void* y,
+                          float* mean, float* rstd, int n_tokens, int seq_len, int d, int vocab, int max_pos, int n_types,
+                          float eps, float dropout_p, uint64_t dropout_seed, float* zero_ptr, int64_t zero_floats, void* stream);
 
 bool imt_prof_enabled();
 const char* imt_prof_intern(const char* kind, int M, int N, int K);
diff --git a/imagetranslate_amd/csrc/model.hip b/imagetranslate_amd/csrc/model.hip
--- a/imagetranslate_amd/csrc/model.hip
+++ b/imagetranslate_amd/csrc/model.hip
@@ -115,7 +115,7 @@
   w.use_scratch(0);
   w.d_emb = c.take(N * d * es);
   w.delta = (float*)c.take((int64_t)B * m->heads * T * 4);
-  w.ln_partial = (float*)c.take((int64_t)(3 * m->n_layers + 1) * IMT_LN_BWD_WS_FLOATS(d) * 4);
+  w.ln_partial = (float*)c.take((int64_t)(3 * m->n_layers + 3) * IMT_LN_BWD_WS_FLOATS(d) * 4);
   w.splitk_bytes = ((N + 127) / 128) * ((d + 127) / 128) <= 128 ? imt_gemm_splitk_ws_bytes() : 0;
   w.splitk = w.splitk_bytes ? c.take(w.splitk_bytes) : nullptr;
   w.bytes = c.off;
@@ -368,9 +368,10 @@
       (void)hipStreamWaitEvent(c.st, (hipEvent_t)const_cast<void*>(io->wait_events[k]), 0);
   };
   wait_site(0);
-  RC(imt_embed_ln_fwd(c.dtype, io->ids, io->pos_ids, io->type_ids, c.P(m->emb_word), c.P(m->emb_pos), c.P(m->emb_type), c.P(m->emb_ln_g),
-                      c.P(m->emb_ln_b), w.emb_sum, x0, w.emb_mean, w.emb_rstd, N, T, d, m->vocab, m->max_pos, m->n_types, m->ln_eps,
-                      training ? m->hidden_dropout : 0.f, site_seed(seed, 1000, 0), c.st));
+  RC(imt_embed_ln_fwd_zero(c.dtype, io->ids, io->pos_ids, io->type_ids, c.P(m->emb_word), c.P(m->emb_pos), c.P(m->emb_type), c.P(m->emb_ln_g),
+                           c.P(m->emb_ln_b), w.emb_sum, x0, w.emb_mean, w.emb_rstd, N, T, d, m->vocab, m->max_pos, m->n_types, m->ln_eps,
+                           training ? m->hidden_dropout : 0.f, site_seed(seed, 1000, 0), w.ln_partial,
+                           (int64_t)(3 * m->n_layers + 3) * IMT_LN_BWD_WS_FLOATS(d), c.st));
   const void* x = x0;
   const MaskSet self_ms{io->key_mask, io->query_mask, io->mask3d, io->causal};
   const MaskSet cross_ms{io->enc_mask, nullptr, nullptr, 0};
@@ -412,9 +413,6 @@
   const void* dy = (layer_hi == m->n_layers) ? io->d_out : w.d_run;
   const bool batched = cross_kv_batched(m);
   DeferredDW dw;
-  const int64_t lnf = IMT_LN_BWD_WS_FLOATS(d);
-  if (layer_hi > layer_lo) (void)hipMemsetAsync(w.ln_site(3 * layer_lo, d), 0, (size_t)(3 * (layer_hi - layer_lo)) * lnf * 4, c.st);
-  if (layer_lo == 0) (void)hipMemsetAsync(w.ln_site(3 * m->n_layers, d), 0, (size_t)lnf * 4, c.st);
   static const bool side_env = !(getenv("IMT_DW_SIDE_STREAM") && atoi(getenv("IMT_DW_SIDE_STREAM")) == 0);
   const bool whole = layer_lo == 0 && layer_hi == m->n_layers && m->n_layers >= 2;
   const bool side = side_env && !imt_prof_enabled() && whole && g_side.init();
@@ -464,18 +462,36 @@
   }
   if (layer_lo == 0) {
     const void* dy0 = (m->n_layers == 0) ? io->d_out : dy;
-    RC(imt_layernorm_bwd(c.dtype, dy0, w.emb_sum, c.P(m->emb_ln_g), w.emb_mean, w.emb_rstd, w.d_emb, c.G(m->emb_ln_g), c.G(m->emb_ln_b), N, d,
-                         training ? m->hidden_dropout : 0.f, site_seed(seed, 1000, 0), nullptr, 0.f, 0, w.ln_site(3 * m->n_layers, d), c.st));
-    RC(imt_embed_bwd(c.dtype, io->ids, io->pos_ids, io->type_ids, w.d_emb, c.G(m->emb_word), c.G(m->emb_pos), c.G(m->emb_type), N, T, d,
-                     m->pad_id, c.st));
+    const float emb_p = training ? m->hidden_dropout : 0.f;
+    float* emb_partial = w.ln_site(3 * m->n_layers, d);
+    const char* sw = getenv("IMT_EMBED_LN_BWD");
+    int rc = IMT_ERR_UNSUPPORTED;
+    if (!(sw && atoi(sw) == 0))
+      rc = imt_embed_ln_bwd(c.dtype, dy0, w.emb_sum, c.P(m->emb_ln_g), w.emb_mean, w.emb_rstd, emb_p, site_seed(seed, 1000, 0), io->ids,
+                            io->pos_ids, io->type_ids, m->pad_id, N, T, d, c.G(m->emb_word), c.G(m->emb_pos), c.G(m->emb_type),
+                            c.G(m->emb_ln_g), c.G(m->emb_ln_b), emb_partial, w.ln_site(3 * m->n_layers + 1, d), nullptr, c.st);
+    if (rc == IMT_ERR_UNSUPPORTED) {
+      RC(imt_layernorm_bwd(c.dtype, dy0, w.emb_sum, c.P(m->emb_ln_g), w.emb_mean, w.emb_rstd, w.d_emb, c.G(m->emb_ln_g), c.G(m->emb_ln_b), N, d,
+                           emb_p, site_seed(seed, 1000, 0), nullptr, 0.f, 0, emb_partial, c.st));
+      RC(imt_embed_bwd(c.dtype, io->ids, io->pos_ids, io->type_ids, w.d_emb, c.G(m->emb_word), c.G(m->emb_pos), c.G(m->emb_type), N, T, d,
+                       m->pad_id, c.st));
+    } else {
+      RC(rc);
+    }
   }
   {
-    static int64_t g_off[3 * MAX_LAYERS + 1], b_off[3 * MAX_LAYERS + 1];
+    static int64_t g_off[3 * MAX_LAYERS + 3], b_off[3 * MAX_LAYERS + 3];
     const int first = 3 * layer_lo, emb = 3 * m->n_layers;
-    const int last = (layer_lo == 0) ? emb + 1 : 3 * layer_hi;
+    const int last = (layer_lo == 0) ? emb + 3 : 3 * layer_hi;
     for (int sidx = first; sidx < last; ++sidx) {
       g_off[sidx - first] = -1; b_off[sidx - first] = -1;
       if (sidx == emb) { g_off[sidx - first] = m->emb_ln_g; b_off[sidx - first] = m->emb_ln_b; continue; }
+      if (sidx > emb) {
+        const int t0 = 2 * (sidx - emb - 1);
+        if (t0 < m->n_types) g_off[sidx - first] = m->emb_type + (int64_t)t0 * d;
+        if (t0 + 1 < m->n_types) b_off[sidx - first] = m->emb_type + (int64_t)(t0 + 1) * d;
+        continue;
+      }
       const int l = sidx / 3, slot = sidx % 3;
       if (l >= layer_hi) continue;
       const imt_layer_desc& p = m->layers[l];
diff --git a/imagetranslate_amd/csrc/rowops.hip b/imagetranslate_amd/csrc/rowops.hip
--- a/imagetranslate_amd/csrc/rowops.hip
+++ b/imagetranslate_amd/csrc/rowops.hip
@@ -17,10 +17,15 @@
                                                      const T* __restrict__ beta, T* __restrict__ y,
                                                      float* __restrict__ mean_out, float* __restrict__ rstd_out,
                                                      int rows, int d, float eps, uint32_t thresh, float inv_keep,
-                                                     uint64_t seed) {
+                                                     uint64_t seed, f32x4* __restrict__ zero_ptr, int64_t zero_vec4) {
   const int lane = threadIdx.x & 63;
   const int row = imt_xcd_block(blockIdx.x, gridDim.x) * ROWS_PER_BLOCK + (threadIdx.x >> 6);
-  if (row >= rows) return;
+  auto zero_share = [&]() {
+    if (SRC == 2 && zero_ptr)
+      for (int64_t i = (int64_t)blockIdx.x * 256 + threadIdx.x; i < zero_vec4; i += (int64_t)gridDim.x * 256)
+        zero_ptr[i] = f32x4{0.f, 0.f, 0.f, 0.f};
+  };
+  if (row >= rows) { zero_share(); return; }
   f32x4 v[NCH], gv[NCH], bv[NCH];
   float s = 0.f;
   if (SRC == 2) {
@@ -93,6 +98,7 @@
       Vec4<T>::store(yr + c, o);
     }
   }
+  zero_share();
 }
 
 template <typename T, int NCH, int WPB>
@@ -283,6 +289,201 @@
   }
 }
 
+template <typename T> struct EmbLnBwdArgs {
+  const T* dy; const T* x; const T* gamma; const float* mean; const float* rstd; T* dx;
+  const int64_t* ids; const int64_t* pos_ids; const int64_t* type_ids;
+  float* dword; float* dpos; float* dtype_tab; float* dgamma; float* dbeta; float* partial; float* type_partial;
+  int64_t pad_id;
+  uint64_t y_seed; uint32_t y_thresh; float y_inv_keep;
+  int rows, d, seq_len, rows_per_wave, posmajor;
+};
+
+IMT_DEVICE void lds_barrier() { asm volatile("s_waitcnt lgkmcnt(0)\n\ts_barrier" ::: "memory"); }
+IMT_DEVICE int64_t uniform64(int64_t v) {
+  const uint32_t lo = __builtin_amdgcn_readfirstlane((uint32_t)v), hi = __builtin_amdgcn_readfirstlane((uint32_t)((uint64_t)v >> 32));
+  return (int64_t)(((uint64_t)hi << 32) | lo);
+}
+
+template <typename T, int NCH, int NT_REG>
+__global__ __launch_bounds__(512, ((NCH <= 2 && sizeof(T) == 2) ? 4 : 1)) void embed_ln_bwd_kernel(EmbLnBwdArgs<T> a,
+                                                                                                   unsigned long long* trace) {
+  constexpr int WPB = 8, NTH = WPB * 64, W = NCH * 256, CPT = (W + NTH - 1) / NTH;
+  __shared__ float lay[WPB][W];
+  __shared__ int64_t m_word[WPB], m_pos[WPB], m_type[WPB];
+  __shared__ int m_live[WPB];
+  IMT_STAMP(trace, 0);
+  const int lane = threadIdx.x & 63, w = __builtin_amdgcn_readfirstlane(threadIdx.x >> 6);
+  const int d = a.d, rows = a.rows;
+  f32x4 g[NCH], ag[NCH], ab[NCH];
+#pragma unroll
+  for (int i = 0; i < NCH; ++i) {
+    const int c = lane * 4 + i * 256;
+    g[i] = Vec4<T>::load(a.gamma + min(c, d - 4));
+    ag[i] = f32x4{0.f, 0.f, 0.f, 0.f};
+    ab[i] = f32x4{0.f, 0.f, 0.f, 0.f};
+  }
+  int64_t first;
+  int stride, count, p_own = 0;
+  if (a.posmajor) {
+    p_own = blockIdx.x % a.seq_len;
+    const int s0 = ((blockIdx.x / a.seq_len) * WPB + w) * a.rows_per_wave;
+    first = (int64_t)s0 * a.seq_len + p_own; stride = a.seq_len; count = min(a.rows_per_wave, rows / a.seq_len - s0);
+  } else {
+    const int rb = (imt_xcd_block(blockIdx.x, gridDim.x) * WPB + w) * a.rows_per_wave;
+    first = rb; stride = 1; count = min(a.rows_per_wave, rows - rb);
+  }
+  const int64_t* pp = a.pos_ids ? a.pos_ids : a.ids;
+  const int64_t* tp = a.type_ids ? a.type_ids : a.ids;
+  float pacc[CPT], tacc[NT_REG][CPT];
+#pragma unroll
+  for (int q = 0; q < CPT; ++q) {
+    pacc[q] = 0.f;
+#pragma unroll
+    for (int t = 0; t < NT_REG; ++t) tacc[t][q] = 0.f;
+  }
+  constexpr int RB = 2;
+  for (int r0 = 0; r0 < a.rows_per_wave; r0 += RB) {
+    f32x4 xb[RB][NCH], db[RB][NCH];
+    float mub[RB], rsb[RB];
+    int64_t wb[RB], pb[RB], tb[RB];
+#pragma unroll
+    for (int k = 0; k < RB; ++k) {
+      const int64_t row = min(first + (int64_t)min(r0 + k, max(count - 1, 0)) * stride, (int64_t)rows - 1);
+      mub[k] = a.mean[row];
+      rsb[k] = a.rstd[row];
+      wb[k] = a.ids[row];
+      pb[k] = pp[row];
+      tb[k] = tp[row];
+#pragma unroll
+      for (int i = 0; i < NCH; ++i) {
+        const int c = min(lane * 4 + i * 256, d - 4);
+        xb[k][i] = Vec4<T>::load(a.x + row * d + c);
+        db[k][i] = Vec4<T>::load(a.dy + row * d + c);
+      }
+    }
+    if (r0 == 0) IMT_STAMP(trace, 1);
+    asm volatile("" : "+v"(db[RB - 1][NCH - 1][3]));
+#pragma unroll
+    for (int k = 0; k < RB; ++k) {
+      if (r0 + k >= a.rows_per_wave) break;
+      const bool live = r0 + k < count;
+      const int64_t row = first + (int64_t)(r0 + k) * stride;
+      if (live) {
+        const float mu = mub[k], rs = rsb[k];
+        float s1 = 0.f, s2 = 0.f;
+#pragma unroll
+        for (int i = 0; i < NCH; ++i) {
+          const int c = lane * 4 + i * 256;
+          if (c < d) {
+            if (a.y_thresh) dropout_apply4(db[k][i], a.y_seed, (uint64_t)row * d + c, a.y_thresh, a.y_inv_keep);
+#pragma unroll
+            for (int e = 0; e < 4; ++e) {
+              xb[k][i][e] = (xb[k][i][e] - mu) * rs;
+              const float dg = db[k][i][e] * g[i][e];
+              s1 += dg;
+              s2 += dg * xb[k][i][e];
+              ag[i][e] += db[k][i][e] * xb[k][i][e];
+              ab[i][e] += db[k][i][e];
+            }
+          }
+        }
+        const float c1 = wave_sum(s1) / (float)d, c2 = wave_sum(s2) / (float)d;
+        if (r0 == 0 && k == 0) IMT_STAMP(trace, 2);
+#pragma unroll
+        for (int i = 0; i < NCH; ++i) {
+          const int c = lane * 4 + i * 256;
+          if (c < d) {
+            f32x4 o;
+#pragma unroll
+            for (int e = 0; e < 4; ++e) o[e] = rs * (db[k][i][e] * g[i][e] - c1 - xb[k][i][e] * c2);
+            if (a.dx) Vec4<T>::store(a.dx + row * d + c, o);
+#pragma unroll
+            for (int e = 0; e < 4; ++e) o[e] = to_f32<T>(from_f32<T>(o[e]));
+            *reinterpret_cast<f32x4*>(&lay[w][c]) = o;
+          }
+        }
+      }
+      if (lane == 0) {
+        m_live[w] = live ? 1 : 0;
+        m_word[w] = wb[k];
+        m_pos[w] = a.pos_ids ? pb[k] : (row % a.seq_len);
+        m_type[w] = a.type_ids ? tb[k] : 0;
+      }
+      lds_barrier();
+#pragma unroll
+      for (int w2 = 0; w2 < WPB; ++w2) {
+        if (!__builtin_amdgcn_readfirstlane(m_live[w2])) continue;
+        const int64_t wi = uniform64(m_word[w2]), pi = uniform64(m_pos[w2]), ti = uniform64(m_type[w2]);
+        float* wrow = a.dword + wi * d;
+        float* prow = a.dpos + pi * d;
+        float* trow = a.dtype_tab + ti * d;
+#pragma unroll
+        for (int q = 0; q < CPT; ++q) {
+          const int c = threadIdx.x + q * NTH;
+          if (c < d) {
+            const float v = lay[w2][c];
+            if (wi != a.pad_id) atomicAdd(wrow + c, v);
+            if (a.posmajor) pacc[q] += v;
+            else atomicAdd(prow + c, v);
+            bool hit = false;
+#pragma unroll
+            for (int t = 0; t < NT_REG; ++t)
+              if (ti == t) { tacc[t][q] += v; hit = true; }
+            if (!hit) atomicAdd(trow + c, v);
+          }
+        }
+      }
+      if (r0 == 0 && k == 0) IMT_STAMP(trace, 3);
+      lds_barrier();
+    }
+  }
+  IMT_STAMP(trace, 4);
+  float sg[CPT], sb[CPT];
+#pragma unroll
+  for (int pass = 0; pass < 2; ++pass) {
+#pragma unroll
+    for (int i = 0; i < NCH; ++i) {
+      const int c = lane * 4 + i * 256;
+      if (c < d) *reinterpret_cast<f32x4*>(&lay[w][c]) = pass == 0 ? ag[i] : ab[i];
+    }
+    lds_barrier();
+#pragma unroll
+    for (int q = 0; q < CPT; ++q) {
+      const int c = threadIdx.x + q * NTH;
+      float s = 0.f;
+      if (c < d) {
+#pragma unroll
+        for (int k = 0; k < WPB; ++k) s += lay[k][c];
+      }
+      if (pass == 0) sg[q] = s; else sb[q] = s;
+    }
+    if (pass == 0) lds_barrier();
+  }
+  IMT_STAMP(trace, 5);
+#pragma unroll
+  for (int q = 0; q < CPT; ++q) {
+    const int c = threadIdx.x + q * NTH;
+    if (c >= d) continue;
+    if (a.partial) {
+      float* pc = a.partial + (size_t)(blockIdx.x & (IMT_LN_PARTIAL_COPIES - 1)) * 2 * d;
+      atomicAdd(pc + c, sg[q]);
+      atomicAdd(pc + d + c, sb[q]);
+    } else {
+      atomicAdd(a.dgamma + c, sg[q]);
+      atomicAdd(a.dbeta + c, sb[q]);
+    }
+    if (a.posmajor) atomicAdd(a.dpos + (int64_t)p_own * d + c, pacc[q]);
+#pragma unroll
+    for (int t = 0; t < NT_REG; ++t) {
+      if (tacc[t][q] == 0.f) continue;
+      float* dst = a.type_partial ? a.type_partial + ((size_t)(t >> 1) * IMT_LN_PARTIAL_COPIES + (blockIdx.x & (IMT_LN_PARTIAL_COPIES - 1))) * 2 * d + (size_t)(t & 1) * d
+                                  : a.dtype_tab + (int64_t)t * d;
+      atomicAdd(dst + c, tacc[t][q]);
+    }
+  }
+  IMT_STAMP(trace, 6);
+}
+
 template <typename T>
 __global__ __launch_bounds__(256) void colsum_kernel(const T* __restrict__ X, int64_t ldx, int M, int N,
                                                      float* __restrict__ out, int rows_per_block,
@@ -369,18 +570,20 @@
 
 template <typename T, int NCH>
 int ln_fwd_launch(int mode, const LnSrc<T>& src, const void* gamma, const void* beta, void* y, float* mean, float* rstd, int rows,
-                  int d, float eps, float p, uint64_t seed, hipStream_t st) {
+                  int d, float eps, float p, uint64_t seed, float* zero_ptr, int64_t zero_floats, hipStream_t st) {
   static const char* const kinds[3] = {"layernorm_fwd", "add_layernorm_fwd", "embed_ln_fwd"};
   ImtProfScope prof(kinds[mode], 0.0, (mode == 0 ? 2.0 : mode == 1 ? 4.0 : 5.0) * rows * d * sizeof(T), st);
   const dim3 grid(imt_cdiv(rows, ROWS_PER_BLOCK));
   const uint32_t th = dropout_thresh(p);
   const float ik = p > 0.f ? 1.f / (1.f - p) : 1.f;
+  f32x4* const z4 = reinterpret_cast<f32x4*>(zero_ptr);
+  const int64_t nz4 = zero_floats / 4;
   if (mode == 0)
-    hipLaunchKernelGGL((ln_fwd_kernel<T, NCH, 0>), grid, dim3(256), 0, st, src, (const T*)gamma, (const T*)beta, (T*)y, mean, rstd, rows, d, eps, th, ik, seed);
+    hipLaunchKernelGGL((ln_fwd_kernel<T, NCH, 0>), grid, dim3(256), 0, st, src, (const T*)gamma, (const T*)beta, (T*)y, mean, rstd, rows, d, eps, th, ik, seed, z4, nz4);
   else if (mode == 1)
-    hipLaunchKernelGGL((ln_fwd_kernel<T, NCH, 1>), grid, dim3(256), 0, st, src, (const T*)gamma, (const T*)beta, (T*)y, mean, rstd, rows, d, eps, th, ik, seed);
+    hipLaunchKernelGGL((ln_fwd_kernel<T, NCH, 1>), grid, dim3(256), 0, st, src, (const T*)gamma, (const T*)beta, (T*)y, mean, rstd, rows, d, eps, th, ik, seed, z4, nz4);
   else
-    hipLaunchKernelGGL((ln_fwd_kernel<T, NCH, 2>), grid, dim3(256), 0, st, src, (const T*)gamma, (const T*)beta, (T*)y, mean, rstd, rows, d, eps, th, ik, seed);
+    hipLaunchKernelGGL((ln_fwd_kernel<T, NCH, 2>), grid, dim3(256), 0, st, src, (const T*)gamma, (const T*)beta, (T*)y, mean, rstd, rows, d, eps, th, ik, seed, z4, nz4);
   IMT_CHECK_LAUNCH();
   return IMT_OK;
 }
@@ -412,7 +615,27 @@
   return IMT_OK;
 }
 
-#define IMT_DISPATCH_NCH(FN, T, d, ...)                                          \
+template <typename T, int NCH>
+int embed_ln_bwd_launch(EmbLnBwdArgs<T> a, hipStream_t st) {
+  constexpr int WPB = 8, NBLK = 512;
+  int blocks;
+  if (a.posmajor) {
+    const int nsent = a.rows / a.seq_len;
+    const int sent_groups = NBLK / a.seq_len > 0 ? NBLK / a.seq_len : 1;
+    a.rows_per_wave = imt_cdiv(imt_cdiv(nsent, sent_groups), WPB);
+    blocks = a.seq_len * imt_cdiv(nsent, a.rows_per_wave * WPB);
+  } else {
+    a.rows_per_wave = imt_cdiv(a.rows, NBLK * WPB);
+    blocks = imt_cdiv(a.rows, a.rows_per_wave * WPB);
+  }
+  ImtProfScope prof("embed_bwd", 0.0, (double)a.rows * a.d * (2.0 * sizeof(T) + 4.0), st);
+  ImtTrace tr("embed_ln_bwd", blocks, st);
+  hipLaunchKernelGGL((embed_ln_bwd_kernel<T, NCH, 4>), dim3(blocks), dim3(WPB * 64), 0, st, a, tr.dev);
+  IMT_CHECK_LAUNCH();
+  return IMT_OK;
+}
+
+#define IMT_DISPATCH_NCH(FN, T, d, ...)                                        \
   do {                                                                           \
     const int nch__ = imt_cdiv(d, 256);                                          \
     if (nch__ <= 1) return FN<T, 1>(__VA_ARGS__);                                \
@@ -427,8 +650,8 @@
 
 template <typename T>
 int ln_fwd_dispatch(int mode, const LnSrc<T>& src, const void* gamma, const void* beta, void* y, float* mean, float* rstd, int rows,
-                    int d, float eps, float p, uint64_t seed, hipStream_t st) {
-  IMT_DISPATCH_NCH(ln_fwd_launch, T, d, mode, src, gamma, beta, y, mean, rstd, rows, d, eps, p, seed, st);
+                    int d, float eps, float p, uint64_t seed, hipStream_t st, float* zero_ptr = nullptr, int64_t zero_floats = 0) {
+  IMT_DISPATCH_NCH(ln_fwd_launch, T, d, mode, src, gamma, beta, y, mean, rstd, rows, d, eps, p, seed, zero_ptr, zero_floats, st);
 }
 
 extern "C" int imt_layernorm_fwd(int dtype, const void* x, const void* gamma, const void* beta, void* y, float* mean,
@@ -461,21 +684,31 @@
   });
 }
 
+int imt_embed_ln_fwd_zero(int dtype, const int64_t* ids, const int64_t* pos_ids, const int64_t* type_ids, const void* word,
+                          const void* pos, const void* type, const void* gamma, const void* beta, void* sum_out, void* y,
+                          float* mean, float* rstd, int n_tokens, int seq_len, int d, int vocab, int max_pos, int n_types,
+                          float eps, float dropout_p, uint64_t dropout_seed, float* zero_ptr, int64_t zero_floats, void* stream) {
+  IMT_CHECK_ARG(imt_ok_dtype(dtype), "embed_ln_fwd: bad dtype");
+  IMT_CHECK_ARG(d > 0 && d % 4 == 0 && seq_len > 0, "embed_ln_fwd: bad dims");
+  IMT_CHECK_ARG(!zero_ptr || (zero_floats >= 0 && zero_floats % 4 == 0 && ((uintptr_t)zero_ptr & 15) == 0), "embed_ln_fwd: bad zero range");
+  IMT_CHECK_ARG(!zero_ptr || n_tokens > 0, "embed_ln_fwd: nothing launched to zero the range");
+  if (n_tokens <= 0) return IMT_OK;
+  IMT_CHECK_ARG(ids && word && pos && type && gamma && beta && sum_out && y && mean && rstd, "embed_ln_fwd: null pointer");
+  hipStream_t st = (hipStream_t)stream;
+  return imt_by_dtype(dtype, [&](auto tag) {
+    using T = typename decltype(tag)::type;
+    LnSrc<T> s{}; s.ids = ids; s.pos_ids = pos_ids; s.type_ids = type_ids; s.word = (const T*)word; s.pos = (const T*)pos;
+    s.type = (const T*)type; s.sum_out = (T*)sum_out; s.seq_len = seq_len; s.vocab = vocab; s.max_pos = max_pos; s.n_types = n_types;
+    return ln_fwd_dispatch<T>(2, s, gamma, beta, y, mean, rstd, n_tokens, d, eps, dropout_p, dropout_seed, st, zero_ptr, zero_floats);
+  });
+}
+
 extern "C" int imt_embed_ln_fwd(int dtype, const int64_t* ids, const int64_t* pos_ids, const int64_t* type_ids, const void* word,
                                 const void* pos, const void* type, const void* gamma, const void* beta, void* sum_out, void* y,
                                 float* mean, float* rstd, int n_tokens, int seq_len, int d, int vocab, int max_pos, int n_types,
                                 float eps, float dropout_p, uint64_t dropout_seed, void* stream) {
-  IMT_CHECK_ARG(imt_ok_dtype(dtype), "embed_ln_fwd: bad dtype");
-  IMT_CHECK_ARG(d > 0 && d % 4 == 0 && seq_len > 0, "embed_ln_fwd: bad dims");
-  if (n_tokens <= 0) return IMT_OK;
-  IMT_CHECK_ARG(ids && word && pos && type && gamma && beta && sum_out && y && mean && rstd, "embed_ln_fwd: null pointer");
-  hipStream_t st = (hipStream_t)stream;
-  return imt_by_dtype(dtype, [&](auto tag) {
-    using T = typename decltype(tag)::type;
-    LnSrc<T> s{}; s.ids = ids; s.pos_ids = pos_ids; s.type_ids = type_ids; s.word = (const T*)word; s.pos = (const T*)pos;
-    s.type = (const T*)type; s.sum_out = (T*)sum_out; s.seq_len = seq_len; s.vocab = vocab; s.max_pos = max_pos; s.n_types = n_types;
-    return ln_fwd_dispatch<T>(2, s, gamma, beta, y, mean, rstd, n_tokens, d, eps, dropout_p, dropout_seed, st);
-  });
+  return imt_embed_ln_fwd_zero(dtype, ids, pos_ids, type_ids, word, pos, type, gamma, beta, sum_out, y, mean, rstd, n_tokens, seq_len, d,
+                               vocab, max_pos, n_types, eps, dropout_p, dropout_seed, nullptr, 0, stream);
 }
 
 constexpr int LN_MAX_SITES = 224;
@@ -485,6 +718,7 @@
   const int site = blockIdx.y;
   const int c = blockIdx.x * 256 + threadIdx.x;
   if (c >= 2 * a.d || a.g_off[site] < 0) return;
+  if (c >= a.d && a.b_off[site] < 0) return;
   const float* p = partials + (size_t)site * IMT_LN_PARTIAL_COPIES * 2 * a.d + c;
   float sum = 0.f;
 #pragma unroll
@@ -565,7 +799,31 @@
   });
 }
 
-extern "C" int imt_colsum(int dtype, const void* X, int64_t ldx, int M, int N, float* out, const float* scale_dev,
+extern "C" int imt_embed_ln_bwd(int dtype, const void* dy, const void* emb_sum, const void* gamma, const float* mean,
+                                const float* rstd, float y_dropout_p, uint64_t y_dropout_seed, const int64_t* ids,
+                                const int64_t* pos_ids, const int64_t* type_ids, int64_t pad_id, int n_tokens, int seq_len, int d,
+                                float* dword, float* dpos, float* dtype_tab, float* dgamma, float* dbeta, float* partial_ws,
+                                float* type_partial_ws, void* dx, void* stream) {
+  IMT_CHECK_ARG(imt_ok_dtype(dtype), "embed_ln_bwd: bad dtype");
+  IMT_CHECK_ARG(d > 0 && d % 4 == 0 && seq_len > 0, "embed_ln_bwd: d must be a positive multiple of 4, seq_len positive");
+  if (n_tokens <= 0) return IMT_OK;
+  IMT_CHECK_ARG(dy && emb_sum && gamma && mean && rstd && ids && dword && dpos && dtype_tab && dgamma && dbeta, "embed_ln_bwd: null pointer");
+  hipStream_t st = (hipStream_t)stream;
+  return imt_by_dtype(dtype, [&](auto tag) -> int {
+    using T = typename decltype(tag)::type;
+    EmbLnBwdArgs<T> a{};
+    a.dy = (const T*)dy; a.x = (const T*)emb_sum; a.gamma = (const T*)gamma; a.mean = mean; a.rstd = rstd; a.dx = (T*)dx;
+    a.ids = ids; a.pos_ids = pos_ids; a.type_ids = type_ids;
+    a.dword = dword; a.dpos = dpos; a.dtype_tab = dtype_tab; a.dgamma = dgamma; a.dbeta = dbeta; a.partial = partial_ws; a.type_partial = type_partial_ws;
+    a.pad_id = pad_id;
+    a.y_seed = y_dropout_seed; a.y_thresh = dropout_thresh(y_dropout_p); a.y_inv_keep = y_dropout_p > 0.f ? 1.f / (1.f - y_dropout_p) : 1.f;
+    a.rows = n_tokens; a.d = d; a.seq_len = seq_len;
+    a.posmajor = (pos_ids == nullptr) && (n_tokens % seq_len == 0);
+    IMT_DISPATCH_NCH(embed_ln_bwd_launch, T, d, a, st);
+  });
+}
+
+extern "C" int imt_colsum(int dtype,const void* X, int64_t ldx, int M, int N, float* out, const float* scale_dev,
                           void* stream) {
   IMT_CHECK_ARG(imt_ok_dtype(dtype), "colsum: bad dtype");
   if (M <= 0 || N <= 0) return IMT_OK;
diff --git a/imagetranslate_amd/hip_ops.py b/imagetranslate_amd/hip_ops.py
--- a/imagetranslate_amd/hip_ops.py
+++ b/imagetranslate_amd/hip_ops.py
@@ -237,6 +237,21 @@
     n, d = dsum.shape
     L.check(L.load().imt_embed_bwd(dt(dsum), _p(ids), _p(pos_ids), _p(type_ids), _p(dsum), _p(dword), _p(dpos),
                                    _p(dtype_tab), n, seq_len, d, pad_id, _stream()), "imt_embed_bwd")
+
+
+def embed_ln_bwd(dy, emb_sum, gamma, mean, rstd, ids, pos_ids, type_ids, dword, dpos, dtype_tab, dgamma, dbeta, seq_len, pad_id,
+                 y_dropout_p=0.0, y_dropout_seed=0, partial_ws=None, type_partial_ws=None, want_dx=False):
+    _req_cuda(dy, emb_sum, gamma, ids, dword, dpos, dtype_tab, dgamma, dbeta, partial_ws, type_partial_ws)
+    n, d = emb_sum.shape
+    dx = torch.empty_like(emb_sum) if want_dx else None
+    if partial_ws is not None:
+        assert partial_ws.dtype == torch.float32 and partial_ws.is_contiguous() and partial_ws.numel() == LN_PARTIAL_COPIES * 2 * d
+    if type_partial_ws is not None:
+        assert type_partial_ws.dtype == torch.float32 and type_partial_ws.is_contiguous() and type_partial_ws.numel() == 2 * LN_PARTIAL_COPIES * 2 * d
+    L.check(L.load().imt_embed_ln_bwd(dt(emb_sum), _p(dy), _p(emb_sum), _p(gamma), _p(mean), _p(rstd), y_dropout_p, y_dropout_seed,
+                                      _p(ids), _p(pos_ids), _p(type_ids), pad_id, n, seq_len, d, _p(dword), _p(dpos), _p(dtype_tab),
+                                      _p(dgamma), _p(dbeta), _p(partial_ws), _p(type_partial_ws), _p(dx), _stream()), "imt_embed_ln_bwd")
+    return dx
 
 
 def _attn_args(q, k, v, B, H, Tq, Tk, head_dim, key_mask, query_mask, mask3d, causal, scale, dropout_p, dropout_seed):
diff --git a/include/imt_hip.h b/include/imt_hip.h
--- a/include/imt_hip.h
+++ b/include/imt_hip.h
@@ -96,6 +96,11 @@
 int imt_embed_bwd(int dtype, const int64_t* ids, const int64_t* pos_ids, const int64_t* type_ids,
                   const void* dsum, float* dword, float* dpos, float* dtype_tab, int n_tokens, int seq_len, int d,
                   int64_t pad_id, void* stream);
+int imt_embed_ln_bwd(int dtype, const void* dy, const void* emb_sum, const void* gamma, const float* mean,
+                     const float* rstd, float y_dropout_p, uint64_t y_dropout_seed, const int64_t* ids,
+                     const int64_t* pos_ids, const int64_t* type_ids, int64_t pad_id, int n_tokens, int seq_len, int d,
+                     float* dword, float* dpos, float* dtype_tab, float* dgamma, float* dbeta, float* partial_ws,
+                     float* type_partial_ws, void* dx, void* stream);
 int imt_embed_ln_fwd(int dtype, const int64_t* ids, const int64_t* pos_ids, const int64_t* type_ids, const void* word,
                      const void* pos, const void* type, const void* gamma, const void* beta, void* sum_out, void* y,
                      float* mean, float* rstd, int n_tokens, int seq_len, int d, int vocab, int max_pos, int n_types, float eps,
```
